# apple/ml-neuman

Measured on AMD Instinct MI355X. Metric: rays_per_sec (800x800 frame, 128 samples/ray coarse + 128 importance, NeuMan background NeRF), higher is better.
Workload: dtype coarse (sampling) pass: split-fp16 hi+lo MFMA x3, f32 accumulate; fine (shading) pass: per-row-scaled int16 as two int8 limbs on the i8 MFMA x3, exact int32 accumulate, encodings on split bf16

## Files before the change

include/neuman_hip.h:

```cpp
#ifndef NEUMAN_HIP_H
#define NEUMAN_HIP_H

#include <stdint.h>

#ifdef __cplusplus
extern "C" {
#endif

#define NM_OK 0
#define NM_ERR_ARG (-1)
#define NM_ERR_HIP (-2)
#define NM_ERR_UNSUPPORTED (-3)

#define NM_ABI_VERSION 1

typedef void* nm_stream_t;

#define NM_PREC_FP32 0
#define NM_PREC_BF16X3 1
#define NM_PREC_BF16 2
#define NM_PREC_I8X3 3
#define NM_PREC_FP16X3 4

#define NM_PE_POSENC 0
#define NM_PE_ROTATE 1

int nm_version(void);
const char* nm_last_error(void);
int nm_device_count(void);

int nm_ray_to_samples(const float* origin, const float* direction, const float* near, const float* far,
                      int64_t R, int S, const float* t_vals, int lindisp, const float* t_rand,
                      float* pts, float* dirs, float* z_vals, nm_stream_t stream);

int nm_z_to_points(const float* origin, const float* direction, const float* z_vals, int64_t R, int S,
                   float* pts, float* dirs, nm_stream_t stream);

int nm_composite(const float* raw, const float* z_vals, const float* rays_d, int64_t R, int S, int white_bkg,
                 const float* noise, float* rgb, float* disp, float* acc, float* weights, float* depth,
                 nm_stream_t stream);

int nm_sample_pdf(const float* bins, const float* weights, int64_t R, int B, const float* u, int N,
                  float* samples, nm_stream_t stream);
int nm_importance_z(const float* z_vals, const float* weights, int64_t R, int S, const float* u, int N,
                    int including_old, float* z_out, nm_stream_t stream);

int nm_near_far(const float* origin, const float* direction, int64_t R, const float* verts, int V, double geo_threshold,
                float* near, float* far, nm_stream_t stream);
int64_t nm_compact_workspace_ints(int64_t R);
int nm_compact_hits(const float* near, const float* far, int64_t R, int32_t* hit_idx, int32_t* miss_idx,
                    int32_t* counts, int32_t* workspace, nm_stream_t stream);

typedef struct nm_mlp_s* nm_mlp_t;

typedef struct nm_mlp_desc {
    int32_t depth;
    int32_t width;
    int32_t skip;
    int32_t pe_kind;
    int32_t pos_n_freqs;
    int32_t dir_n_freqs;
    int32_t plain_head;
} nm_mlp_desc;

int64_t nm_mlp_pack_bytes(const nm_mlp_desc* desc);
int nm_mlp_pack(const nm_mlp_desc* desc, const float* const* host_params, void* host_out);
int nm_mlp_pack_f16(const nm_mlp_desc* desc, const float* const* host_params, void* host_out);
int64_t nm_mlp_pack_i8_bytes(const nm_mlp_desc* desc);
int nm_mlp_pack_i8(const nm_mlp_desc* desc, const float* const* host_params, void* host_out);
int64_t nm_mlp_pack_i8s_bytes(const nm_mlp_desc* desc);
int nm_mlp_pack_i8s(const nm_mlp_desc* desc, const float* const* host_params, void* host_out);
int nm_mlp_create(const nm_mlp_desc* desc, const float* const* host_params, const float* host_pos_tab,
                  const float* host_dir_tab, nm_mlp_t* out);
int nm_mlp_destroy(nm_mlp_t mlp);

int nm_mlp_forward(nm_mlp_t mlp, const float* pts, const float* dirs, int64_t n, int precision,
                   float sigma_scale, float* out, nm_stream_t stream);
int nm_mlp_refresh_f16(nm_mlp_t mlp, const float* const* dev_params, nm_stream_t stream);
int nm_mlp_forward_save(nm_mlp_t mlp, const float* pts, const float* dirs, int64_t n, float* save_h, float* save_hv,
                        float* out, nm_stream_t stream);
int nm_mlp_forward_save_bits(nm_mlp_t mlp, const float* pts, const float* dirs, int64_t n, float* save_h, float* save_hv,
                             uint32_t* save_bits, float* out, nm_stream_t stream);
int64_t nm_mlp_backward_chain_workspace_floats(int64_t n);
int nm_mlp_backward_chain(nm_mlp_t mlp, const float* const* dev_params, const float* dz_top, const float* d_feat, const float* d_raw,
                          const float* acts, const uint32_t* relu_bits, int64_t n, float* dz_out, float* bias_grads, float* workspace,
                          int64_t workspace_floats, nm_stream_t stream);
int nm_mlp_forward_save16(nm_mlp_t mlp, const float* pts, const float* dirs, int64_t n, uint16_t* save_h16, float* save_feat, uint16_t* save_feat16,
                          float* save_hv, uint32_t* save_bits, uint32_t* save_hvbits, uint16_t* save_x0h, uint16_t* save_d0h, float* out,
                          nm_stream_t stream);
int nm_mlp_backward_chain16(nm_mlp_t mlp, const float* const* dev_params, const float* d_feat, const float* d_raw, const uint32_t* relu_bits,
                            int64_t n, const float* amax, uint16_t* dz16, uint16_t* dfeat16, float* dz32_layer5, float* dz32_layer0,
                            float* bias_grads, float* workspace, int64_t workspace_floats, nm_stream_t stream);
int nm_mlp_backward_plain16(nm_mlp_t mlp, const float* const* dev_params, const float* d_out, const uint32_t* relu_bits, int64_t n, const float* amax,
                            uint16_t* dz16, float* dz32_layer5, float* dz32_layer0, float* bias_grads, float* workspace, int64_t workspace_floats,
                            nm_stream_t stream);
int nm_mlp_backward_net16(nm_mlp_t mlp, const float* const* dev_params, const float* d_raw, const float* d_feat_add, const uint32_t* relu_bits,
                          const uint32_t* hv_bits, int64_t n, const float* amax, uint16_t* dz16, uint16_t* dfeat16, uint16_t* dhv16, float* dz32_layer5, float* dz32_layer0,
                          float* dhv32, float* bias_grads, float* workspace, int64_t workspace_floats, nm_stream_t stream);
int nm_mlp_forward_rays(nm_mlp_t mlp, const float* origin, const float* direction, const float* z_vals,
                        int64_t R, int S, int precision, float sigma_scale, float* out, nm_stream_t stream);
int nm_mlp_sigma_rays(nm_mlp_t mlp, const float* origin, const float* direction, const float* z_vals,
                      int64_t R, int S, int precision, float sigma_scale, float* out, nm_stream_t stream);
int nm_mlp_forward_ray_chunk(nm_mlp_t mlp, const float* origin, const float* direction, const float* z_vals, int S_total,
                             const int32_t* ray_idx, const int32_t* n_rays_dev, int64_t n_rays, int s0, int S, int precision,
                             float sigma_scale, float* out, nm_stream_t stream);
int nm_mlp_sigma_ray_chunk(nm_mlp_t mlp, const float* origin, const float* direction, const float* z_vals, int S_total,
                           const int32_t* ray_idx, const int32_t* n_rays_dev, int64_t n_rays, int s0, int S, int precision,
                           float sigma_scale, float* out, nm_stream_t stream);
float nm_occ_probe_offset(int probes, int seed, int k, int axis);
int64_t nm_occ_build_workspace_floats(int res, int probes);
int nm_occ_build(nm_mlp_t mlp, const float* aabb, int res, int probes, int dilate, float sigma_threshold, int seed, int precision,
                 float* workspace, int64_t workspace_floats, uint32_t* bits, nm_stream_t stream);
int64_t nm_occ_compact_workspace_ints(int64_t n_samples);
int nm_occ_compact_samples(const uint32_t* bits, int res, const float* aabb, const float* origin, const float* direction, const float* z_vals,
                           int64_t R, int S, int32_t* sample_idx, int32_t* counts, int32_t* workspace, nm_stream_t stream);
int nm_mlp_forward_samples(nm_mlp_t mlp, const float* origin, const float* direction, const float* z_vals, int64_t R, int S,
                           const int32_t* sample_idx, const int32_t* n_dev, int64_t n_max, int precision, float sigma_scale, float* out,
                           nm_stream_t stream);
int nm_mlp_sigma_samples(nm_mlp_t mlp, const float* origin, const float* direction, const float* z_vals, int64_t R, int S,
                         const int32_t* sample_idx, const int32_t* n_dev, int64_t n_max, int precision, float sigma_scale, float* out,
                         nm_stream_t stream);
int nm_occ_compact_points(const uint32_t* bits, int res, const float* aabb, const float* pts, int64_t n, int32_t* point_idx, int32_t* counts,
                          int32_t* workspace, nm_stream_t stream);
int nm_mlp_forward_listed(nm_mlp_t mlp, const float* pts, const float* dirs, int64_t n_points, const int32_t* point_idx, const int32_t* n_dev,
                          int64_t n_max, int precision, float sigma_scale, float* out, nm_stream_t stream);
int nm_transmittance_chunk(const float* raw, const float* z_vals, const float* rays_d, const int32_t* ray_idx, const int32_t* n_rays_dev,
                           int64_t n_rays, int s0, int S, int S_total, float* T, nm_stream_t stream);
int nm_transmittance_chunk_dz(const float* raw, const float* dz, const float* rays_d, const int32_t* ray_idx, const int32_t* n_rays_dev,
                              int64_t n_rays, int s0, int S, int S_total, float* T, nm_stream_t stream);
int nm_mlp_sigma_f16t_debug(nm_mlp_t mlp, const float* pts, const float* dirs, int64_t n, int stage, float* state, float* out, nm_stream_t stream);
int nm_mlp_forward_debug(nm_mlp_t mlp, const float* pts, const float* dirs, int64_t n, int precision,
                         int stage, float* hidden, nm_stream_t stream);
int nm_mlp_forward_profile(nm_mlp_t mlp, const float* pts, const float* dirs, int64_t n, int precision, float* out,
                           uint64_t* cycles, nm_stream_t stream);

#define NM_SEARCH_TREE 0
#define NM_SEARCH_ALL 1
#define NM_SEARCH_TREE_WIDE 2
typedef struct nm_mesh_s* nm_mesh_t;
int nm_mesh_create(const float* verts, int V, const int32_t* faces, int F, int search, nm_mesh_t* out,
                   nm_stream_t stream);
int nm_mesh_update(nm_mesh_t mesh, const float* verts, nm_stream_t stream);
int nm_mesh_destroy(nm_mesh_t mesh);
int nm_mesh_info(nm_mesh_t mesh, int32_t* levels, int64_t* nodes, int64_t* bytes);
int nm_warp_to_canonical(nm_mesh_t mesh, const float* pts, int64_t R, int S, const double* T, float* can_pts,
                         float* can_dirs, float* closest, nm_stream_t stream);
int nm_signed_distance(nm_mesh_t mesh, const float* pts, int64_t N, float* sdist, int32_t* face, float* closest,
                       nm_stream_t stream);

int nm_warp_apply_forward(const float* T, const int32_t* tri, const float* bary, const float* pts, int64_t N, float* can, nm_stream_t stream);
int nm_warp_apply_backward(const float* T, const int32_t* tri, const float* bary, const float* pts, const float* g_can, int64_t N, int64_t V,
                           float* g_T, float* g_bary, nm_stream_t stream);
int nm_bary_forward(const float* verts, const int32_t* tri, const float* closest, int64_t N, float* bary, nm_stream_t stream);
int nm_bary_backward(const float* verts, const int32_t* tri, const float* closest, const float* g_bary, int64_t N, int64_t V, float* g_verts,
                     nm_stream_t stream);

typedef struct nm_smpl_s* nm_smpl_t;
int nm_smpl_create(const float* v_template, const float* shapedirs, const float* j_regressor, const int32_t* parents,
                   const float* lbs_weights, const float* da_pose, int V, int J, int NB, nm_smpl_t* out);
int nm_smpl_destroy(nm_smpl_t smpl);
int64_t nm_smpl_vertex_workspace_floats(nm_smpl_t smpl);
int nm_smpl_vertex_forward(nm_smpl_t smpl, const float* pose, const float* beta, const double* alignment, double scale, const float* da_pose,
                           float* workspace, float* world_out, float* T_out, nm_stream_t stream);
int nm_smpl_vertex_backward(nm_smpl_t smpl, const float* pose, const float* beta, const double* alignment, double scale, const float* da_pose,
                            const float* g_world, const float* g_T, float* workspace, float* g_pose, float* g_beta, float* g_align,
                            nm_stream_t stream);
int nm_smpl_frames(nm_smpl_t smpl, const float* poses, const float* betas, const double* alignments, int B, double scale,
                   int precise, double* T_out, float* world_out, float* static_out, nm_stream_t stream);

int64_t nm_render_rays_bkg_workspace_floats(int64_t R, int S, int N);
int nm_render_rays_bkg(nm_mlp_t coarse, nm_mlp_t fine, const float* origin, const float* direction, const float* near, const float* far,
                       int64_t R, int S, int N, const float* t_vals, const float* u, int white_bkg, int precision_coarse, int precision_fine,
                       float* workspace, float* raw_out, float* z_out, float* rgb, float* depth, float* acc, nm_stream_t stream);
int64_t nm_render_rays_human_workspace_floats(int64_t R, int S, int posed);
int nm_render_rays_human(nm_mlp_t human, nm_mesh_t mesh, const double* T, const float* origin, const float* direction, const float* near,
                         const float* far, int64_t R, int S, const float* t_vals, int white_bkg, float sigma_scale, int precision,
                         float* workspace, float* raw_out, float* z_out, float* rgb, float* depth, float* acc, nm_stream_t stream);
int64_t nm_render_rays_human_occ_workspace_floats(int64_t R, int S, int posed);
int nm_render_rays_human_occ(nm_mlp_t human, nm_mesh_t mesh, const double* T, const uint32_t* bits, int res, const float* aabb, const float* origin,
                             const float* direction, const float* near, const float* far, int64_t R, int S, const float* t_vals, int white_bkg,
                             float sigma_scale, int precision, float* workspace, float* raw_out, float* z_out, int32_t* counts, float* rgb, float* depth,
                             float* acc, nm_stream_t stream);
int64_t nm_render_rays_hybrid_workspace_floats(int64_t R, int S, int N, int S_human);
int nm_render_rays_hybrid(nm_mlp_t coarse, nm_mlp_t fine, nm_mlp_t human, nm_mesh_t mesh, const double* T, const float* verts, int V,
                          double geo_threshold, const float* origin, const float* direction, int64_t R, float bkg_near, float bkg_far, int S, int N,
                          int S_human, const float* t_vals, const float* u, const float* t_vals_human, int white_bkg, int precision_coarse,
                          int precision_fine, int precision_human, float* workspace, float* rgb, float* depth, float* acc, nm_stream_t stream);
int nm_merge_composite_lists(int k, const float* const* z, const float* const* raw, const int32_t* const* rows, const int* S, int64_t R,
                             const float* rays_d, int white_bkg, float* rgb, float* depth, float* acc, nm_stream_t stream);
int nm_importance_from_raw(const float* raw, const float* z_vals, const float* rays_d, int64_t R, int S, const float* u, int N, float* z_out,
                           float* weights_out, nm_stream_t stream);
int nm_merged_intervals(int k, const float* const* z, const int* S, int64_t R, float* const* dz, nm_stream_t stream);
int64_t nm_merge_composite_workspace_floats(int64_t R, int Sa, int Sb);
int nm_merge_composite(const float* za, const float* rawa, int Sa, const float* zb, const float* rawb, int Sb, int64_t R, const float* rays_d,
                       int white_bkg, float* workspace, float* rgb, float* depth, float* acc, nm_stream_t stream);

int nm_merge_sorted(const float* za, const float* rawa, int Sa, const float* zb, const float* rawb, int Sb,
                    int64_t R, float* z_out, float* raw_out, nm_stream_t stream);

int nm_gather_rows(const float* src, const int32_t* idx, const int32_t* n_dev, int64_t n_max, int width,
                   float* dst, nm_stream_t stream);
int nm_scatter_rows(const float* src, const int32_t* idx, const int32_t* n_dev, int64_t n_max, int width,
                    float* dst, nm_stream_t stream);

int nm_shot_rays(const int32_t* xy, int64_t n, int width, int mode, const double* inv_intrinsic,
                 const double* cam2world, float* origin, float* direction, nm_stream_t stream);

int nm_shot_rays_cams(const int32_t* xy, const int32_t* cam_id, int64_t n, int mode, const double* cams,
                      int n_cams, float* origin, float* direction, nm_stream_t stream);

int nm_frame_to_uint8(const float* src, int64_t n, uint8_t* dst, nm_stream_t stream);
int nm_ssd_u8(const uint8_t* a, const uint8_t* b, int64_t n, uint64_t* ssd, nm_stream_t stream);
#define NM_SSIM_WORKSPACE_DOUBLES 4096
int nm_ssim_u8(const uint8_t* a, const uint8_t* b, int H, int W, int C, double* ssim, double* workspace, nm_stream_t stream);

#define NM_GEMM_ACCUMULATE 1
#define NM_GEMM_BIAS 2
#define NM_GEMM_RELU 4
#define NM_GEMM_MASK 8
#define NM_GEMM_COLSUM 16
int64_t nm_gemm_workspace_floats(int M, int N, int K);
int nm_gemm_f32(int a_kmajor, int b_kmajor, int M, int N, int K, const float* A, int lda, const float* B, int ldb, float* C,
                int ldc, const float* bias, const float* mask, int ldmask, int flags, float* workspace,
                int64_t workspace_floats, nm_stream_t stream);
int nm_gemm_bf16x3(int a_kmajor, int b_kmajor, int M, int N, int K, const float* A, int lda, const float* B, int ldb, float* C,
                   int ldc, const float* bias, const float* mask, int ldmask, int flags, float* workspace,
                   int64_t workspace_floats, nm_stream_t stream);
int nm_gemm_fp16x3(int a_kmajor, int b_kmajor, int M, int N, int K, const float* A, int lda, const float* B, int ldb, float* C,
                   int ldc, const float* bias, const float* mask, int ldmask, int flags, float* workspace,
                   int64_t workspace_floats, nm_stream_t stream);
int nm_pe_encode(const float* x, int64_t n, int dims, int kind, int n_freqs, const float* table, float* out, int ld,
                 nm_stream_t stream);
int nm_pe_encode16(const float* x, int64_t n, int dims, int kind, int n_freqs, const float* table, uint16_t* out, int ld, int ones_col,
                   nm_stream_t stream);
int nm_absmax(const float* x, int64_t count, float* out_max, nm_stream_t stream);
int64_t nm_wgrad16_workspace_floats(int nprod, int64_t n, int p_cols, int q_cols);
int nm_wgrad16(int nprod, int p_cols, int q_cols, const uint16_t* const* dz16, const uint16_t* const* act16, float* const* dW, const int* ldw,
               int64_t n, const float* amax, float* workspace, int64_t workspace_floats, nm_stream_t stream);
int64_t nm_wgrad_heads16_workspace_floats(int64_t n);
int nm_wgrad_heads16(const float* d_raw, const uint16_t* h16_7, const float* hv, int64_t n, float* out644, float* amax, float* workspace,
                     int64_t workspace_floats, nm_stream_t stream);
int64_t nm_wgrad_out16_workspace_floats(int64_t n);
int nm_wgrad_out16(const float* d_out, const uint16_t* h16_7, int64_t n, float* out1028, float* amax, float* workspace, int64_t workspace_floats,
                   nm_stream_t stream);
int64_t nm_wgrad_alpha16_workspace_floats(int64_t n);
int nm_wgrad_alpha16(const float* d_raw, const uint16_t* h16, int64_t n, float* out, float* workspace, int64_t workspace_floats,
                     nm_stream_t stream);
int64_t nm_colsum_workspace_floats(int64_t n, int W);
int nm_colsum(const float* X, int64_t n, int W, int ld, float* out, float* workspace, int64_t workspace_floats, nm_stream_t stream);
int nm_pe_backward(const float* x, int64_t n, int dims, int kind, int n_freqs, const float* table, const float* g, int ld,
                   float* dx, nm_stream_t stream);
int nm_composite_backward(const float* raw, const float* z_vals, const float* rays_d, int64_t R, int S, int white_bkg,
                          const float* g_rgb, const float* g_acc, const float* g_depth, const float* g_weights,
// ... 15 lines not shown
```

ml-neuman_amd/csrc/mlp_host.hip:

```cpp
#include <math.h>
#include <stdarg.h>
#include <stdio.h>
#include <stdlib.h>
#include <string.h>

#include <algorithm>
#include <vector>

#include "common.h"
#include "mlp_layout.h"
#include "mlp_launch.h"

namespace nm {

static thread_local char g_err[512] = "";

void set_error(const char* fmt, ...) {
    va_list ap;
    va_start(ap, fmt);
    vsnprintf(g_err, sizeof(g_err), fmt, ap);
    va_end(ap);
}
int check_hip(hipError_t e, const char* what) {
    if (e == hipSuccess) return NM_OK;
// ... 289 lines not shown
    }
}

static void pack_image8(const nm_mlp_desc* d, const float* const* P, uint8_t* img) {
    memset(img, 0, (size_t)image8_bytes());
    float* units = reinterpret_cast<float*>(img + kWeightBytes8 + kWeightPadBytes);
    float* bias = units + kBiasFloats;
    float* kappa = bias + kBiasFloats;
    const int kpe = 3 + 6 * d->pos_n_freqs, kdpe = 3 + 6 * d->dir_n_freqs;
    std::vector<double> est_in(288, 0.0), est(288, 0.0);
    for (int st = 0; st < kStages; ++st) {
        const StageShape8 sh = stage_shape8(st);
        const int nh = sh.i8steps * 32;
        const int nrows = sh.nblk * 32;
        float* u = units + stage_b_off(st);
        float* b = bias + stage_b_off(st);
        if (st <= 7) memcpy(b, P[P_PTS_W + 2 * st + 1], 256 * 4);
        else if (d->plain_head) { if (st == 8) memcpy(b + 256, P[P_OUT_B], 4 * 4); }
        else if (st == 8) { memcpy(b, P[P_FEAT_B], 256 * 4); b[256] = P[P_ALPHA_B][0]; }
        else if (st == 9) memcpy(b, P[P_VIEWS_B], 128 * 4);
        else memcpy(b, P[P_RGB_B], 3 * 4);
        kappa[st] = 1.f;
        for (int n = 0; n < nrows; ++n) u[n] = 1.f;
        for (int n = 0; n < nrows; ++n) {
            double v = (double)b[n] * b[n];
            const float* pe = nullptr;
            int npe = 0;
            if (st == 0) { pe = P[P_PTS_W] + (int64_t)n * kpe; npe = kpe; }
            else if (st == 5) { pe = P[P_PTS_W + 10] + (int64_t)n * (kpe + 256); npe = kpe; }
            else if (st == 9 && !d->plain_head) { pe = P[P_VIEWS_W] + (int64_t)n * (256 + kdpe) + 256; npe = kdpe; }
            for (int f = 0; f < npe; ++f) v += (double)pe[f] * pe[f];
            int col0 = 0;
            const float* row = sh.i8steps ? hidden_row(d, P, st, n, &col0) : nullptr;
            if (row) for (int f = 0; f < nh; ++f) { const double w = (double)row[col0 + f] * est_in[f]; v += w * w; }
            est[n] = sqrt(v);
        }
        if (sh.i8steps) {
            const float* uin = units + stage_b_off(st - 1);
            std::vector<float> q(nrows, 0.f);
            float kap = 0.f;
            for (int n = 0; n < nrows; ++n) {
                int col0 = 0;
                const float* row = hidden_row(d, P, st, n, &col0);
                float mx = 0.f;
                if (row) for (int f = 0; f < nh; ++f) mx = fmaxf(mx, fabsf(row[col0 + f] * uin[f]));
                q[n] = mx / (float)kFixedMax;
            }
            std::vector<double> stored;
            for (int n = 0; n < nrows; ++n) if (q[n] > 0.f) stored.push_back(est[n] / q[n]);
            if (!stored.empty()) {
                std::nth_element(stored.begin(), stored.begin() + stored.size() / 2, stored.end());
                const double cap = (double)kUnitOutlier * stored[stored.size() / 2];
                for (int n = 0; n < nrows; ++n) {
                    int col0 = 0;
                    if (hidden_row(d, P, st, n, &col0) && cap > 0.0 && est[n] > cap * q[n]) q[n] = (float)(est[n] / cap);
                }
            }
            const int nxt = st == 10 ? -1 : st + 1, nfeed = st == 9 ? 128 : 256;
            if (nxt > 0 && !(d->plain_head && nxt > 8)) {
                std::vector<double> c(nfeed, 0.0), g;
                for (int m = 0; m < stage_shape8(nxt).nblk * 32; ++m) {
                    int col0 = 0;
                    const float* row = hidden_row(d, P, nxt, m, &col0);
                    if (row) for (int n = 0; n < nfeed; ++n) c[n] = fmax(c[n], fabs((double)row[col0 + n]));
                }
                for (int n = 0; n < nfeed; ++n) if (q[n] > 0.f && c[n] > 0.0) g.push_back(q[n] * c[n]);
                if (!g.empty()) {
                    std::nth_element(g.begin(), g.begin() + g.size() / 2, g.end());
                    const double med = g[g.size() / 2], top = *std::max_element(g.begin(), g.end());
                    if (top > (double)kBalanceFrom * med) {
                        std::vector<double> qs;
                        double qtop = 0.0;
                        for (int n = 0; n < nfeed; ++n) if (q[n] > 0.f && c[n] > 0.0) { qs.push_back(q[n]); if (q[n] * c[n] == top) qtop = q[n]; }
                        std::nth_element(qs.begin(), qs.begin() + qs.size() / 2, qs.end());
                        const bool row_outlier = qtop > (double)kBalanceFrom * qs[qs.size() / 2];
                        const double floor_g = row_outlier ? sqrt(top * med) : cbrt(top * med * med);
                        for (int n = 0; n < nfeed; ++n)
                            if (q[n] > 0.f && c[n] > 0.0 && q[n] * c[n] < floor_g) q[n] = (float)(floor_g / c[n]);
                    }
                }
            }
            for (int n = 0; n < nrows; ++n) kap = fmaxf(kap, q[n]);
            if (!(kap > 0.f)) kap = 1.f;
            kappa[st] = kap;
            for (int n = 0; n < nrows; ++n) {
                if (!(q[n] > 0.f)) q[n] = kap;
                u[n] = q[n] / kap;
            }
            for (int nb = 0; nb < sh.nblk; ++nb)
                for (int r = 0; r < 32; ++r) {
                    const int n = 32 * nb + r;
                    int col0 = 0;
                    const float* row = hidden_row(d, P, st, n, &col0);
                    for (int t = 0; t < sh.i8steps; ++t) {
                        int8_t* hi = reinterpret_cast<int8_t*>(img + frag_off8(st, nb, t));
                        int8_t* lo = hi + 1024;
                        for (int g = 0; g < 2; ++g)
                            for (int e = 0; e < 16; ++e) {
                                const int f = slot_feature8(2 * t + g, e);
                                const float w = row ? row[col0 + f] * uin[f] : 0.f;
                                int v = (int)lrintf(w / q[n]);
                                if (v > kFixedMax) v = kFixedMax;
                                if (v < -kFixedMax) v = -kFixedMax;
                                const int l = ((v + 128) & 255) - 128;
                                const int h = (v - l) >> 8;
                                hi[(g * 32 + r) * 16 + e] = (int8_t)h;
                                lo[(g * 32 + r) * 16 + e] = (int8_t)l;
                            }
                    }
                }
        }
        for (int n = 0; n < nrows; ++n) b[n] /= u[n];
        est_in.swap(est);
        for (int nb = 0; nb < sh.nblk; ++nb)
            for (int t = 0; t < sh.bfsteps; ++t) {
                uint16_t* hi = reinterpret_cast<uint16_t*>(img + frag_off8(st, nb, sh.i8steps + t));
                uint16_t* lo = hi + 64 * 8;
                const int cc0 = st == 9 ? 32 : 0;
                for (int lane = 0; lane < 64; ++lane)
                    for (int j = 0; j < 8; ++j) {
                        const int n = 32 * nb + (lane & 31);
                        const float wv = stage_weight(d, P, st, n, cc0 + 2 * t + (lane >> 5), j) / u[n];
                        const uint16_t h = f32_to_bf16(wv);
                        hi[lane * 8 + j] = h;
                        lo[lane * 8 + j] = f32_to_bf16(wv - bf16_to_f32(h));
                    }
            }
    }
}

static void pack_stream8s(const uint8_t* img8, uint8_t* out, bool plain = false) {
    memset(out, 0, (size_t)(kWeightBytes8 + kWeightPadBytes));
    uint8_t* dst = out;
    auto put = [&](int st, int nb, int t0, int n) {
        for (int t = 0; t < n; ++t, dst += kStepBytes) memcpy(dst, img8 + frag_off8(st, nb, t0 + t), (size_t)kStepBytes);
    };
    for (int nb = 0; nb < 8; ++nb) put(0, nb, 0, 4);
    for (int st = 1; st <= 7; ++st) {
        for (int nb = 0; nb < 8; ++nb) put(st, nb, 0, 8);
        if (st == 5)
            for (int nb = 0; nb < 8; ++nb) put(5, nb, 8, 4);
    }
    put(8, 8, 0, 8);
    if (plain) {
        for (int nb = 0; nb < 2; ++nb) { put(0, nb, 0, 4); dst += 4 * kStepBytes; }
        if (dst - out != kPlainStreamBytes8) abort();
        return;
    }
    for (int nb = 0; nb < 8; ++nb) put(8, nb, 0, 8);
    for (int nb = 0; nb < 4; ++nb) put(9, nb, 0, 10);
    put(10, 0, 0, 4);
    if (dst - out != kWeightBytes8) abort();
}

constexpr int kSigmaSteps = 8 * 4 + 6 * 8 * 16 + 8 * 20 + 16;
static void sigma_stream_table(std::vector<int>& tab, int ndir) {
    tab.clear();
    std::vector<int> direct;
    auto put = [&](int st, int b, int t0, int n) {
        for (int t = 0; t < n; ++t)
            for (int k = 0; k < 4; ++k) {
                const int off = (int)frag_off(st, b + (k >> 1), t0 + t) + 1024 * (k & 1);
                (k < 4 - ndir ? tab : direct).push_back(off);
            }
    };
    for (int st = 0; st <= 7; ++st) {
        const StageShape sh = stage_shape(st);
        for (int b = 0; b < 8; b += 2) {
            if (sh.pe_steps) put(st, b, 0, sh.pe_steps);
            for (int t0 = sh.pe_steps; t0 < sh.steps; t0 += 8) put(st, b, t0, 8);
        }
    }
    for (int t = 0; t < 16; ++t) { tab.push_back((int)frag_off(8, 8, t)); tab.push_back((int)frag_off(8, 8, t) + 1024); }
    tab.insert(tab.end(), direct.begin(), direct.end());
    if ((int)tab.size() != 2 * kSigmaSteps) abort();
}
__global__ void sigma_stream_kernel(const uint4* __restrict__ image, const int* __restrict__ tab, int npieces, uint4* __restrict__ out) {
    const int i = blockIdx.x * blockDim.x + threadIdx.x;
    if (i >= npieces * 64) return;
    out[i] = image[tab[i >> 6] / 16 + (i & 63)];
}

static void pack_stream8(const uint8_t* img8, uint8_t* out) {
    memset(out, 0, (size_t)kWeightBytes8w);
    for (int q = 0; q < 4; ++q) {
        uint8_t* dst = out + wstream_off(q);
        auto put = [&](int st, int nb, int t0, int n) {
            for (int t = 0; t < n; ++t, dst += kStepBytes) memcpy(dst, img8 + frag_off8(st, nb, t0 + t), (size_t)kStepBytes);
        };
        put(0, 2 * q, 0, 4); put(0, 2 * q + 1, 0, 4);
        for (int st = 1; st <= 8; ++st) {
            put(st, 2 * q, 0, 8); put(st, 2 * q + 1, 0, 8);
            if (st == 5) { put(5, 2 * q, 8, 4); put(5, 2 * q + 1, 8, 4); }
        }
        if (q < 2) put(8, 8, 0, 8);
        put(9, q, 0, 8); put(9, q, 8, 2);
        dst += 2 * kStepBytes;
        if (q < 2) put(10, 0, 0, 4);
        dst += kW8Pad * kStepBytes;
        if (dst != out + wstream_off(q) + (int64_t)wstream_steps(q) * kStepBytes) abort();
    }
}

}

struct nm_mlp_s {
    nm_mlp_desc desc;
    uint8_t* d_image;
    uint8_t* d_image16;
    float* d_consts8;
    uint8_t* d_stream8;
    uint8_t* d_image8;
    uint8_t* d_stream16t;
    int* d_sigma_tab;
    uint8_t* d_bwd_image;
    int sigma_ndir;
    float* d_petab;
    float* d_ref;
    float* d_wscale16;
    int ref_off[12], ref_boff[12];
    int pos_octaves, dir_octaves;
};

extern "C" {

int nm_version(void) { return NM_ABI_VERSION; }
const char* nm_last_error(void) { return nm::g_err; }
int nm_device_count(void) {
    int n = 0;
    if (hipGetDeviceCount(&n) != hipSuccess) { (void)hipGetLastError(); return 0; }
    return n;
}

int64_t nm_mlp_pack_bytes(const nm_mlp_desc* desc) {
    if (nm::validate_desc(desc) != NM_OK) return -1;
    return nm::image_bytes();
}

int nm_mlp_pack(const nm_mlp_desc* desc, const float* const* host_params, void* host_out) {
    if (int e = nm::validate_desc(desc)) return e;
    NM_REQUIRE(host_params && host_out, "nm_mlp_pack: null pointer");
    for (int i = 0; i < (desc->plain_head ? 18 : 24); ++i) NM_REQUIRE(host_params[i], "nm_mlp_pack: host_params[%d] is null", i);
    if (int e = nm::check_finite("nm_mlp_pack", desc, host_params)) return e;
    nm::pack_image(desc, host_params, static_cast<uint8_t*>(host_out));
    return NM_OK;
}

int nm_mlp_pack_f16(const nm_mlp_desc* desc, const float* const* host_params, void* host_out) {
    if (int e = nm::validate_desc(desc)) return e;
    NM_REQUIRE(host_params && host_out, "nm_mlp_pack_f16: null pointer");
    for (int i = 0; i < (desc->plain_head ? 18 : 24); ++i) NM_REQUIRE(host_params[i], "nm_mlp_pack_f16: host_params[%d] is null", i);
    if (int e = nm::check_finite("nm_mlp_pack_f16", desc, host_params)) return e;
    nm::pack_image(desc, host_params, static_cast<uint8_t*>(host_out), true);
    return NM_OK;
}

int64_t nm_mlp_pack_i8_bytes(const nm_mlp_desc* desc) {
    if (nm::validate_desc(desc) != NM_OK) return -1;
    return nm::image8_bytes();
}

int nm_mlp_pack_i8(const nm_mlp_desc* desc, const float* const* host_params, void* host_out) {
    if (int e = nm::validate_desc(desc)) return e;
    NM_REQUIRE(host_params && host_out, "nm_mlp_pack_i8: null pointer");
    for (int i = 0; i < (desc->plain_head ? 18 : 24); ++i) NM_REQUIRE(host_params[i], "nm_mlp_pack_i8: host_params[%d] is null", i);
    if (int e = nm::check_finite("nm_mlp_pack_i8", desc, host_params)) return e;
    nm::pack_image8(desc, host_params, static_cast<uint8_t*>(host_out));
    return NM_OK;
}

int64_t nm_mlp_pack_i8s_bytes(const nm_mlp_desc* desc) {
    if (nm::validate_desc(desc) != NM_OK) return -1;
    return nm::kWeightBytes8 + nm::kWeightPadBytes;
}

int nm_mlp_pack_i8s(const nm_mlp_desc* desc, const float* const* host_params, void* host_out) {
    if (int e = nm::validate_desc(desc)) return e;
    NM_REQUIRE(host_params && host_out, "nm_mlp_pack_i8s: null pointer");
    for (int i = 0; i < (desc->plain_head ? 18 : 24); ++i) NM_REQUIRE(host_params[i], "nm_mlp_pack_i8s: host_params[%d] is null", i);
    if (int e = nm::check_finite("nm_mlp_pack_i8s", desc, host_params)) return e;
    std::vector<uint8_t> img8((size_t)nm::image8_bytes());
    nm::pack_image8(desc, host_params, img8.data());
    nm::pack_stream8s(img8.data(), static_cast<uint8_t*>(host_out), desc->plain_head != 0);
    return NM_OK;
}

int nm_mlp_create(const nm_mlp_desc* desc, const float* const* host_params, const float* host_pos_tab,
                  const float* host_dir_tab, nm_mlp_t* out) {
    if (int e = nm::validate_desc(desc)) return e;
    NM_REQUIRE(host_params && host_pos_tab && host_dir_tab && out, "nm_mlp_create: null pointer");
    const int plain = desc->plain_head;
    for (int i = 0; i < (plain ? 18 : 24); ++i) NM_REQUIRE(host_params[i], "nm_mlp_create: host_params[%d] is null", i);
    if (int e = nm::check_finite("nm_mlp_create", desc, host_params)) return e;
    const int64_t bytes = nm_mlp_pack_bytes(desc);
    std::vector<uint8_t> img((size_t)bytes);
    nm::pack_image(desc, host_params, img.data());
    std::vector<uint8_t> img16((size_t)bytes);
    nm::pack_image(desc, host_params, img16.data(), true);
    std::vector<uint8_t> img8((size_t)nm::image8_bytes());
    std::vector<uint8_t> str8((size_t)nm::kWeightBytes8w);
    std::vector<uint8_t> str8s((size_t)(nm::kWeightBytes8 + nm::kWeightPadBytes));
    nm::pack_image8(desc, host_params, img8.data());
    nm::pack_stream8(img8.data(), str8.data());
    nm::pack_stream8s(img8.data(), str8s.data(), plain != 0);

    const int kpe = 3 + 6 * desc->pos_n_freqs, kdpe = 3 + 6 * desc->dir_n_freqs;
    const int K[12] = {kpe, 256, 256, 256, 256, kpe + 256, 256, 256, plain ? 0 : 256 + kdpe, plain ? 0 : 256, 256, plain ? 0 : 128};
    const int N[12] = {256, 256, 256, 256, 256, 256, 256, 256, plain ? 0 : 128, plain ? 0 : 256, plain ? 4 : 1, plain ? 0 : 3};
    const int src[12] = {0, 2, 4, 6, 8, 10, 12, 14, 16, 18, plain ? (int)nm::P_OUT_W : 20, 22};
    nm_mlp_s* m = new nm_mlp_s();
    m->desc = *desc;
    int woff = 0;
    for (int l = 0; l < 12; ++l) { m->ref_off[l] = woff; woff += K[l] * N[l]; }
    int boff = woff;
    for (int l = 0; l < 12; ++l) { m->ref_boff[l] = boff; boff += N[l]; }
    std::vector<float> ref((size_t)boff);
    for (int l = 0; l < 12; ++l) {
        if (!K[l]) continue;
        const float* W = host_params[src[l]];
        for (int k = 0; k < K[l]; ++k)
            for (int n = 0; n < N[l]; ++n) ref[m->ref_off[l] + (size_t)k * N[l] + n] = W[(size_t)n * K[l] + k];
        memcpy(&ref[m->ref_boff[l]], host_params[src[l] + 1], (size_t)N[l] * 4);
    }
    float tab[192];
    memset(tab, 0, sizeof(tab));
    const int npos = desc->pe_kind == NM_PE_POSENC ? desc->pos_n_freqs : 9 * desc->pos_n_freqs;
    const int ndir = desc->pe_kind == NM_PE_POSENC ? desc->dir_n_freqs : 9 * desc->dir_n_freqs;
    memcpy(tab, host_pos_tab, (size_t)npos * 4);
    memcpy(tab + 96, host_dir_tab, (size_t)ndir * 4);
    auto octaves = [&](const float* t, int nfreq) {
        const int per = desc->pe_kind == NM_PE_POSENC ? 1 : 9;
        for (int b = 0; b + 1 < nfreq; ++b)
            for (int k = 0; k < per; ++k)
                if (t[(b + 1) * per + k] != 2.f * t[b * per + k]) return 0;
        return 1;
    };
    m->pos_octaves = octaves(tab, desc->pos_n_freqs);
    m->dir_octaves = octaves(tab + 96, desc->dir_n_freqs);

    m->d_image = nullptr; m->d_image16 = nullptr; m->d_consts8 = nullptr; m->d_stream8 = nullptr; m->d_image8 = nullptr; m->d_stream16t = nullptr; m->d_sigma_tab = nullptr; m->d_bwd_image = nullptr; m->d_petab = nullptr; m->d_ref = nullptr; m->d_wscale16 = nullptr;
    int rc = nm::check_hip(hipMalloc(&m->d_image, (size_t)bytes), "nm_mlp_create: hipMalloc(image)");
    const size_t consts_off = (size_t)(nm::kWeightBytes8 + nm::kWeightPadBytes), consts_bytes = img8.size() - consts_off;
    if (!rc) rc = nm::check_hip(hipMalloc(&m->d_consts8, consts_bytes), "nm_mlp_create: hipMalloc(consts8)");
    if (!rc) rc = nm::check_hip(hipMemcpy(m->d_consts8, img8.data() + consts_off, consts_bytes, hipMemcpyHostToDevice), "nm_mlp_create: upload consts8");
    if (!rc) rc = nm::check_hip(hipMalloc(&m->d_stream8, str8.size()), "nm_mlp_create: hipMalloc(stream8)");
    if (!rc) rc = nm::check_hip(hipMemcpy(m->d_stream8, str8.data(), str8.size(), hipMemcpyHostToDevice), "nm_mlp_create: upload stream8");
    if (!rc) rc = nm::check_hip(hipMalloc(&m->d_image8, consts_off), "nm_mlp_create: hipMalloc(image8)");
    if (!rc) rc = nm::check_hip(hipMemcpy(m->d_image8, str8s.data(), consts_off, hipMemcpyHostToDevice), "nm_mlp_create: upload image8");
    if (!rc) rc = nm::check_hip(hipMalloc(&m->d_petab, sizeof(tab)), "nm_mlp_create: hipMalloc(petab)");
    if (!rc) rc = nm::check_hip(hipMalloc(&m->d_ref, ref.size() * 4), "nm_mlp_create: hipMalloc(ref)");
    if (!rc) rc = nm::check_hip(hipMemcpy(m->d_image, img.data(), (size_t)bytes, hipMemcpyHostToDevice), "nm_mlp_create: upload image");
    if (!rc) rc = nm::check_hip(hipMalloc(&m->d_image16, (size_t)bytes), "nm_mlp_create: hipMalloc(image16)");
    if (!rc) rc = nm::check_hip(hipMemcpy(m->d_image16, img16.data(), (size_t)bytes, hipMemcpyHostToDevice), "nm_mlp_create: upload image16");
    if (!rc) rc = nm::check_hip(hipMemcpy(m->d_petab, tab, sizeof(tab), hipMemcpyHostToDevice), "nm_mlp_create: upload petab");
    if (!rc) rc = nm::check_hip(hipMemcpy(m->d_ref, ref.data(), ref.size() * 4, hipMemcpyHostToDevice), "nm_mlp_create: upload ref");
    if (!rc && !plain) {
        std::vector<int> stab;
        m->sigma_ndir = nm::sigma_f16t_ndir();
        nm::sigma_stream_table(stab, m->sigma_ndir);
        rc = nm::check_hip(hipMalloc(&m->d_sigma_tab, stab.size() * sizeof(int)), "nm_mlp_create: hipMalloc(sigma table)");
        if (!rc) rc = nm::check_hip(hipMemcpy(m->d_sigma_tab, stab.data(), stab.size() * sizeof(int), hipMemcpyHostToDevice), "nm_mlp_create: upload sigma table");
        if (!rc) rc = nm::check_hip(hipMalloc(&m->d_stream16t, (size_t)nm::kSigmaSteps * nm::kStepBytes), "nm_mlp_create: hipMalloc(stream16t)");
        if (!rc) {
            const int n16 = nm::kSigmaSteps * (nm::kStepBytes / 16);
            hipLaunchKernelGGL(nm::sigma_stream_kernel, dim3((n16 + 255) / 256), dim3(256), 0, 0, reinterpret_cast<const uint4*>(m->d_image16), m->d_sigma_tab,
                               2 * nm::kSigmaSteps, reinterpret_cast<uint4*>(m->d_stream16t));
            rc = nm::check_launch("sigma_stream_kernel");
            if (!rc) rc = nm::check_hip(hipDeviceSynchronize(), "nm_mlp_create: sigma stream");
        }
    }
    if (rc) { nm_mlp_destroy(m); return rc; }
    *out = m;
    return NM_OK;
}

int nm_mlp_refresh_f16(nm_mlp_t m, const float* const* dev_params, nm_stream_t stream) {
    NM_REQUIRE(m && dev_params, "nm_mlp_refresh_f16: null pointer");
    nm::DevParams P;
    const int need = m->desc.plain_head ? 18 : 24;
    for (int i = 0; i < 24; ++i) {
        NM_REQUIRE(i >= need || dev_params[i], "nm_mlp_refresh_f16: dev_params[%d] is null", i);
        P.p[i] = i < need ? dev_params[i] : nullptr;
    }
    if (!m->d_wscale16)
        if (int rc = nm::check_hip(hipMalloc(&m->d_wscale16, 3 * nm::kStages * sizeof(float)), "nm_mlp_refresh_f16: hipMalloc")) return rc;
    hipStream_t st = nm::as_stream(stream);
    float* bias = reinterpret_cast<float*>(m->d_image16 + nm::kWeightBytes + nm::kWeightPadBytes);
    unsigned* scale_work = reinterpret_cast<unsigned*>(m->d_wscale16 + nm::kStages);
    if (int rc = nm::check_hip(hipMemsetAsync(scale_work, 0, 2 * nm::kStages * sizeof(unsigned), st), "nm_mlp_refresh_f16: clear")) return rc;
    hipLaunchKernelGGL(nm::f16_stage_scale_kernel, dim3(nm::kStages, nm::kScaleSlices), dim3(1024), 0, st, m->desc, P, scale_work, m->d_wscale16);
    const int threads = (int)(nm::kWeightBytes / nm::kStepBytes) * 64;
    hipLaunchKernelGGL(nm::f16_pack_kernel, dim3((threads + 255) / 256), dim3(256), 0, st, m->desc, P, m->d_wscale16, m->d_image16);
    hipLaunchKernelGGL(nm::f16_bias_kernel, dim3((nm::kBiasFloats + nm::kF16TabFloats + 255) / 256), dim3(256), 0, st, P, m->d_wscale16, bias, m->desc.plain_head);
    if (m->d_stream16t) {
        const int n16 = nm::kSigmaSteps * (nm::kStepBytes / 16);
        hipLaunchKernelGGL(nm::sigma_stream_kernel, dim3((n16 + 255) / 256), dim3(256), 0, st, reinterpret_cast<const uint4*>(m->d_image16), m->d_sigma_tab,
                           2 * nm::kSigmaSteps, reinterpret_cast<uint4*>(m->d_stream16t));
    }
    return nm::check_launch("nm_mlp_refresh_f16");
}

int nm_mlp_destroy(nm_mlp_t m) {
    if (!m) return NM_OK;
    if (m->d_image) (void)hipFree(m->d_image);
    if (m->d_image16) (void)hipFree(m->d_image16);
    if (m->d_consts8) (void)hipFree(m->d_consts8);
    if (m->d_stream8) (void)hipFree(m->d_stream8);
    if (m->d_image8) (void)hipFree(m->d_image8);
    if (m->d_stream16t) (void)hipFree(m->d_stream16t);
    if (m->d_sigma_tab) (void)hipFree(m->d_sigma_tab);
    if (m->d_bwd_image) (void)hipFree(m->d_bwd_image);
    if (m->d_petab) (void)hipFree(m->d_petab);
    if (m->d_ref) (void)hipFree(m->d_ref);
    if (m->d_wscale16) (void)hipFree(m->d_wscale16);
    delete m;
    return NM_OK;
}

static int mlp_dispatch(nm_mlp_t m, const float* pts, const float* dirs, const float* origin, const float* direction,
                        const float* z, int64_t n, int S, int in_mode, int precision, int stop_stage, float sigma_scale,
                        float* out, float* dbg, nm_stream_t stream, void* prof = nullptr, int sigma_only = 0,
                        const nm::MlpChunk* chunk = nullptr) {
    NM_REQUIRE(m, "nm_mlp_forward: null handle");
    NM_REQUIRE(n >= 0, "nm_mlp_forward: negative n");
    NM_REQUIRE(precision == NM_PREC_FP32 || precision == NM_PREC_BF16X3 || precision == NM_PREC_BF16 || precision == NM_PREC_I8X3 ||
                   precision == NM_PREC_FP16X3,
               "nm_mlp_forward: bad precision %d", precision);
    if (n == 0) return NM_OK;
    NM_REQUIRE(!(chunk && precision == NM_PREC_FP32), "nm_mlp_forward_ray_chunk: the exact-f32 validation kernel has no chunked form");
    NM_REQUIRE(!(m->desc.plain_head && precision == NM_PREC_I8X3 && (stop_stage != -2 || dbg || prof || sigma_only)),
               "nm_mlp_forward: the plain-head (use_viewdirs=False) net's i8x3 form is the whole-network launch only (no stage-by-stage / density-only form)");
    NM_REQUIRE(!(m->desc.plain_head && stop_stage > 7), "nm_mlp_forward_debug: the plain-head net has stages -1..7 only");
    if (precision == NM_PREC_FP32) {
        nm::RefLaunch L;
        L.plain_head = m->desc.plain_head;
        L.wt = m->d_ref; L.bias = m->d_ref; L.petab = m->d_petab;
        for (int i = 0; i < 12; ++i) { L.off[i] = m->ref_off[i]; L.boff[i] = m->ref_boff[i]; }
        L.pe_kind = m->desc.pe_kind; L.pos_nfreq = m->desc.pos_n_freqs; L.dir_nfreq = m->desc.dir_n_freqs;
        return nm::launch_mlp_ref(L, pts, dirs, origin, direction, z, n, S, in_mode, stop_stage, sigma_scale, out, dbg,
                                  nm::as_stream(stream));
    }
    nm::MlpLaunch L;
    L.wpack = m->d_image;
    L.bias = reinterpret_cast<const float*>(m->d_image + nm::kWeightBytes + nm::kWeightPadBytes);
    L.wpack16 = m->d_image16;
    L.bias16 = reinterpret_cast<const float*>(m->d_image16 + nm::kWeightBytes + nm::kWeightPadBytes);
    L.petab = m->d_petab;
    L.pe_kind = m->desc.pe_kind; L.pos_nfreq = m->desc.pos_n_freqs; L.dir_nfreq = m->desc.dir_n_freqs;
    L.pos_octaves = m->pos_octaves; L.dir_octaves = m->dir_octaves;
    L.plain_head = m->desc.plain_head;
    L.wstream8 = m->d_stream8;
    L.consts8 = m->d_consts8;
    static const bool i8_as = [] { const char* e = getenv("NEUMAN_I8_KERNEL"); return !e || !strcmp(e, "as"); }();
    const char* sk = getenv("NEUMAN_SIGMA_KERNEL");
    const bool sigma_t = !(sk && !strcmp(sk, "w")) && m->d_stream16t;
    if (sigma_t && precision == NM_PREC_FP16X3 && sigma_only == 1 && stop_stage == -2 && !dbg && !prof && !m->desc.plain_head)
        return nm::launch_sigma_f16t(L, m->d_stream16t, m->sigma_ndir, pts, dirs, origin, direction, z, n, S, in_mode, sigma_scale, out, nm::as_stream(stream), chunk, nullptr, -1);
    if ((i8_as || m->desc.plain_head) && precision == NM_PREC_I8X3 && stop_stage == -2 && !dbg && !prof && !sigma_only)
        return nm::launch_mlp_i8s(L, m->d_image8, pts, dirs, origin, direction, z, n, S, in_mode, sigma_scale, out, nm::as_stream(stream), chunk);
    return nm::launch_mlp_mfma(L, pts, dirs, origin, direction, z, n, S, in_mode, precision, stop_stage, sigma_scale, out, dbg,
                               prof, nm::as_stream(stream), sigma_only, chunk);
}

int nm_mlp_forward(nm_mlp_t mlp, const float* pts, const float* dirs, int64_t n, int precision, float sigma_scale,
                   float* out, nm_stream_t stream) {
    NM_REQUIRE(n == 0 || (pts && dirs && out), "nm_mlp_forward: null pointer");
    NM_REQUIRE((reinterpret_cast<uintptr_t>(out) & 15) == 0, "nm_mlp_forward: out must be 16-byte aligned");
    return mlp_dispatch(mlp, pts, dirs, nullptr, nullptr, nullptr, n, 1, 0, precision, -2, sigma_scale, out, nullptr, stream);
}

int nm_mlp_forward_save(nm_mlp_t m, const float* pts, const float* dirs, int64_t n, float* save_h, float* save_hv, float* out,
                        nm_stream_t stream) {
    return nm_mlp_forward_save_bits(m, pts, dirs, n, save_h, save_hv, nullptr, out, stream);
}

static int forward_save_impl(nm_mlp_t m, const float* pts, const float* dirs, int64_t n, float* save_h, float* save_hv, uint32_t* save_bits,
                             void* save_h16, float* out, nm_stream_t stream, void* save_feat16 = nullptr, uint32_t* save_hvbits = nullptr,
                             void* save_x0h = nullptr, void* save_d0h = nullptr) {
    NM_REQUIRE(m, "nm_mlp_forward_save: null handle");
    NM_REQUIRE(n >= 0, "nm_mlp_forward_save: negative n");
    if (n == 0) return NM_OK;
    const bool plain = m->desc.plain_head != 0;
    NM_REQUIRE(!plain || (save_h16 && !save_h && !save_feat16 && !save_hvbits && !save_d0h), "nm_mlp_forward_save: the plain-head net keeps save_h16 / save_bits / save_x0h only");
    NM_REQUIRE(pts && (dirs || plain) && (plain || ((save_h || (save_h16 && save_feat16)) && save_hv)) && out, "nm_mlp_forward_save: null pointer");
    NM_REQUIRE(((reinterpret_cast<uintptr_t>(out) | reinterpret_cast<uintptr_t>(save_h) | reinterpret_cast<uintptr_t>(save_hv) | reinterpret_cast<uintptr_t>(save_h16) |
                 reinterpret_cast<uintptr_t>(save_feat16)) & 15) == 0, "nm_mlp_forward_save: outputs must be 16-byte aligned");
    nm::MlpLaunch L;
    L.wpack = m->d_image;
    L.bias = reinterpret_cast<const float*>(m->d_image + nm::kWeightBytes + nm::kWeightPadBytes);
    L.wpack16 = m->d_image16;
    L.bias16 = reinterpret_cast<const float*>(m->d_image16 + nm::kWeightBytes + nm::kWeightPadBytes);
    L.petab = m->d_petab;
    L.pe_kind = m->desc.pe_kind; L.pos_nfreq = m->desc.pos_n_freqs; L.dir_nfreq = m->desc.dir_n_freqs;
    L.pos_octaves = m->pos_octaves; L.dir_octaves = m->dir_octaves;
    L.plain_head = plain ? 1 : 0;
    L.wstream8 = m->d_stream8;
    L.consts8 = m->d_consts8;
    L.save_h = save_h; L.save_hv = save_hv; L.save_bits = save_bits; L.save_h16 = save_h16; L.save_feat16 = save_feat16; L.save_hvbits = save_hvbits; L.save_x0h = save_x0h; L.save_d0h = save_d0h;
    return nm::launch_mlp_mfma(L, pts, dirs ? dirs : pts, nullptr, nullptr, nullptr, n, 1, 0, NM_PREC_FP16X3, -2, 1.f, out, nullptr, nullptr,
                               nm::as_stream(stream), 0, nullptr);
}

int nm_mlp_forward_save_bits(nm_mlp_t m, const float* pts, const float* dirs, int64_t n, float* save_h, float* save_hv, uint32_t* save_bits,
                             float* out, nm_stream_t stream) {
    return forward_save_impl(m, pts, dirs, n, save_h, save_hv, save_bits, nullptr, out, stream);
}

int nm_mlp_forward_save16(nm_mlp_t m, const float* pts, const float* dirs, int64_t n, uint16_t* save_h16, float* save_feat, uint16_t* save_feat16,
                          float* save_hv, uint32_t* save_bits, uint32_t* save_hvbits, uint16_t* save_x0h, uint16_t* save_d0h, float* out, nm_stream_t stream) {
    NM_REQUIRE(n == 0 || (save_h16 && save_bits && (save_feat || save_feat16 || (m && m->desc.plain_head))), "nm_mlp_forward_save16: null pointer");
    NM_REQUIRE(((reinterpret_cast<uintptr_t>(save_x0h) | reinterpret_cast<uintptr_t>(save_d0h)) & 15) == 0, "nm_mlp_forward_save16: outputs must be 16-byte aligned");
    return forward_save_impl(m, pts, dirs, n, save_feat, save_hv, save_bits, save_h16, out, stream, save_feat16, save_hvbits, save_x0h, save_d0h);
}

int64_t nm_mlp_backward_chain_workspace_floats(int64_t n) { return ((n + nm::kTileM - 1) / nm::kTileM) * 9 * 256; }

int nm_mlp_backward_chain(nm_mlp_t m, const float* const* dev_params, const float* dz_top, const float* d_feat, const float* d_raw, const float* acts,
                          const uint32_t* relu_bits, int64_t n, float* dz_out, float* bias_grads, float* workspace, int64_t workspace_floats,
                          nm_stream_t stream) {
    NM_REQUIRE(m && dev_params, "nm_mlp_backward_chain: null pointer");
    NM_REQUIRE(n >= 0, "nm_mlp_backward_chain: negative n");
    if (n == 0) return NM_OK;
    NM_REQUIRE((dz_top || (d_feat && d_raw)) && (acts || relu_bits) && dz_out && bias_grads && workspace, "nm_mlp_backward_chain: null pointer");
    NM_REQUIRE(!d_feat || !m->desc.plain_head, "nm_mlp_backward_chain: the plain-head net has no feature layer (pass dz_top)");
    NM_REQUIRE(workspace_floats >= nm_mlp_backward_chain_workspace_floats(n), "nm_mlp_backward_chain: workspace of %lld floats, %lld needed",
               (long long)workspace_floats, (long long)nm_mlp_backward_chain_workspace_floats(n));
    NM_REQUIRE(((reinterpret_cast<uintptr_t>(dz_top) | reinterpret_cast<uintptr_t>(d_feat) | reinterpret_cast<uintptr_t>(d_raw) | reinterpret_cast<uintptr_t>(acts) |
                 reinterpret_cast<uintptr_t>(dz_out) | reinterpret_cast<uintptr_t>(workspace)) & 15) == 0, "nm_mlp_backward_chain: buffers must be 16-byte aligned");
    nm::DevParams P;
    const int need = d_feat ? 24 : 16;
    for (int i = 0; i < 24; ++i) {
        NM_REQUIRE(i >= need || dev_params[i], "nm_mlp_backward_chain: dev_params[%d] is null", i);
        P.p[i] = i < need ? dev_params[i] : nullptr;
    }
    if (!m->d_bwd_image)
        if (int rc = nm::check_hip(hipMalloc(&m->d_bwd_image, (size_t)nm::mlp_bwd_image_bytes()), "nm_mlp_backward_chain: hipMalloc")) return rc;
    return nm::launch_mlp_bwd(P, 3 + 6 * m->desc.pos_n_freqs, m->d_bwd_image, dz_top, d_feat, d_raw, acts, relu_bits, n, dz_out, workspace, bias_grads,
                              nm::as_stream(stream));
}

int nm_mlp_backward_chain16(nm_mlp_t m, const float* const* dev_params, const float* d_feat, const float* d_raw, const uint32_t* relu_bits, int64_t n,
                            const float* amax, uint16_t* dz16, uint16_t* dfeat16, float* dz32_layer5, float* dz32_layer0, float* bias_grads,
                            float* workspace, int64_t workspace_floats, nm_stream_t stream) {
    NM_REQUIRE(m && dev_params, "nm_mlp_backward_chain16: null pointer");
    NM_REQUIRE(n >= 0, "nm_mlp_backward_chain16: negative n");
    if (n == 0) return NM_OK;
    NM_REQUIRE(d_feat && d_raw && relu_bits && amax && dz16 && bias_grads && workspace, "nm_mlp_backward_chain16: null pointer");
    NM_REQUIRE(!m->desc.plain_head, "nm_mlp_backward_chain16: the plain-head net has no feature layer");
    NM_REQUIRE(workspace_floats >= nm_mlp_backward_chain_workspace_floats(n), "nm_mlp_backward_chain16: workspace of %lld floats, %lld needed",
               (long long)workspace_floats, (long long)nm_mlp_backward_chain_workspace_floats(n));
    NM_REQUIRE(((reinterpret_cast<uintptr_t>(d_feat) | reinterpret_cast<uintptr_t>(d_raw) | reinterpret_cast<uintptr_t>(dz16) | reinterpret_cast<uintptr_t>(dfeat16) |
                 reinterpret_cast<uintptr_t>(dz32_layer5) | reinterpret_cast<uintptr_t>(dz32_layer0) | reinterpret_cast<uintptr_t>(workspace)) & 15) == 0,
               "nm_mlp_backward_chain16: buffers must be 16-byte aligned");
    nm::DevParams P;
    for (int i = 0; i < 24; ++i) {
        NM_REQUIRE(dev_params[i], "nm_mlp_backward_chain16: dev_params[%d] is null", i);
        P.p[i] = dev_params[i];
    }
    if (!m->d_bwd_image)
        if (int rc = nm::check_hip(hipMalloc(&m->d_bwd_image, (size_t)nm::mlp_bwd_image_bytes()), "nm_mlp_backward_chain16: hipMalloc")) return rc;
    nm::Bwd16 h;
    h.dz16 = dz16; h.dfeat16 = dfeat16; h.amax = amax;
    for (int i = 0; i < 8; ++i) h.dz32[i] = nullptr;
    h.dz32[5] = dz32_layer5; h.dz32[0] = dz32_layer0;
    return nm::launch_mlp_bwd(P, 3 + 6 * m->desc.pos_n_freqs, m->d_bwd_image, nullptr, d_feat, d_raw, nullptr, relu_bits, n, nullptr, workspace, bias_grads,
                              nm::as_stream(stream), &h);
}

int nm_mlp_backward_net16(nm_mlp_t m, const float* const* dev_params, const float* d_raw, const float* d_feat_add, const uint32_t* relu_bits,
                          const uint32_t* hv_bits, int64_t n, const float* amax, uint16_t* dz16, uint16_t* dfeat16, uint16_t* dhv16, float* dz32_layer5, float* dz32_layer0, float* dhv32,
                          float* bias_grads, float* workspace, int64_t workspace_floats, nm_stream_t stream) {
    NM_REQUIRE(m && dev_params, "nm_mlp_backward_net16: null pointer");
    NM_REQUIRE(n >= 0, "nm_mlp_backward_net16: negative n");
    if (n == 0) return NM_OK;
    NM_REQUIRE(d_raw && relu_bits && hv_bits && amax && dz16 && dfeat16 && dhv16 && bias_grads && workspace, "nm_mlp_backward_net16: null pointer");
    NM_REQUIRE(!m->desc.plain_head, "nm_mlp_backward_net16: the plain-head net has no views layer");
    NM_REQUIRE(workspace_floats >= nm_mlp_backward_chain_workspace_floats(n), "nm_mlp_backward_net16: workspace of %lld floats, %lld needed",
               (long long)workspace_floats, (long long)nm_mlp_backward_chain_workspace_floats(n));
    NM_REQUIRE(((reinterpret_cast<uintptr_t>(d_raw) | reinterpret_cast<uintptr_t>(d_feat_add) | reinterpret_cast<uintptr_t>(dz16) | reinterpret_cast<uintptr_t>(dfeat16) |
                 reinterpret_cast<uintptr_t>(dhv16) | reinterpret_cast<uintptr_t>(dz32_layer5) | reinterpret_cast<uintptr_t>(dz32_layer0) | reinterpret_cast<uintptr_t>(dhv32) |
                 reinterpret_cast<uintptr_t>(workspace)) & 15) == 0, "nm_mlp_backward_net16: buffers must be 16-byte aligned");
    nm::DevParams P;
    for (int i = 0; i < 24; ++i) {
        NM_REQUIRE(dev_params[i], "nm_mlp_backward_net16: dev_params[%d] is null", i);
        P.p[i] = dev_params[i];
    }
    NM_REQUIRE((reinterpret_cast<uintptr_t>(P.p[nm::P_RGB_W]) & 15) == 0, "nm_mlp_backward_net16: rgb_linear.weight must be 16-byte aligned");
    if (!m->d_bwd_image)
        if (int rc = nm::check_hip(hipMalloc(&m->d_bwd_image, (size_t)nm::mlp_bwd_image_bytes()), "nm_mlp_backward_net16: hipMalloc")) return rc;
    nm::Bwd16 h;
    h.dz16 = dz16; h.dfeat16 = dfeat16; h.amax = amax;
    for (int i = 0; i < 8; ++i) h.dz32[i] = nullptr;
    h.dz32[5] = dz32_layer5; h.dz32[0] = dz32_layer0;
    h.hvbits = hv_bits; h.dhv16 = dhv16; h.dhv32 = dhv32; h.kdir = 3 + 6 * m->desc.dir_n_freqs;
    return nm::launch_mlp_bwd(P, 3 + 6 * m->desc.pos_n_freqs, m->d_bwd_image, nullptr, d_feat_add, d_raw, nullptr, relu_bits, n, nullptr, workspace, bias_grads,
                              nm::as_stream(stream), &h);
}

int nm_mlp_backward_plain16(nm_mlp_t m, const float* const* dev_params, const float* d_out, const uint32_t* relu_bits, int64_t n, const float* amax,
                            uint16_t* dz16, float* dz32_layer5, float* dz32_layer0, float* bias_grads, float* workspace, int64_t workspace_floats,
                            nm_stream_t stream) {
    NM_REQUIRE(m && dev_params, "nm_mlp_backward_plain16: null pointer");
    NM_REQUIRE(n >= 0, "nm_mlp_backward_plain16: negative n");
    if (n == 0) return NM_OK;
    NM_REQUIRE(d_out && relu_bits && amax && dz16 && bias_grads && workspace, "nm_mlp_backward_plain16: null pointer");
    NM_REQUIRE(m->desc.plain_head, "nm_mlp_backward_plain16: the net has the view-dependent head (nm_mlp_backward_net16)");
    NM_REQUIRE(workspace_floats >= nm_mlp_backward_chain_workspace_floats(n), "nm_mlp_backward_plain16: workspace of %lld floats, %lld needed",
               (long long)workspace_floats, (long long)nm_mlp_backward_chain_workspace_floats(n));
    NM_REQUIRE(((reinterpret_cast<uintptr_t>(d_out) | reinterpret_cast<uintptr_t>(dz16) | reinterpret_cast<uintptr_t>(dz32_layer5) | reinterpret_cast<uintptr_t>(dz32_layer0) |
                 reinterpret_cast<uintptr_t>(workspace)) & 15) == 0, "nm_mlp_backward_plain16: buffers must be 16-byte aligned");
    nm::DevParams P;
    for (int i = 0; i < 24; ++i) {
        NM_REQUIRE(i >= 18 || dev_params[i], "nm_mlp_backward_plain16: dev_params[%d] is null", i);
        P.p[i] = i < 18 ? dev_params[i] : nullptr;
    }
    if (!m->d_bwd_image)
        if (int rc = nm::check_hip(hipMalloc(&m->d_bwd_image, (size_t)nm::mlp_bwd_image_bytes()), "nm_mlp_backward_plain16: hipMalloc")) return rc;
    nm::Bwd16 h;
    h.dz16 = dz16; h.dfeat16 = nullptr; h.amax = amax;
    for (int i = 0; i < 8; ++i) h.dz32[i] = nullptr;
    h.dz32[5] = dz32_layer5; h.dz32[0] = dz32_layer0;
    h.plain = 1;
    return nm::launch_mlp_bwd(P, 3 + 6 * m->desc.pos_n_freqs, m->d_bwd_image, nullptr, nullptr, d_out, nullptr, relu_bits, n, nullptr, workspace, bias_grads,
                              nm::as_stream(stream), &h);
}

int nm_mlp_forward_rays(nm_mlp_t mlp, const float* origin, const float* direction, const float* z_vals, int64_t R, int S,
                        int precision, float sigma_scale, float* out, nm_stream_t stream) {
    NM_REQUIRE(R == 0 || (origin && direction && z_vals && out), "nm_mlp_forward_rays: null pointer");
    NM_REQUIRE(R >= 0 && S >= 1, "nm_mlp_forward_rays: bad sizes");
    NM_REQUIRE((reinterpret_cast<uintptr_t>(out) & 15) == 0, "nm_mlp_forward_rays: out must be 16-byte aligned");
    return mlp_dispatch(mlp, nullptr, nullptr, origin, direction, z_vals, R * (int64_t)S, S, 1, precision, -2, sigma_scale, out,
                        nullptr, stream);
}

int nm_mlp_sigma_rays(nm_mlp_t mlp, const float* origin, const float* direction, const float* z_vals, int64_t R, int S,
                      int precision, float sigma_scale, float* out, nm_stream_t stream) {
    NM_REQUIRE(R == 0 || (origin && direction && z_vals && out), "nm_mlp_sigma_rays: null pointer");
    NM_REQUIRE(R >= 0 && S >= 1, "nm_mlp_sigma_rays: bad sizes");
    NM_REQUIRE((reinterpret_cast<uintptr_t>(out) & 15) == 0, "nm_mlp_sigma_rays: out must be 16-byte aligned");
    return mlp_dispatch(mlp, nullptr, nullptr, origin, direction, z_vals, R * (int64_t)S, S, 1, precision, -2, sigma_scale, out,
                        nullptr, stream, nullptr, 1);
}

int nm_mlp_forward_ray_chunk(nm_mlp_t mlp, const float* origin, const float* direction, const float* z_vals, int S_total,
                             const int32_t* ray_idx, const int32_t* n_rays_dev, int64_t n_rays, int s0, int S, int precision,
                             float sigma_scale, float* out, nm_stream_t stream) {
    NM_REQUIRE(n_rays == 0 || (origin && direction && z_vals && ray_idx && out), "nm_mlp_forward_ray_chunk: null pointer");
    NM_REQUIRE(n_rays >= 0 && S >= 1 && s0 >= 0 && s0 + S <= S_total, "nm_mlp_forward_ray_chunk: bad sizes (s0=%d S=%d S_total=%d)", s0, S, S_total);
    NM_REQUIRE((reinterpret_cast<uintptr_t>(out) & 15) == 0, "nm_mlp_forward_ray_chunk: out must be 16-byte aligned");
    nm::MlpChunk c{ray_idx, n_rays_dev, s0, S_total};
    return mlp_dispatch(mlp, nullptr, nullptr, origin, direction, z_vals, n_rays * (int64_t)S, S, 2, precision, -2, sigma_scale, out,
                        nullptr, stream, nullptr, 0, &c);
}

int nm_mlp_sigma_ray_chunk(nm_mlp_t mlp, const float* origin, const float* direction, const float* z_vals, int S_total,
                           const int32_t* ray_idx, const int32_t* n_rays_dev, int64_t n_rays, int s0, int S, int precision,
                           float sigma_scale, float* out, nm_stream_t stream) {
    NM_REQUIRE(n_rays == 0 || (origin && direction && z_vals && ray_idx && out), "nm_mlp_sigma_ray_chunk: null pointer");
    NM_REQUIRE(n_rays >= 0 && S >= 1 && s0 >= 0 && s0 + S <= S_total, "nm_mlp_sigma_ray_chunk: bad sizes (s0=%d S=%d S_total=%d)", s0, S, S_total);
    NM_REQUIRE((reinterpret_cast<uintptr_t>(out) & 15) == 0, "nm_mlp_sigma_ray_chunk: out must be 16-byte aligned");
    nm::MlpChunk c{ray_idx, n_rays_dev, s0, S_total};
    return mlp_dispatch(mlp, nullptr, nullptr, origin, direction, z_vals, n_rays * (int64_t)S, S, 2, precision, -2, sigma_scale, out,
                        nullptr, stream, nullptr, 1, &c);
}

static int forward_samples(const char* what, int sigma_only, nm_mlp_t mlp, const float* origin, const float* direction, const float* z_vals, int64_t R,
                           int S, const int32_t* sample_idx, const int32_t* n_dev, int64_t n_max, int precision, float sigma_scale, float* out,
                           nm_stream_t stream) {
    NM_REQUIRE(n_max == 0 || (origin && direction && z_vals && sample_idx && out), "%s: null pointer", what);
    NM_REQUIRE(R >= 0 && S >= 1 && n_max >= 0 && n_max <= R * (int64_t)S && R * (int64_t)S < (1ll << 31), "%s: bad sizes (R=%lld S=%d n_max=%lld)", what,
               (long long)R, S, (long long)n_max);
    NM_REQUIRE(precision != NM_PREC_FP32, "%s: the exact-f32 validation kernel has no sample-list form", what);
    NM_REQUIRE((reinterpret_cast<uintptr_t>(out) & 15) == 0, "%s: out must be 16-byte aligned", what);
    nm::MlpChunk c{sample_idx, n_dev, 0, S};
    return mlp_dispatch(mlp, nullptr, nullptr, origin, direction, z_vals, n_max, S, 3, precision, -2, sigma_scale, out, nullptr, stream, nullptr,
                        sigma_only, &c);
}

int nm_mlp_forward_samples(nm_mlp_t mlp, const float* origin, const float* direction, const float* z_vals, int64_t R, int S,
                           const int32_t* sample_idx, const int32_t* n_dev, int64_t n_max, int precision, float sigma_scale, float* out,
                           nm_stream_t stream) {
    return forward_samples("nm_mlp_forward_samples", 0, mlp, origin, direction, z_vals, R, S, sample_idx, n_dev, n_max, precision, sigma_scale, out, stream);
}

int nm_mlp_sigma_samples(nm_mlp_t mlp, const float* origin, const float* direction, const float* z_vals, int64_t R, int S,
                         const int32_t* sample_idx, const int32_t* n_dev, int64_t n_max, int precision, float sigma_scale, float* out,
                         nm_stream_t stream) {
    return forward_samples("nm_mlp_sigma_samples", 1, mlp, origin, direction, z_vals, R, S, sample_idx, n_dev, n_max, precision, sigma_scale, out, stream);
}

}

bool nm::mlp_plain_head(nm_mlp_t m) { return m && m->desc.plain_head; }

extern "C" {

int nm_mlp_forward_listed(nm_mlp_t mlp, const float* pts, const float* dirs, int64_t n_points, const int32_t* point_idx, const int32_t* n_dev,
                          int64_t n_max, int precision, float sigma_scale, float* out, nm_stream_t stream) {
    NM_REQUIRE(n_max == 0 || (pts && dirs && point_idx && out), "nm_mlp_forward_listed: null pointer");
    NM_REQUIRE(n_points >= 0 && n_max >= 0 && n_max <= n_points && n_points < (1ll << 31), "nm_mlp_forward_listed: bad sizes (n_points=%lld n_max=%lld)",
               (long long)n_points, (long long)n_max);
    NM_REQUIRE(precision != NM_PREC_FP32, "nm_mlp_forward_listed: the exact-f32 validation kernel has no point-list form");
    NM_REQUIRE((reinterpret_cast<uintptr_t>(out) & 15) == 0, "nm_mlp_forward_listed: out must be 16-byte aligned");
    nm::MlpChunk c{point_idx, n_dev, 0, 1};
    return mlp_dispatch(mlp, pts, dirs, nullptr, nullptr, nullptr, n_max, 1, 4, precision, -2, sigma_scale, out, nullptr, stream, nullptr, 0, &c);
}

int nm_mlp_forward_profile(nm_mlp_t mlp, const float* pts, const float* dirs, int64_t n, int precision, float* out,
                           uint64_t* cycles, nm_stream_t stream) {
    NM_REQUIRE(n == 0 || (pts && dirs && out && cycles), "nm_mlp_forward_profile: null pointer");
    NM_REQUIRE(precision == NM_PREC_BF16X3 || precision == NM_PREC_I8X3 || precision == NM_PREC_FP16X3,
               "nm_mlp_forward_profile: precision %d has no profiling build",
               precision);
    return mlp_dispatch(mlp, pts, dirs, nullptr, nullptr, nullptr, n, 1, 0, precision, -2, 1.f, out, nullptr, stream, cycles);
}

int nm_mlp_sigma_f16t_debug(nm_mlp_t mlp, const float* pts, const float* dirs, int64_t n, int stage, float* state, float* out, nm_stream_t stream) {
    NM_REQUIRE(mlp && pts && dirs && state && out && n > 0, "nm_mlp_sigma_f16t_debug: null pointer");
    NM_REQUIRE(stage >= 0 && stage % 100 <= 7 && !mlp->desc.plain_head, "nm_mlp_sigma_f16t_debug: stage %d outside 0..7 (+ 100 x tile round)", stage);
    nm::MlpLaunch L;
    L.petab = mlp->d_petab;
    L.pe_kind = mlp->desc.pe_kind; L.pos_nfreq = mlp->desc.pos_n_freqs; L.dir_nfreq = mlp->desc.dir_n_freqs;
    L.pos_octaves = mlp->pos_octaves; L.dir_octaves = mlp->dir_octaves;
    L.plain_head = 0;
    L.bias16 = reinterpret_cast<const float*>(mlp->d_image16 + nm::kWeightBytes + nm::kWeightPadBytes);
    return nm::launch_sigma_f16t(L, mlp->d_stream16t, mlp->sigma_ndir, pts, dirs, nullptr, nullptr, nullptr, n, 1, 0, 1.f, out, nm::as_stream(stream), nullptr, state, stage);
}

int nm_mlp_forward_debug(nm_mlp_t mlp, const float* pts, const float* dirs, int64_t n, int precision, int stage,
                         float* hidden, nm_stream_t stream) {
    NM_REQUIRE(n == 0 || (pts && dirs && hidden), "nm_mlp_forward_debug: null pointer");
    NM_REQUIRE(stage >= -1 && stage <= 9, "nm_mlp_forward_debug: stage %d outside -1..9", stage);
    return mlp_dispatch(mlp, pts, dirs, nullptr, nullptr, nullptr, n, 1, 0, precision, stage, 1.f, nullptr, hidden, stream);
}

}
```

ml-neuman_amd/csrc/mlp_i8as.h:

```cpp
#pragma once
#include "mlp_device.h"

namespace {

typedef __attribute__((ext_vector_type(4))) int i32x4;
typedef __attribute__((ext_vector_type(16))) int i32x16;
typedef __attribute__((ext_vector_type(2))) short i16x2;
typedef __attribute__((address_space(3))) const float lds_cfloat;
typedef __attribute__((ext_vector_type(4))) float vf4;
typedef __attribute__((address_space(3))) const vf4 lds_cvf4;

constexpr int kRows = 32;
struct Args8s {
    MlpArgs a;
    const float* consts8;
    const uint4* image8;
};

__device__ __forceinline__ i32x4 as_i32x4(uint4 v) { return __builtin_bit_cast(i32x4, v); }

template <bool F16 = false>
__device__ __forceinline__ void fill_pe_wave(uint4* pw, bool is_dir, const MlpArgs& a, int64_t base_row, int lane) {
    const PeSpec spec = is_dir ? a.dir : a.pos;
    const float* tab = a.petab + (is_dir ? 96 : 0);
    unsigned short* hi = reinterpret_cast<unsigned short*>(pw);
    auto put = [&](int row, int p, float v, bool clamp = false) {
        const int off = ((p >> 3) * (2 * kRows) + row) * 8 + (p & 7);
        if (F16) {
            float sv = v * kF16ActScale;
            if (clamp) sv = __builtin_amdgcn_fmed3f(sv, -65504.f, 65504.f);
            const _Float16 hb = (_Float16)sv;
            const _Float16 lb = (_Float16)(sv - (float)hb);
            hi[off] = __builtin_bit_cast(unsigned short, hb);
            hi[off + kRows * 8] = __builtin_bit_cast(unsigned short, lb);
            return;
        }
        const bf16x2 hb = __builtin_convertvector((f32x2){v, 0.f}, bf16x2);
        const f32x2 hf = __builtin_convertvector(hb, f32x2);
        const bf16x2 lb = __builtin_convertvector((f32x2){v - hf.x, 0.f}, bf16x2);
        hi[off] = (unsigned short)(__builtin_bit_cast(unsigned, hb) & 0xffffu);
        hi[off + kRows * 8] = (unsigned short)(__builtin_bit_cast(unsigned, lb) & 0xffffu);
    };
    if (spec.octaves) {
#pragma unroll 1
        for (int round = 0; round < 2; ++round) {
            const int j = 2 * round + (lane >> 5), row = lane & 31;
            if (j > 2) break;
            int64_t i = base_row + row;
            if (i >= a.n) i = a.n - 1;
            float x0, x1, x2;
            sample_input(a, i, is_dir, x0, x1, x2);
            const float xj = j == 0 ? x0 : (j == 1 ? x1 : x2);
            const float a0 = spec.kind == NM_PE_POSENC ? xj * tab[0] : fmaf(x2, tab[3 * j + 2], fmaf(x1, tab[3 * j + 1], x0 * tab[3 * j]));
            put(row, j, xj);
            double sn, cs;
            sincos_f64((double)a0, sn, cs);
            const int n3 = 3 * spec.nfreq;
            for (int b = 0; b < spec.nfreq; ++b) {
                if (spec.kind == NM_PE_POSENC) { put(row, 3 + 6 * b + j, (float)sn); put(row, 3 + 6 * b + 3 + j, (float)cs); }
                else { put(row, 3 + 3 * b + j, (float)sn); put(row, 3 + n3 + 3 * b + j, (float)cs); }
                const double s2 = 2.0 * sn * cs, c2 = 1.0 - 2.0 * sn * sn;
                sn = s2; cs = c2;
            }
        }
    } else {
        const int nchunks = is_dir ? 4 : nm::kPeChunks;
        for (int item = lane; item < nchunks * kRows; item += 64) {
            const int c = item >> 5, row = item & 31;
            int64_t i = base_row + row;
            if (i >= a.n) i = a.n - 1;
            float x0, x1, x2;
            sample_input(a, i, is_dir, x0, x1, x2);
#pragma unroll
            for (int e = 0; e < 8; ++e) put(row, 8 * c + e, pe_feature(8 * c + e, x0, x1, x2, spec, tab), true);
        }
    }
}

struct X8 {
    uint4 h[8], l[8];
};

__device__ __forceinline__ void glds16(const void* gsrc, unsigned lds_dst) {
    unsigned keep;
    asm volatile("s_mov_b32 %0, m0\n\ts_mov_b32 m0, %2\n\ts_nop 0\n\tglobal_load_lds_dwordx4 %1, off\n\ts_mov_b32 m0, %0"
                 : "=&s"(keep) : "v"(gsrc), "s"(lds_dst) : "memory");
}
__device__ __forceinline__ void bias16(f32x16& f, lds_cfloat* bias_blk) {
#pragma unroll
    for (int q = 0; q < 4; ++q) {
        const vf4 bs = *(lds_cvf4*)(bias_blk + 8 * q);
        f[4 * q] = bs.x; f[4 * q + 1] = bs.y; f[4 * q + 2] = bs.z; f[4 * q + 3] = bs.w;
    }
}
__device__ __forceinline__ void dequant16(f32x16& f, const i32x16& t, float sx256, lds_cfloat* bias_blk) {
#pragma unroll
    for (int q = 0; q < 4; ++q) {
        const vf4 bs = *(lds_cvf4*)(bias_blk + 8 * q);
        const float bsv[4] = {bs.x, bs.y, bs.z, bs.w};
#pragma unroll
        for (int j = 0; j < 4; ++j) f[4 * q + j] = fmaf((float)t[4 * q + j], sx256, bsv[j]);
    }
}
template <bool RELU>
__device__ __forceinline__ float max16(float m, const f32x16& f) {
#pragma unroll
    for (int r = 0; r < 16; ++r) m = fmaxf(m, RELU ? f[r] : fabsf(f[r]));
    return m;
}
__device__ __forceinline__ float row_max(float m) {
    typedef __attribute__((ext_vector_type(2))) unsigned u32x2;
    const u32x2 sw = __builtin_amdgcn_permlane32_swap(__float_as_uint(m), __float_as_uint(m), false, false);
    return fmaxf(__uint_as_float(sw.x), __uint_as_float(sw.y));
}
template <bool RELU>
__device__ __forceinline__ void quant16(const f32x16& f, float inv, uint4& xh, uint4& xl) {
    i16x2 P[8], Y[8];
#pragma unroll
    for (int i = 0; i < 8; ++i) {
        float y0 = f[2 * i] * inv, y1 = f[2 * i + 1] * inv;
        if (RELU) {
            y0 = __builtin_amdgcn_fmed3f(y0, 0.f, 1.f);
            y1 = __builtin_amdgcn_fmed3f(y1, 0.f, 1.f);
        }
        const i16x2 p = __builtin_amdgcn_cvt_pknorm_i16(y0, y1);
        P[i] = p;
        Y[i] = p + (i16x2){128, 128};
    }
    unsigned lo[4], hi[4];
#pragma unroll
    for (int k = 0; k < 4; ++k) {
        lo[k] = __builtin_amdgcn_perm(__builtin_bit_cast(unsigned, P[2 * k + 1]), __builtin_bit_cast(unsigned, P[2 * k]), 0x06040200u);
        hi[k] = __builtin_amdgcn_perm(__builtin_bit_cast(unsigned, Y[2 * k + 1]), __builtin_bit_cast(unsigned, Y[2 * k]), 0x07050301u);
    }
    xh = make_uint4(hi[0], hi[1], hi[2], hi[3]);
    xl = make_uint4(lo[0], lo[1], lo[2], lo[3]);
}
__device__ __forceinline__ float inv_of(float M) { return M > 0.f ? ((float)nm::kFixedMax / 32767.f) * __builtin_amdgcn_rcpf(M) : 0.f; }
__device__ __forceinline__ float scale_of(float M) { return M > 0.f ? M * (1.f / (float)nm::kFixedMax) : 1.f; }


}
```

ml-neuman_amd/csrc/mlp_i8s.hip:

```cpp
#include "mlp_i8as.h"

namespace {

constexpr int kWaves = 8;
constexpr int kTile = kWaves * kRows;
constexpr int kPWaveU4 = nm::kPeChunks * 2 * kRows;
constexpr int kPeU4 = kWaves * kPWaveU4;
constexpr int kStepU4 = nm::kStepBytes / 16;
constexpr int kSlotU4 = 12 * kStepU4;
constexpr int kSlots = 3;
constexpr int kBiasU4 = (nm::kBiasFloats + 16 + 3) / 4;
constexpr int kTileBlocks = 82;
__host__ __device__ constexpr int block_steps(int i) {
    i = i >= kTileBlocks ? i - kTileBlocks : i;
    return i < 8 ? 4 : i < 77 ? 8 : i < 81 ? 10 : 4;
}
__host__ __device__ constexpr int block_pieces(int nsteps) { return (2 * nsteps + kWaves - 1) / kWaves; }

struct Ring {
    const char* src;
    const uint4* rd;
    unsigned lds0;
    int off;
    int slot;
    int refill, np, nsteps2;
};
__device__ __forceinline__ void ring_piece(const Ring& R, int off, int slot, int j) {
    glds16(R.src + off + j * (kWaves * 1024), __builtin_amdgcn_readfirstlane(R.lds0 + slot * (kSlotU4 * 16) + j * (kWaves * 1024)));
}
__device__ __forceinline__ void ring_advance(Ring& R, int nsteps) {
    R.off += nsteps * nm::kStepBytes;
    if (R.off == (int)nm::kWeightBytes8) R.off = 0;
}
__device__ __forceinline__ const uint4* ring_enter(Ring& R, int i) {
    const int np1 = block_pieces(block_steps(i + 1));
    if (np1 == 1) asm volatile("s_waitcnt vmcnt(1)" ::: "memory");
    else if (np1 == 2) asm volatile("s_waitcnt vmcnt(2)" ::: "memory");
    else asm volatile("s_waitcnt vmcnt(3)" ::: "memory");
    __builtin_amdgcn_s_barrier();
    const uint4* cur = R.rd + R.slot * kSlotU4;
    R.refill = R.slot == 0 ? kSlots - 1 : R.slot - 1;
    R.slot = R.slot == kSlots - 1 ? 0 : R.slot + 1;
    R.np = block_pieces(block_steps(i + 2));
    R.nsteps2 = block_steps(i + 2);
    return cur;
}
__device__ __forceinline__ void ring_copy(Ring& R, int j) {
    if (j < R.np) ring_piece(R, R.off, R.refill, j);
    if (j == R.np - 1) ring_advance(R, R.nsteps2);
}
struct W8 {
    uint4 h, l;
};

template <int NSTEPS, bool PEND, bool RELU = true>
__device__ __forceinline__ void k_i8_impl(i32x16& t, const X8& X, const uint4* ws, Ring& R, f32x16& fp, const i32x16& tp, lds_cfloat* bias_blk,
                                          float sx256, float& m) {
    i32x16 ah, ac;
#pragma unroll
    for (int r = 0; r < 16; ++r) { ah[r] = 0; ac[r] = 0; }
    W8 w[2];
    w[0].h = ws[0]; w[0].l = ws[64];
    w[1].h = ws[kStepU4]; w[1].l = ws[kStepU4 + 64];
#pragma unroll
    for (int s = 0; s < NSTEPS; ++s) {
        const uint4 wh = w[s & 1].h, wl = w[s & 1].l;
        ac = __builtin_amdgcn_mfma_i32_32x32x32_i8(as_i32x4(wh), as_i32x4(X.l[s]), ac, 0, 0, 0);
        ah = __builtin_amdgcn_mfma_i32_32x32x32_i8(as_i32x4(wh), as_i32x4(X.h[s]), ah, 0, 0, 0);
        ac = __builtin_amdgcn_mfma_i32_32x32x32_i8(as_i32x4(wl), as_i32x4(X.h[s]), ac, 0, 0, 0);
        if (s + 2 < NSTEPS) { w[s & 1].h = ws[(s + 2) * kStepU4]; w[s & 1].l = ws[(s + 2) * kStepU4 + 64]; }
        if (s == 0 || s == 2 || s == 4) ring_copy(R, s >> 1);
        if (PEND) {
            const int r = 2 * s;
            const float b0 = bias_blk[8 * (r >> 2) + (r & 3)], b1 = bias_blk[8 * (r >> 2) + (r & 3) + 1];
            const float f0 = fmaf((float)tp[r], sx256, b0), f1 = fmaf((float)tp[r + 1], sx256, b1);
            fp[r] = f0;
            fp[r + 1] = f1;
            m = RELU ? fmaxf(m, fmaxf(f0, f1)) : fmaxf(m, fmaxf(fabsf(f0), fabsf(f1)));
            __builtin_amdgcn_sched_barrier(0);
        }
    }
#pragma unroll
    for (int r = 0; r < 16; ++r) t[r] = (ah[r] << 8) + ac[r];
}
template <int NSTEPS>
__device__ __forceinline__ void k_i8(i32x16& t, const X8& X, const uint4* ws, Ring& R) {
    f32x16 nf;
    float nm_ = 0.f;
    k_i8_impl<NSTEPS, false>(t, X, ws, R, nf, t, nullptr, 0.f, nm_);
}
template <int NSTEPS, bool COPY = false>
__device__ __forceinline__ void k_bf(f32x16& f, const uint4* pw, int g, int s, const uint4* ws, Ring* R = nullptr, int j0 = 0) {
#pragma unroll
    for (int t = 0; t < NSTEPS; ++t) {
        if (COPY && (t == 1 || t == 3)) ring_copy(*R, j0 + (t >> 1));
        const uint4 wh = ws[t * kStepU4], wl = ws[t * kStepU4 + 64];
        const uint4 xh = pw[(2 * t + g) * (2 * kRows) + s], xl = pw[(2 * t + g) * (2 * kRows) + kRows + s];
        f = __builtin_amdgcn_mfma_f32_32x32x16_bf16(as_bf16x8(wh), as_bf16x8(xl), f, 0, 0, 0);
        f = __builtin_amdgcn_mfma_f32_32x32x16_bf16(as_bf16x8(wl), as_bf16x8(xh), f, 0, 0, 0);
        f = __builtin_amdgcn_mfma_f32_32x32x16_bf16(as_bf16x8(wh), as_bf16x8(xh), f, 0, 0, 0);
    }
}
template <bool PLAIN>
__global__ __launch_bounds__(kWaves * 64, 2) void nerf_mlp_i8s_kernel(const Args8s A) {
    __shared__ uint4 lds[kPeU4 + kSlots * kSlotU4 + kBiasU4];
    const MlpArgs a = resolve_args(A.a);
    const int tid = threadIdx.x, lane = tid & 63;
    const int w = __builtin_amdgcn_readfirstlane(tid >> 6);
    const int g = lane >> 5, s = lane & 31;
    uint4* pw = lds + w * kPWaveU4;
    Ring R;
    R.src = reinterpret_cast<const char*>(A.image8) + lane * 16 + w * 1024;
    R.rd = lds + kPeU4 + lane;
    R.lds0 = (unsigned)(uintptr_t)(lds + kPeU4) + w * 1024;
    R.off = 0;
    R.slot = 0;
    {
        float* lb = reinterpret_cast<float*>(lds + kPeU4 + kSlots * kSlotU4);
        for (int i = tid; i < nm::kBiasFloats + 16; i += kWaves * 64) lb[i] = A.consts8[nm::kBiasFloats + i];
    }
    __syncthreads();
    ring_piece(R, 0, 0, 0);
    ring_piece(R, block_steps(0) * nm::kStepBytes, 1, 0);
    R.off = (block_steps(0) + block_steps(1)) * nm::kStepBytes;
    const float u_sigma = A.consts8[nm::stage_b_off(8) + 256];
    const float u_r = A.consts8[nm::stage_b_off(10)], u_g = A.consts8[nm::stage_b_off(10) + 1], u_b = A.consts8[nm::stage_b_off(10) + 2];
    const float* kappa = reinterpret_cast<const float*>(lds + kPeU4 + kSlots * kSlotU4) + nm::kBiasFloats;
    unsigned bias_lds = (unsigned)(uintptr_t)(lds + kPeU4 + kSlots * kSlotU4) + 16 * g;
    asm volatile("" : "+v"(bias_lds));
    lds_cfloat* bias = (lds_cfloat*)(uintptr_t)bias_lds;
    const int64_t ntiles = (a.n + kTile - 1) / kTile;
    for (int i = lane; i < kPWaveU4; i += 64) pw[i] = make_uint4(0, 0, 0, 0);

#pragma unroll 1
    for (int64_t tile = blockIdx.x; tile < ntiles; tile += gridDim.x) {
        const int64_t row0 = tile * kTile + w * kRows;
        fill_pe_wave(pw, false, a, row0, lane);
        X8 X;
        float sx;
        {
            f32x16 f[8];
            float m = 0.f;
#pragma unroll
            for (int b = 0; b < 8; ++b) {
                const uint4* ws = ring_enter(R, b);
                bias16(f[b], bias + nm::stage_b_off(0) + 32 * b);
                k_bf<4, true>(f[b], pw, g, s, ws, &R);
                m = max16<true>(m, f[b]);
            }
            const float M = row_max(m), inv = inv_of(M);
#pragma unroll
            for (int b = 0; b < 8; ++b) quant16<true>(f[b], inv, X.h[b], X.l[b]);
            sx = scale_of(M);
        }
#pragma unroll 1
        for (int st = 1; st <= 7; ++st) {
            const float sxin = sx * (256.f * kappa[st]);
            const int i0 = 8 * st + (st > 5 ? 4 : 0);
            f32x16 f[8];
            float m = 0.f;
            i32x16 tp;
#pragma unroll
            for (int b = 0; b < 8; ++b) {
                const uint4* ws = ring_enter(R, i0 + b);
                if (b == 0) {
                    k_i8<8>(tp, X, ws, R);
                } else {
                    i32x16 t;
                    k_i8_impl<8, true>(t, X, ws, R, f[b - 1], tp, bias + 256 * st + 32 * (b - 1), sxin, m);
                    tp = t;
                }
            }
            dequant16(f[7], tp, sxin, bias + 256 * st + 32 * 7);
            if (st == 5) {
#pragma unroll
                for (int u = 0; u < 4; ++u) {
                    const uint4* ws = ring_enter(R, 48 + u);
                    k_bf<4, true>(f[2 * u], pw, g, s, ws, &R, 0);
                    k_bf<4, true>(f[2 * u + 1], pw, g, s, ws + 4 * kStepU4, &R, 2);
                }
                m = 0.f;
#pragma unroll
                for (int b = 0; b < 7; ++b) m = max16<true>(m, f[b]);
            }
            m = max16<true>(m, f[7]);
            const float M = row_max(m), inv = inv_of(M);
#pragma unroll
            for (int b = 0; b < 8; ++b) quant16<true>(f[b], inv, X.h[b], X.l[b]);
            sx = scale_of(M);
            if (st == 5 && !(PLAIN && a.sigma_only == 2)) {
                fill_pe_wave(pw, true, a, row0, lane);
            }
        }
        if (PLAIN && a.sigma_only == 2) {
            i32x16 t;
            f32x16 fo;
            k_i8<8>(t, X, ring_enter(R, 68), R);
            dequant16(fo, t, sx * (256.f * kappa[8]), bias + nm::stage_b_off(8) + 256);
            const float* up = A.consts8 + nm::stage_b_off(8) + 256;
            const int64_t i = row0 + s;
            if (g == 0 && i < a.n)
                reinterpret_cast<float4*>(a.out)[sample_record(a, i)] = make_float4(fo[0] * up[0], fo[1] * up[1], fo[2] * up[2], fo[3] * up[3] * a.sigma_scale);
            R.off = (block_steps(0) + block_steps(1)) * nm::kStepBytes;
            continue;
        }
        float sigma;
        {
            const float sxin = sx * (256.f * kappa[8]);
            {
                i32x16 t;
                f32x16 fa;
                k_i8<8>(t, X, ring_enter(R, 68), R);
                dequant16(fa, t, sxin, bias + nm::stage_b_off(8) + 256);
                sigma = fa[0] * u_sigma;
            }
            f32x16 f[8];
            float m = 0.f;
#pragma unroll
            for (int b = 0; b < 8; ++b) {
                i32x16 t;
                k_i8<8>(t, X, ring_enter(R, 69 + b), R);
                dequant16(f[b], t, sxin, bias + nm::stage_b_off(8) + 32 * b);
                m = max16<false>(m, f[b]);
            }
            const float M = row_max(m), inv = inv_of(M);
#pragma unroll
            for (int b = 0; b < 8; ++b) quant16<false>(f[b], inv, X.h[b], X.l[b]);
            sx = scale_of(M);
        }
        {
            const float sxin = sx * (256.f * kappa[9]);
            f32x16 f[4];
            float m = 0.f;
#pragma unroll
            for (int b = 0; b < 4; ++b) {
                i32x16 t;
                const uint4* ws = ring_enter(R, 77 + b);
                k_i8<8>(t, X, ws, R);
                dequant16(f[b], t, sxin, bias + nm::stage_b_off(9) + 32 * b);
                k_bf<2>(f[b], pw, g, s, ws + 8 * kStepU4);
                m = max16<true>(m, f[b]);
            }
            const float M = row_max(m), inv = inv_of(M);
#pragma unroll
            for (int b = 0; b < 4; ++b) quant16<true>(f[b], inv, X.h[b], X.l[b]);
            sx = scale_of(M);
        }
        {
            i32x16 t;
            f32x16 fr;
            k_i8<4>(t, X, ring_enter(R, 81), R);
            dequant16(fr, t, sx * (256.f * kappa[10]), bias + nm::stage_b_off(10));
            const int64_t i = row0 + s;
            if (g == 0 && i < a.n)
                reinterpret_cast<float4*>(a.out)[sample_record(a, i)] =
                    make_float4(fr[0] * u_r, fr[1] * u_g, fr[2] * u_b,
                                sigma * a.sigma_scale);
        }
    }
    asm volatile("s_waitcnt vmcnt(0)" ::: "memory");
}

}

namespace nm {

int launch_mlp_i8s(const MlpLaunch& L, const void* image8, const float* pts, const float* dirs, const float* origin, const float* direction,
                   const float* z, int64_t n, int S, int in_mode, float sigma_scale, float* out, hipStream_t stream, const MlpChunk* chunk) {
    Args8s A;
    MlpArgs& a = A.a;
    a.ray_idx = chunk ? chunk->ray_idx : nullptr;
    a.n_rays_dev = chunk ? chunk->n_rays_dev : nullptr;
    a.s0 = chunk ? chunk->s0 : 0;
    a.S_total = chunk ? chunk->S_total : S;
    a.wpack = nullptr; a.bias = nullptr;
    a.petab = L.petab;
    a.pts = pts; a.dirs = dirs; a.origin = origin; a.direction = direction; a.z = z;
    a.out = out; a.dbg = nullptr; a.prof = nullptr; a.n = n; a.S = S; a.in_mode = in_mode; a.stop_stage = -2; a.sigma_scale = sigma_scale;
    a.sigma_only = L.plain_head ? 2 : 0;
    a.save_h = nullptr; a.save_hv = nullptr; a.save_bits = nullptr; a.save_h16 = nullptr; a.save_feat16 = nullptr; a.save_hvbits = nullptr; a.save_x0h = nullptr; a.save_d0h = nullptr;
    a.pos = PeSpec{L.pe_kind, L.pos_nfreq, L.pos_octaves};
    a.dir = PeSpec{L.pe_kind, L.dir_nfreq, L.dir_octaves};
    A.consts8 = L.consts8;
    A.image8 = reinterpret_cast<const uint4*>(image8);
    const int64_t ntiles = (n + kTile - 1) / kTile;
    int dev = 0, cus = 256;
    if (hipGetDevice(&dev) == hipSuccess) {
        int v = 0;
        if (hipDeviceGetAttribute(&v, hipDeviceAttributeMultiprocessorCount, dev) == hipSuccess && v > 0) cus = v;
    }
    const int grid = (int)(ntiles < cus ? ntiles : cus);
    if (L.plain_head) hipLaunchKernelGGL(nerf_mlp_i8s_kernel<true>, dim3(grid), dim3(kWaves * 64), 0, stream, A);
    else hipLaunchKernelGGL(nerf_mlp_i8s_kernel<false>, dim3(grid), dim3(kWaves * 64), 0, stream, A);
    return check_launch("nerf_mlp_i8s_kernel");
}

}
```

ml-neuman_amd/csrc/mlp_launch.h:

```cpp
#pragma once
#include "common.h"

namespace nm {

enum { P_OUT_W = 16, P_OUT_B = 17 };
enum { P_PTS_W = 0, P_VIEWS_W = 16, P_VIEWS_B = 17, P_FEAT_W = 18, P_FEAT_B = 19, P_ALPHA_W = 20, P_ALPHA_B = 21, P_RGB_W = 22, P_RGB_B = 23 };
struct DevParams {
    const float* p[24];
};

struct MlpLaunch {
    const void* wpack; const float* bias; const float* petab;
    int pe_kind, pos_nfreq, dir_nfreq;
    int pos_octaves, dir_octaves;
    int plain_head;
    const void* wpack16; const float* bias16;
    const void* wstream8; const float* consts8;
    float* save_h = nullptr;
    float* save_hv = nullptr;
    unsigned* save_bits = nullptr;
    void* save_h16 = nullptr;
    void* save_feat16 = nullptr;
    unsigned* save_hvbits = nullptr;
    void* save_x0h = nullptr; void* save_d0h = nullptr;
};
struct RefLaunch {
    const float* wt; const float* bias; int off[12]; int boff[12]; const float* petab;
    int pe_kind, pos_nfreq, dir_nfreq;
    int plain_head;
};

struct MlpChunk {
    const int* ray_idx; const int* n_rays_dev; int s0, S_total;
};

int launch_mlp_mfma(const MlpLaunch& L, const float* pts, const float* dirs, const float* origin, const float* direction,
                    const float* z, int64_t n, int S, int in_mode, int precision, int stop_stage, float sigma_scale, float* out,
                    float* dbg, void* prof, hipStream_t stream, int sigma_only = 0, const MlpChunk* chunk = nullptr);
int launch_mlp_i8s(const MlpLaunch& L, const void* image8, const float* pts, const float* dirs, const float* origin, const float* direction,
                   const float* z, int64_t n, int S, int in_mode, float sigma_scale, float* out, hipStream_t stream, const MlpChunk* chunk);
int sigma_f16t_ndir();
int launch_sigma_f16t(const MlpLaunch& L, const void* stream16t, int stream_ndir, const float* pts, const float* dirs, const float* origin, const float* direction,
                      const float* z, int64_t n, int S, int in_mode, float sigma_scale, float* out, hipStream_t stream, const MlpChunk* chunk,
                      float* dbg, int dbg_stage);
int64_t mlp_bwd_image_bytes();
struct Bwd16 {
    void* dz16; void* dfeat16; const float* amax; float* dz32[8];
    const unsigned* hvbits = nullptr; void* dhv16 = nullptr; float* dhv32 = nullptr; int kdir = 0;
    int plain = 0;
};
int launch_mlp_bwd(const DevParams& P, int kpe, uint8_t* image, const float* dz_top, const float* d_feat, const float* d_raw, const float* acts,
                   const unsigned* relu_bits, int64_t n, float* dz_out, float* colsum, float* gb, hipStream_t stream, const Bwd16* h = nullptr);
int launch_mlp_ref(const RefLaunch& L, const float* pts, const float* dirs, const float* origin, const float* direction,
                   const float* z, int64_t n, int S, int in_mode, int stop_stage, float sigma_scale, float* out, float* dbg,
                   hipStream_t stream);

}
```

ml-neuman_amd/neuman_hip/_lib.py:

```python
import ctypes
import os

import torch

_HERE = os.path.dirname(os.path.abspath(__file__))
LIB_PATH = os.environ.get("NEUMAN_HIP_LIB") or os.path.join(_HERE, "..", "lib", "libneuman_hip.so")

c_f32p = ctypes.c_void_p
c_i32p = ctypes.c_void_p
c_stream = ctypes.c_void_p
i64 = ctypes.c_int64
i32 = ctypes.c_int

NM_PREC_FP32, NM_PREC_BF16X3, NM_PREC_BF16, NM_PREC_I8X3, NM_PREC_FP16X3 = 0, 1, 2, 3, 4
NM_PE_POSENC, NM_PE_ROTATE = 0, 1
PRECISIONS = {"fp32": NM_PREC_FP32, "bf16x3": NM_PREC_BF16X3, "bf16": NM_PREC_BF16, "i8x3": NM_PREC_I8X3, "fp16x3": NM_PREC_FP16X3}


class MlpDesc(ctypes.Structure):
    _fields_ = [("depth", ctypes.c_int32), ("width", ctypes.c_int32), ("skip", ctypes.c_int32),
                ("pe_kind", ctypes.c_int32), ("pos_n_freqs", ctypes.c_int32), ("dir_n_freqs", ctypes.c_int32),
                ("plain_head", ctypes.c_int32)]


SIGNATURES = {
    "nm_version": (i32, []),
    "nm_last_error": (ctypes.c_char_p, []),
    "nm_device_count": (i32, []),
    "nm_ray_to_samples": (i32, [c_f32p, c_f32p, c_f32p, c_f32p, i64, i32, c_f32p, i32, c_f32p, c_f32p, c_f32p, c_f32p, c_stream]),
    "nm_z_to_points": (i32, [c_f32p, c_f32p, c_f32p, i64, i32, c_f32p, c_f32p, c_stream]),
    "nm_composite": (i32, [c_f32p, c_f32p, c_f32p, i64, i32, i32, c_f32p, c_f32p, c_f32p, c_f32p, c_f32p, c_f32p, c_stream]),
    "nm_sample_pdf": (i32, [c_f32p, c_f32p, i64, i32, c_f32p, i32, c_f32p, c_stream]),
    "nm_importance_z": (i32, [c_f32p, c_f32p, i64, i32, c_f32p, i32, i32, c_f32p, c_stream]),
    "nm_near_far": (i32, [c_f32p, c_f32p, i64, c_f32p, i32, ctypes.c_double, c_f32p, c_f32p, c_stream]),
    "nm_compact_workspace_ints": (i64, [i64]),
    "nm_occ_probe_offset": (ctypes.c_float, [i32, i32, i32, i32]),
    "nm_occ_build_workspace_floats": (i64, [i32, i32]),
    "nm_occ_build": (i32, [ctypes.c_void_p, ctypes.c_void_p, i32, i32, i32, ctypes.c_float, i32, i32, c_f32p, i64, c_i32p, c_stream]),
    "nm_occ_compact_workspace_ints": (i64, [i64]),
    "nm_occ_compact_samples": (i32, [c_i32p, i32, ctypes.c_void_p, c_f32p, c_f32p, c_f32p, i64, i32, c_i32p, c_i32p, c_i32p, c_stream]),
    "nm_mlp_forward_samples": (i32, [ctypes.c_void_p, c_f32p, c_f32p, c_f32p, i64, i32, c_i32p, c_i32p, i64, i32, ctypes.c_float, c_f32p, c_stream]),
    "nm_mlp_sigma_samples": (i32, [ctypes.c_void_p, c_f32p, c_f32p, c_f32p, i64, i32, c_i32p, c_i32p, i64, i32, ctypes.c_float, c_f32p, c_stream]),
    "nm_occ_compact_points": (i32, [c_i32p, i32, ctypes.c_void_p, c_f32p, i64, c_i32p, c_i32p, c_i32p, c_stream]),
    "nm_mlp_forward_listed": (i32, [ctypes.c_void_p, c_f32p, c_f32p, i64, c_i32p, c_i32p, i64, i32, ctypes.c_float, c_f32p, c_stream]),
    "nm_render_rays_human_occ_workspace_floats": (i64, [i64, i32, i32]),
    "nm_render_rays_human_occ": (i32, [ctypes.c_void_p, ctypes.c_void_p, ctypes.c_void_p, c_i32p, i32, ctypes.c_void_p, c_f32p, c_f32p, c_f32p, c_f32p, i64, i32,
                                       c_f32p, i32, ctypes.c_float, i32, c_f32p, c_f32p, c_f32p, c_i32p, c_f32p, c_f32p, c_f32p, c_stream]),
    "nm_compact_hits": (i32, [c_f32p, c_f32p, i64, c_i32p, c_i32p, c_i32p, c_i32p, c_stream]),
    "nm_mlp_pack_bytes": (i64, [ctypes.POINTER(MlpDesc)]),
    "nm_mlp_pack_i8s_bytes": (i64, [ctypes.POINTER(MlpDesc)]),
    "nm_mlp_pack_i8s": (i32, [ctypes.POINTER(MlpDesc), ctypes.POINTER(ctypes.c_void_p), ctypes.c_void_p]),
    "nm_mlp_pack": (i32, [ctypes.POINTER(MlpDesc), ctypes.POINTER(ctypes.c_void_p), ctypes.c_void_p]),
    "nm_mlp_pack_f16": (i32, [ctypes.POINTER(MlpDesc), ctypes.POINTER(ctypes.c_void_p), ctypes.c_void_p]),
    "nm_mlp_pack_i8_bytes": (i64, [ctypes.POINTER(MlpDesc)]),
    "nm_mlp_pack_i8": (i32, [ctypes.POINTER(MlpDesc), ctypes.POINTER(ctypes.c_void_p), ctypes.c_void_p]),
    "nm_mlp_create": (i32, [ctypes.POINTER(MlpDesc), ctypes.POINTER(ctypes.c_void_p), ctypes.c_void_p, ctypes.c_void_p,
                            ctypes.POINTER(ctypes.c_void_p)]),
    "nm_mlp_destroy": (i32, [ctypes.c_void_p]),
    "nm_mlp_forward": (i32, [ctypes.c_void_p, c_f32p, c_f32p, i64, i32, ctypes.c_float, c_f32p, c_stream]),
    "nm_mlp_refresh_f16": (i32, [ctypes.c_void_p, ctypes.c_void_p, c_stream]),
    "nm_mlp_forward_save": (i32, [ctypes.c_void_p, c_f32p, c_f32p, i64, c_f32p, c_f32p, c_f32p, c_stream]),
    "nm_mlp_backward_chain_workspace_floats": (i64, [i64]),
    "nm_mlp_forward_save_bits": (i32, [ctypes.c_void_p, c_f32p, c_f32p, i64, c_f32p, c_f32p, ctypes.c_void_p, c_f32p, c_stream]),
    "nm_mlp_backward_chain": (i32, [ctypes.c_void_p, ctypes.c_void_p, c_f32p, c_f32p, c_f32p, c_f32p, ctypes.c_void_p, i64, c_f32p, c_f32p, c_f32p, i64, c_stream]),
    "nm_mlp_forward_save16": (i32, [ctypes.c_void_p, c_f32p, c_f32p, i64, ctypes.c_void_p, c_f32p, ctypes.c_void_p, c_f32p, ctypes.c_void_p, ctypes.c_void_p,
                                    ctypes.c_void_p, ctypes.c_void_p, c_f32p, c_stream]),
    "nm_mlp_backward_plain16": (i32, [ctypes.c_void_p, ctypes.c_void_p, c_f32p, ctypes.c_void_p, i64, c_f32p, ctypes.c_void_p, c_f32p, c_f32p, c_f32p, c_f32p, i64, c_stream]),
    "nm_mlp_backward_net16": (i32, [ctypes.c_void_p, ctypes.c_void_p, c_f32p, c_f32p, ctypes.c_void_p, ctypes.c_void_p, i64, c_f32p, ctypes.c_void_p, ctypes.c_void_p,
                                    ctypes.c_void_p, c_f32p, c_f32p, c_f32p, c_f32p, c_f32p, i64, c_stream]),
    "nm_mlp_backward_chain16": (i32, [ctypes.c_void_p, ctypes.c_void_p, c_f32p, c_f32p, ctypes.c_void_p, i64, c_f32p, ctypes.c_void_p, ctypes.c_void_p, c_f32p, c_f32p,
                                      c_f32p, c_f32p, i64, c_stream]),
    "nm_mlp_forward_rays": (i32, [ctypes.c_void_p, c_f32p, c_f32p, c_f32p, i64, i32, i32, ctypes.c_float, c_f32p, c_stream]),
    "nm_mlp_sigma_rays": (i32, [ctypes.c_void_p, c_f32p, c_f32p, c_f32p, i64, i32, i32, ctypes.c_float, c_f32p, c_stream]),
    "nm_mlp_forward_ray_chunk": (i32, [ctypes.c_void_p, c_f32p, c_f32p, c_f32p, i32, c_i32p, c_i32p, i64, i32, i32, i32, ctypes.c_float, c_f32p,
                                       c_stream]),
    "nm_mlp_sigma_ray_chunk": (i32, [ctypes.c_void_p, c_f32p, c_f32p, c_f32p, i32, c_i32p, c_i32p, i64, i32, i32, i32, ctypes.c_float, c_f32p,
                                     c_stream]),
    "nm_transmittance_chunk": (i32, [c_f32p, c_f32p, c_f32p, c_i32p, c_i32p, i64, i32, i32, i32, c_f32p, c_stream]),
    "nm_transmittance_chunk_dz": (i32, [c_f32p, c_f32p, c_f32p, c_i32p, c_i32p, i64, i32, i32, i32, c_f32p, c_stream]),
    "nm_mlp_sigma_f16t_debug": (i32, [ctypes.c_void_p, c_f32p, c_f32p, i64, i32, c_f32p, c_f32p, c_stream]),
    "nm_mlp_forward_debug": (i32, [ctypes.c_void_p, c_f32p, c_f32p, i64, i32, i32, c_f32p, c_stream]),
    "nm_mlp_forward_profile": (i32, [ctypes.c_void_p, c_f32p, c_f32p, i64, i32, c_f32p, ctypes.c_void_p, c_stream]),
    "nm_mesh_create": (i32, [c_f32p, i32, c_i32p, i32, i32, ctypes.POINTER(ctypes.c_void_p), c_stream]),
    "nm_mesh_update": (i32, [ctypes.c_void_p, c_f32p, c_stream]),
    "nm_mesh_destroy": (i32, [ctypes.c_void_p]),
    "nm_mesh_info": (i32, [ctypes.c_void_p, ctypes.c_void_p, ctypes.c_void_p, ctypes.c_void_p]),
    "nm_warp_to_canonical": (i32, [ctypes.c_void_p, c_f32p, i64, i32, ctypes.c_void_p, c_f32p, c_f32p, c_f32p, c_stream]),
    "nm_warp_apply_forward": (i32, [c_f32p, c_i32p, c_f32p, c_f32p, i64, c_f32p, c_stream]),
    "nm_warp_apply_backward": (i32, [c_f32p, c_i32p, c_f32p, c_f32p, c_f32p, i64, i64, c_f32p, c_f32p, c_stream]),
    "nm_bary_forward": (i32, [c_f32p, c_i32p, c_f32p, i64, c_f32p, c_stream]),
    "nm_bary_backward": (i32, [c_f32p, c_i32p, c_f32p, c_f32p, i64, i64, c_f32p, c_stream]),
    "nm_smpl_create": (i32, [c_f32p, c_f32p, c_f32p, c_i32p, c_f32p, c_f32p, i32, i32, i32, ctypes.POINTER(ctypes.c_void_p)]),
    "nm_smpl_destroy": (i32, [ctypes.c_void_p]),
    "nm_smpl_vertex_workspace_floats": (i64, [ctypes.c_void_p]),
    "nm_smpl_vertex_forward": (i32, [ctypes.c_void_p, c_f32p, c_f32p, ctypes.c_void_p, ctypes.c_double, c_f32p, c_f32p, c_f32p, c_f32p, c_stream]),
    "nm_smpl_vertex_backward": (i32, [ctypes.c_void_p, c_f32p, c_f32p, ctypes.c_void_p, ctypes.c_double, c_f32p, c_f32p, c_f32p, c_f32p, c_f32p,
                                      c_f32p, c_f32p, c_stream]),
    "nm_smpl_frames": (i32, [ctypes.c_void_p, c_f32p, c_f32p, ctypes.c_void_p, i32, ctypes.c_double, i32, ctypes.c_void_p, c_f32p, c_f32p,
                             c_stream]),
    "nm_gemm_workspace_floats": (i64, [i32, i32, i32]),
    "nm_gemm_f32": (i32, [i32, i32, i32, i32, i32, c_f32p, i32, c_f32p, i32, c_f32p, i32, c_f32p, c_f32p, i32, i32, c_f32p, i64, c_stream]),
    "nm_gemm_bf16x3": (i32, [i32, i32, i32, i32, i32, c_f32p, i32, c_f32p, i32, c_f32p, i32, c_f32p, c_f32p, i32, i32, c_f32p, i64, c_stream]),
    "nm_gemm_fp16x3": (i32, [i32, i32, i32, i32, i32, c_f32p, i32, c_f32p, i32, c_f32p, i32, c_f32p, c_f32p, i32, i32, c_f32p, i64, c_stream]),
    "nm_pe_encode": (i32, [c_f32p, i64, i32, i32, i32, c_f32p, c_f32p, i32, c_stream]),
    "nm_pe_encode16": (i32, [c_f32p, i64, i32, i32, i32, c_f32p, ctypes.c_void_p, i32, i32, c_stream]),
    "nm_absmax": (i32, [c_f32p, i64, c_f32p, c_stream]),
    "nm_wgrad16_workspace_floats": (i64, [i32, i64, i32, i32]),
    "nm_wgrad16": (i32, [i32, i32, i32, ctypes.POINTER(ctypes.c_void_p), ctypes.POINTER(ctypes.c_void_p), ctypes.POINTER(ctypes.c_void_p), ctypes.POINTER(ctypes.c_int), i64,
                         c_f32p, c_f32p, i64, c_stream]),
    "nm_wgrad_heads16_workspace_floats": (i64, [i64]),
    "nm_wgrad_heads16": (i32, [c_f32p, ctypes.c_void_p, c_f32p, i64, c_f32p, c_f32p, c_f32p, i64, c_stream]),
    "nm_wgrad_out16_workspace_floats": (i64, [i64]),
    "nm_wgrad_out16": (i32, [c_f32p, ctypes.c_void_p, i64, c_f32p, c_f32p, c_f32p, i64, c_stream]),
    "nm_wgrad_alpha16_workspace_floats": (i64, [i64]),
    "nm_wgrad_alpha16": (i32, [c_f32p, ctypes.c_void_p, i64, c_f32p, c_f32p, i64, c_stream]),
    "nm_colsum_workspace_floats": (i64, [i64, i32]),
    "nm_colsum": (i32, [c_f32p, i64, i32, i32, c_f32p, c_f32p, i64, c_stream]),
    "nm_pe_backward": (i32, [c_f32p, i64, i32, i32, i32, c_f32p, c_f32p, i32, c_f32p, c_stream]),
    "nm_composite_backward": (i32, [c_f32p, c_f32p, c_f32p, i64, i32, i32, c_f32p, c_f32p, c_f32p, c_f32p, c_f32p, c_stream]),
    "nm_signed_distance": (i32, [ctypes.c_void_p, c_f32p, i64, c_f32p, c_i32p, c_f32p, c_stream]),
    "nm_ssim_u8": (i32, [ctypes.c_void_p, ctypes.c_void_p, i32, i32, i32, ctypes.c_void_p, ctypes.c_void_p, c_stream]),
    "nm_merge_sorted": (i32, [c_f32p, c_f32p, i32, c_f32p, c_f32p, i32, i64, c_f32p, c_f32p, c_stream]),
    "nm_gather_rows": (i32, [c_f32p, c_i32p, c_i32p, i64, i32, c_f32p, c_stream]),
    "nm_scatter_rows": (i32, [c_f32p, c_i32p, c_i32p, i64, i32, c_f32p, c_stream]),
    "nm_shot_rays": (i32, [c_i32p, i64, i32, i32, ctypes.POINTER(ctypes.c_double), ctypes.POINTER(ctypes.c_double), c_f32p, c_f32p,
                           c_stream]),
    "nm_shot_rays_cams": (i32, [c_i32p, c_i32p, i64, i32, ctypes.c_void_p, i32, c_f32p, c_f32p, c_stream]),
    "nm_render_rays_bkg_workspace_floats": (i64, [i64, i32, i32]),
    "nm_render_rays_bkg": (i32, [ctypes.c_void_p, ctypes.c_void_p, c_f32p, c_f32p, c_f32p, c_f32p, i64, i32, i32, c_f32p, c_f32p, i32, i32, i32, c_f32p, c_f32p,
                                 c_f32p, c_f32p, c_f32p, c_f32p, c_stream]),
    "nm_render_rays_human_workspace_floats": (i64, [i64, i32, i32]),
    "nm_render_rays_human": (i32, [ctypes.c_void_p, ctypes.c_void_p, ctypes.c_void_p, c_f32p, c_f32p, c_f32p, c_f32p, i64, i32, c_f32p, i32, ctypes.c_float, i32,
                                   c_f32p, c_f32p, c_f32p, c_f32p, c_f32p, c_f32p, c_stream]),
    "nm_render_rays_hybrid_workspace_floats": (i64, [i64, i32, i32, i32]),
    "nm_render_rays_hybrid": (i32, [ctypes.c_void_p, ctypes.c_void_p, ctypes.c_void_p, ctypes.c_void_p, ctypes.c_void_p, c_f32p, i32, ctypes.c_double, c_f32p, c_f32p,
                                    i64, ctypes.c_float, ctypes.c_float, i32, i32, i32, c_f32p, c_f32p, c_f32p, i32, i32, i32, i32, c_f32p, c_f32p, c_f32p, c_f32p,
                                    c_stream]),
    "nm_merge_composite_lists": (i32, [i32, ctypes.POINTER(ctypes.c_void_p), ctypes.POINTER(ctypes.c_void_p), ctypes.POINTER(ctypes.c_void_p),
                                       ctypes.POINTER(ctypes.c_int), i64, c_f32p, i32, c_f32p, c_f32p, c_f32p, c_stream]),
    "nm_merged_intervals": (i32, [i32, ctypes.POINTER(ctypes.c_void_p), ctypes.POINTER(ctypes.c_int), i64, ctypes.POINTER(ctypes.c_void_p), c_stream]),
    "nm_importance_from_raw": (i32, [c_f32p, c_f32p, c_f32p, i64, i32, c_f32p, i32, c_f32p, c_f32p, c_stream]),
    "nm_merge_composite_workspace_floats": (i64, [i64, i32, i32]),
    "nm_merge_composite": (i32, [c_f32p, c_f32p, i32, c_f32p, c_f32p, i32, i64, c_f32p, i32, c_f32p, c_f32p, c_f32p, c_f32p, c_stream]),
    "nm_loss_workspace_doubles": (i64, []),
    "nm_loss_bimodal": (i32, [c_f32p, i64, i32, ctypes.c_float, c_f32p, c_f32p, ctypes.c_void_p, c_stream]),
    "nm_loss_pair_mse": (i32, [i32, c_f32p, c_f32p, i64, ctypes.c_float, c_f32p, c_f32p, c_f32p, ctypes.c_void_p, c_stream]),
    "nm_loss_shape": (i32, [c_f32p, c_f32p, i64, c_f32p, c_f32p, i64, ctypes.c_float, ctypes.c_float, ctypes.c_float, ctypes.c_float, c_f32p, c_f32p, c_f32p,
                            ctypes.c_void_p, c_f32p, c_stream]),
    "nm_frame_to_uint8": (i32, [c_f32p, i64, ctypes.c_void_p, c_stream]),
    "nm_ssd_u8": (i32, [ctypes.c_void_p, ctypes.c_void_p, i64, ctypes.c_void_p, c_stream]),
}

_lib = None


class NeumanHipError(RuntimeError):
    pass


def lib():
    global _lib
    if _lib is None:
        path = os.path.abspath(LIB_PATH)
        if not os.path.exists(path):
            raise NeumanHipError(f"{path} is missing: run `python ml-neuman_amd/build.py` (there is no CPU fallback)")
        handle = ctypes.CDLL(path)
        for name, (res, args) in SIGNATURES.items():
            fn = getattr(handle, name)
            fn.restype = res
            fn.argtypes = args
        _lib = handle
    return _lib


def check(rc, what):
    if rc != 0:
        raise NeumanHipError(f"{what} failed (code {rc}): {lib().nm_last_error().decode(errors='replace')}")


def stream_ptr():
    return ctypes.c_void_p(torch.cuda.current_stream().cuda_stream)


def dev_ptr(t, dtype=torch.float32, name="tensor"):
    if t is None:
        return None
    if not isinstance(t, torch.Tensor) or not t.is_cuda:
        raise NeumanHipError(f"{name} must be a CUDA (HIP) tensor: libneuman_hip has no CPU path")
    if t.dtype != dtype:
        raise NeumanHipError(f"{name} must be {dtype}, got {t.dtype}")
    if not t.is_contiguous():
        raise NeumanHipError(f"{name} must be contiguous")
    return ctypes.c_void_p(t.data_ptr())


def require_gpu():
    if not torch.cuda.is_available() or lib().nm_device_count() < 1:
        raise NeumanHipError("no HIP device visible: the NeuMan HIP path cannot run (there is no CPU fallback)")
```

ml-neuman_amd/neuman_hip/render_utils.py:

```python
import ctypes
import os

import numpy as np
import torch

from . import _lib, occupancy, parallel, ray_utils
from .ray_utils import DEFAULT_GEO_THRESH

MAX_RAYS_PER_LAUNCH = int(os.environ.get("NEUMAN_MAX_RAYS_PER_LAUNCH", 1 << 20))
TERMINATION_EPS = float(os.environ.get("NEUMAN_TERMINATION_EPS", "0"))
TERMINATION_CHUNK = int(os.environ.get("NEUMAN_TERMINATION_CHUNK", "32"))
TERMINATION_COARSE = float(os.environ.get("NEUMAN_TERMINATION_COARSE", "4e-13"))
TERMINATION_MIN_CHUNK = 16
FUSED_HYBRID_RAYS = int(os.environ.get("NEUMAN_FUSED_HYBRID_RAYS", 1 << 17))


def raw2outputs(raw, z_vals, rays_d, raw_noise_std=0, white_bkg=True, want_weights=True):
    _lib.require_gpu()
    R, S = z_vals.shape
    dev = raw.device
    noise = None
    if raw_noise_std > 0.:
        noise = (torch.randn((R, S), device=dev) * raw_noise_std).contiguous()
    if torch.is_grad_enabled() and raw.requires_grad:
# ... 87 lines not shown
        _transmittance_chunk(raw, z, dz, d, live, counts, R, s0 - c, c, S, T)
        T_eff = T if occluder is None else T * torch.where(z[:, s0] >= occluder[0], occluder[1], torch.ones_like(T))
        nxt = torch.empty(R, device=dev, dtype=torch.int32)
        counts = torch.zeros(2, device=dev, dtype=torch.int32)
        _lib.check(_lib.lib().nm_compact_hits(_lib.dev_ptr(thr), _lib.dev_ptr(T_eff.contiguous()), R, _lib.dev_ptr(nxt, torch.int32), None,
                                              _lib.dev_ptr(counts, torch.int32), _lib.dev_ptr(ws, torch.int32), _lib.stream_ptr()), "nm_compact_hits")
        live = nxt
        if adaptive:
            n_new = int(counts[0].item())
            if n_new == 0:
                break
            cut = 1.0 - n_new / max(1, n_live)
            chunk = max(TERMINATION_MIN_CHUNK, chunk // 2) if cut > 0.02 else min(max(chunk, TERMINATION_CHUNK), chunk * 2)
            n_live = n_new
    if stats is not None:
        n = int(evaluated.item())
        stats['evaluated'] = stats.get('evaluated', 0) + n
        stats['total'] = stats.get('total', 0) + R * S
        stats['launches'] = stats.get('launches', 0) + launches
    return raw


def transmittance_of(raw, z, d, dz=None):
    R, S = z.shape
    T = torch.ones(R, device=z.device, dtype=torch.float32)
    _transmittance_chunk(raw.contiguous(), z.contiguous(), None if dz is None else dz.contiguous(), d.contiguous(), None, None, R, 0, S, S, T)
    return T


def human_march_rays(human_net, o, d, near, far, samples_per_ray, mesh, eps, sigma_scale=1.0, precision=None, chunk=None, trace=None,
                     stats=None, dz=None):
    _lib.require_gpu()
    R, S = o.shape[0], int(samples_per_ray)
    dev = o.device
    chunk = chunk or TERMINATION_MIN_CHUNK
    pts, _, z = ray_utils.sample_z(o.contiguous(), d.contiguous(), near.reshape(-1).contiguous(), far.reshape(-1).contiguous(), S, want_points=True)
    raw = torch.zeros((R, S, 4), device=dev, dtype=torch.float32)
    T = torch.ones(R, device=dev, dtype=torch.float32)
    d = d.contiguous()
    live = torch.arange(R, device=dev)
    s0, evaluated, launches = 0, 0, 0
    grid = occupancy.grid_of(human_net)
    occ_stats = {} if grid is not None else None
    while s0 < S and live.numel() > 0:
        c = min(chunk, S - s0)
        a = s0 - 1 if (s0 + c == S and c == 1) else s0
        b = min(S, s0 + c + 1)
        can_pts, can_dirs, _ = ray_utils.warp_to_canonical_dev(pts[live, a:b].contiguous(), mesh)
        k = s0 - a
        if grid is None:
            out = human_net(can_pts[:, k:k + c].contiguous(), can_dirs[:, k:k + c].contiguous(), precision=precision, sigma_scale=sigma_scale,
                            role='shading')
            evaluated += live.numel() * c
        else:
            out = occupancy.forward_points(human_net, can_pts[:, k:k + c].contiguous(), can_dirs[:, k:k + c].contiguous(), precision=precision,
                                           sigma_scale=sigma_scale, role='shading', stats=occ_stats)
        raw[live, s0:s0 + c] = out
        launches += 1
        s0 += c
        if s0 >= S or eps <= 0:
            continue
        idx = live.to(torch.int32)
        cnt = torch.tensor([idx.numel(), 0], device=dev, dtype=torch.int32)
        _transmittance_chunk(raw, z, dz, d, idx, cnt, R, s0 - c, c, S, T)
        n_live = live.numel()
        live = live[T[live] >= eps]
        chunk = max(TERMINATION_MIN_CHUNK, chunk // 2) if live.numel() < 0.98 * n_live else chunk * 2
    if occ_stats is not None:
        evaluated = occ_stats.get('evaluated', 0)
        _note(trace, occupancy_human={'evaluated': evaluated, 'total': R * S})
    if stats is not None:
        stats['human_evaluated'] = stats.get('human_evaluated', 0) + evaluated
        stats['human_total'] = stats.get('human_total', 0) + R * S
        stats['human_launches'] = stats.get('human_launches', 0) + launches
    _note(trace, human_z=z)
    return raw, z


def _given_near_far(given, actor, i, j, o, d, verts, geo_threshold):
    if given is not None and 'near_far' in given:
        n, f = given['near_far'][actor]
        return n[i:j].to(torch.float32).contiguous(), f[i:j].to(torch.float32).contiguous()
    return ray_utils.geometry_guided_near_far(o, d, verts, geo_threshold)


def _ws(n_floats, device):
    return torch.empty(max(int(n_floats), 4), device=device, dtype=torch.float32)


def bkg_pass_rays_fused(coarse_net, fine_net, o, d, near, far, samples_per_ray, importance_samples_per_ray, white_bkg, precision=None):
    _lib.require_gpu()
    if _occupancy_on(coarse_net, fine_net):
        raw, z = bkg_pass_rays(coarse_net, fine_net, o.contiguous(), d.contiguous(), near.reshape(-1).contiguous(), far.reshape(-1).contiguous(),
                               samples_per_ray, importance_samples_per_ray, white_bkg, precision)
        return raw, z
    R, S = o.shape[0], int(samples_per_ray)
    N = int(importance_samples_per_ray) if fine_net is not None else 0
    dev = o.device
    for n_ in (coarse_net, fine_net):
        if n_ is not None:
            n_._guard(o, d, near)
    raw = torch.empty((R, S + N, 4), device=dev, dtype=torch.float32)
    z = torch.empty((R, S + N), device=dev, dtype=torch.float32)
    ws = _ws(_lib.lib().nm_render_rays_bkg_workspace_floats(R, S, N), dev)
    t_vals = torch.linspace(0., 1., steps=S, device=dev)
    u = torch.linspace(0., 1., steps=N, device=dev) if N else None
    _lib.check(_lib.lib().nm_render_rays_bkg(
        coarse_net.handle(), fine_net.handle() if fine_net is not None else None, _lib.dev_ptr(o.contiguous()), _lib.dev_ptr(d.contiguous()),
        _lib.dev_ptr(near.reshape(-1).contiguous()), _lib.dev_ptr(far.reshape(-1).contiguous()), R, S, N, _lib.dev_ptr(t_vals), _lib.dev_ptr(u),
        int(bool(white_bkg)), coarse_net._prec(precision, None if fine_net is not None else 'shading'),
        fine_net._prec(precision, 'shading') if fine_net is not None else 0, _lib.dev_ptr(ws), _lib.dev_ptr(raw), _lib.dev_ptr(z), None, None, None,
        _lib.stream_ptr()), "nm_render_rays_bkg")
    return raw, z


def _occupancy_on(*nets):
    on = any(occupancy.grid_of(n_) is not None for n_ in nets)
    if on and TERMINATION_EPS > 0:
        raise NotImplementedError("an occupancy grid together with early ray termination (TERMINATION_EPS > 0) is not served: "
                                  "detach the grid or set TERMINATION_EPS = 0")
    return on


def _occupancy_pass(net, o, d, z, precision, role, sigma_only, trace, key):
    stats = {} if trace is not None else None
    raw = occupancy.forward_rays(net, o, d, z, precision=precision, role=role, sigma_only=sigma_only, stats=stats)
    _note(trace, **{key: stats})
    return raw


def bkg_place_z(coarse_net, fine_net, o, d, near, far, samples_per_ray, importance_samples_per_ray, white_bkg, precision=None, trace=None):
    occ = _occupancy_on(coarse_net)
    _, _, z = ray_utils.sample_z(o, d, near, far, samples_per_ray)
    if occ:
        if fine_net is None:
            return z, _occupancy_pass(coarse_net, o, d, z, precision, 'shading', False, trace, 'occupancy_coarse')
        raw = _occupancy_pass(coarse_net, o, d, z, precision, None, True, trace, 'occupancy_coarse')
        z_fine, w = ray_utils.importance_z_from_raw(raw, z, d, importance_samples_per_ray, want_weights=trace is not None)
        _note(trace, coarse_z=z, coarse_w=w)
        return z_fine, None
    if fine_net is None:
        return z, (None if TERMINATION_EPS > 0 else coarse_net.forward_rays(o, d, z, precision=precision, role='shading'))
    if TERMINATION_EPS > 0:
        stats = {} if trace is not None else None
        raw = march_pass_rays(coarse_net, o, d, z, TERMINATION_COARSE, precision=precision, role=None, stats=stats, sigma_only=True)
        _note(trace, march_coarse=stats)
    else:
        raw = coarse_net.forward_rays(o, d, z, precision=precision, role=None, sigma_only=True)
    z_fine, w = ray_utils.importance_z_from_raw(raw, z, d, importance_samples_per_ray, want_weights=trace is not None)
    _note(trace, coarse_z=z, coarse_w=w)
    return z_fine, None


def bkg_shade(net, o, d, z, precision=None, trace=None, occluder=None, dz=None):
    if _occupancy_on(net):
        return _occupancy_pass(net, o, d, z, precision, 'shading', False, trace, 'occupancy')
    if TERMINATION_EPS > 0:
        stats = {} if trace is not None else None
        raw = march_pass_rays(net, o, d, z, TERMINATION_EPS, precision=precision, stats=stats, occluder=occluder, dz=dz)
        _note(trace, march=stats)
        return raw
    return net.forward_rays(o, d, z, precision=precision, role='shading')


def bkg_pass_rays(coarse_net, fine_net, o, d, near, far, samples_per_ray, importance_samples_per_ray, white_bkg,
                  precision=None, trace=None, given_z=None, occluder=None, dz=None):
    net = fine_net if fine_net is not None else coarse_net
    if given_z is not None:
        z = given_z.to(torch.float32).contiguous()
        _note(trace, bkg_z=z)
        return net.forward_rays(o, d, z, precision=precision, role='shading'), z
    z, raw = bkg_place_z(coarse_net, fine_net, o, d, near, far, samples_per_ray, importance_samples_per_ray, white_bkg, precision, trace)
    if raw is None:
        raw = bkg_shade(net, o, d, z, precision, trace, occluder, dz)
    _note(trace, bkg_z=z)
    return raw, z


def render_vanilla_rays(coarse_net, fine_net, o, d, near, far, samples_per_ray, importance_samples_per_ray, white_bkg=True,
                        precision=None, trace=None, given=None):
    R = o.shape[0]
    rgb = torch.empty((R, 3), device=o.device, dtype=torch.float32)
    depth = torch.empty(R, device=o.device, dtype=torch.float32)
    for i, j in _chunks(R):
        oc, dc = o[i:j], d[i:j]
        n = torch.full((j - i,), float(near), device=o.device, dtype=torch.float32)
        f = torch.full((j - i,), float(far), device=o.device, dtype=torch.float32)
        raw, z = bkg_pass_rays(coarse_net, fine_net, oc, dc, n, f, samples_per_ray, importance_samples_per_ray, white_bkg,
                               precision, trace, given['bkg_z'][i:j] if given is not None and 'bkg_z' in given else None)
        rgb[i:j], _, _, _, depth[i:j] = raw2outputs(raw, z, dc, white_bkg=white_bkg, want_weights=False)
    return rgb, depth


def human_pass_rays(human_net, o, d, near, far, samples_per_ray, mesh=None, render_can=False, sigma_scale=1.0, precision=None,
                    trace=None):
    _lib.require_gpu()
    R, S = o.shape[0], int(samples_per_ray)
    dev = o.device
    human_net._guard(o, d, near)
    posed = not render_can
    grid = occupancy.grid_of(human_net)
    raw = torch.empty((R, S, 4), device=dev, dtype=torch.float32)
    z = torch.empty((R, S), device=dev, dtype=torch.float32)
    t_vals = torch.linspace(0., 1., steps=S, device=dev)
    if grid is None:
        ws = _ws(_lib.lib().nm_render_rays_human_workspace_floats(R, S, int(posed)), dev)
        _lib.check(_lib.lib().nm_render_rays_human(
            human_net.handle(), mesh.handle if posed else None, _lib.dev_ptr(mesh.T, torch.float64, 'T') if posed else None, _lib.dev_ptr(o.contiguous()),
            _lib.dev_ptr(d.contiguous()), _lib.dev_ptr(near.reshape(-1).contiguous()), _lib.dev_ptr(far.reshape(-1).contiguous()), R, S, _lib.dev_ptr(t_vals), 1,
            float(sigma_scale), human_net._prec(precision, 'shading'), _lib.dev_ptr(ws), _lib.dev_ptr(raw), _lib.dev_ptr(z), None, None, None, _lib.stream_ptr()),
            "nm_render_rays_human")
    else:
        grid.check_device(dev)
        counts = torch.zeros(2, device=dev, dtype=torch.int32)
        ws = _ws(_lib.lib().nm_render_rays_human_occ_workspace_floats(R, S, int(posed)), dev)
        _lib.check(_lib.lib().nm_render_rays_human_occ(
            human_net.handle(), mesh.handle if posed else None, _lib.dev_ptr(mesh.T, torch.float64, 'T') if posed else None,
            _lib.dev_ptr(grid.bits, torch.int32), grid.res, grid.box_c(), _lib.dev_ptr(o.contiguous()), _lib.dev_ptr(d.contiguous()),
            _lib.dev_ptr(near.reshape(-1).contiguous()), _lib.dev_ptr(far.reshape(-1).contiguous()), R, S, _lib.dev_ptr(t_vals), 1, float(sigma_scale),
            human_net._prec(precision, 'shading'), _lib.dev_ptr(ws), _lib.dev_ptr(raw), _lib.dev_ptr(z), _lib.dev_ptr(counts, torch.int32), None, None, None,
            _lib.stream_ptr()), "nm_render_rays_human_occ")
        if trace is not None:
            _note(trace, occupancy_human={'evaluated': int(counts[0].item()), 'total': R * S})
    if trace is not None:
        if posed:
            n3 = (R * S * 3 + 3) & ~3
            _note(trace, human_z=z, can_pts=ws[n3:n3 + R * S * 3].reshape(R, S, 3).clone(), can_dirs=ws[2 * n3:2 * n3 + R * S * 3].reshape(R, S, 3).clone())
        else:
            _note(trace, human_z=z)
    return raw, z


def merge_composite(za, rawa, zb, rawb, rays_d, white_bkg=True):
    _lib.require_gpu()
    R, Sa = za.shape
    Sb = zb.shape[1]
    dev = za.device
    rgb = torch.empty((R, 3), device=dev, dtype=torch.float32)
    depth = torch.empty(R, device=dev, dtype=torch.float32)
    acc = torch.empty(R, device=dev, dtype=torch.float32)
    ws = _ws(_lib.lib().nm_merge_composite_workspace_floats(R, Sa, Sb), dev)
    _lib.check(_lib.lib().nm_merge_composite(_lib.dev_ptr(za.contiguous()), _lib.dev_ptr(rawa.contiguous()), Sa, _lib.dev_ptr(zb.contiguous()),
                                             _lib.dev_ptr(rawb.contiguous()), Sb, R, _lib.dev_ptr(rays_d.contiguous()), int(bool(white_bkg)), _lib.dev_ptr(ws),
                                             _lib.dev_ptr(rgb), _lib.dev_ptr(depth), _lib.dev_ptr(acc), _lib.stream_ptr()), "nm_merge_composite")
    return rgb, depth, acc


def merge_composite_lists(z_lists, raw_lists, rays_d, white_bkg=True, rows=None):
    _lib.require_gpu()
    k = len(z_lists)
    R = rays_d.shape[0]
    dev = rays_d.device
    zs = [z.to(torch.float32).contiguous() for z in z_lists]
    raws = [r_.to(torch.float32).contiguous() for r_ in raw_lists]
    rows = [None] * k if rows is None else [None if x is None else x.to(torch.int32).contiguous() for x in rows]
    for l_ in range(k):
        if rows[l_] is None and zs[l_].shape[0] != R:
            raise _lib.NeumanHipError(f"merge_composite_lists: list {l_} has {zs[l_].shape[0]} rows for {R} rays")
    arr = ctypes.c_void_p * k
    rgb = torch.empty((R, 3), device=dev, dtype=torch.float32)
    depth = torch.empty(R, device=dev, dtype=torch.float32)
    acc = torch.empty(R, device=dev, dtype=torch.float32)
    _lib.check(_lib.lib().nm_merge_composite_lists(
        k, arr(*[z.data_ptr() for z in zs]), arr(*[r_.data_ptr() for r_ in raws]), arr(*[None if x is None else x.data_ptr() for x in rows]),
        (ctypes.c_int * k)(*[int(z.shape[1]) for z in zs]), R, _lib.dev_ptr(rays_d.contiguous()), int(bool(white_bkg)), _lib.dev_ptr(rgb), _lib.dev_ptr(depth),
        _lib.dev_ptr(acc), _lib.stream_ptr()), "nm_merge_composite_lists")
    return rgb, depth, acc


def render_smpl_nerf_rays(human_net, o, d, posed_verts, mesh, samples_per_ray, white_bkg=True, render_can=False,
                          geo_threshold=DEFAULT_GEO_THRESH, interval_comp=1.0, precision=None, trace=None, given=None):
    R = o.shape[0]
    rgb = torch.full((R, 3), 1.0 if white_bkg else 0.0, device=o.device, dtype=torch.float32)
    depth = torch.zeros(R, device=o.device, dtype=torch.float32)
    acc = torch.zeros(R, device=o.device, dtype=torch.float32)
    for i, j in _chunks(R):
        oc, dc = o[i:j].contiguous(), d[i:j].contiguous()
        near, far = _given_near_far(given, 0, i, j, oc, dc, posed_verts, geo_threshold)
        _note(trace, near=near, far=far)
        hit, _ = ray_utils.compact_hits(near, far)
        if hit.numel() == 0:
            continue
        ho, hd = ray_utils.gather_rows(oc, hit), ray_utils.gather_rows(dc, hit)
        hn, hf = ray_utils.gather_rows(near, hit), ray_utils.gather_rows(far, hit)
        _note(trace, hit=hit + i)
        if TERMINATION_EPS > 0 and not render_can:
            mstats = {} if trace is not None else None
            raw, z = human_march_rays(human_net, ho, hd, hn, hf, samples_per_ray, mesh, TERMINATION_EPS, interval_comp, precision, None, trace, mstats)
            _note(trace, march_human=mstats)
        else:
            raw, z = human_pass_rays(human_net, ho, hd, hn, hf, samples_per_ray, mesh, render_can, interval_comp, precision, trace)
        _rgb, _, _acc, _, _depth = raw2outputs(raw, z, hd, white_bkg=white_bkg, want_weights=False)
        ray_utils.scatter_rows(rgb[i:j], hit, _rgb)
        ray_utils.scatter_rows(depth[i:j], hit, _depth)
        ray_utils.scatter_rows(acc[i:j], hit, _acc)
    return rgb, depth, acc


def render_hybrid_rays(coarse_bkg, fine_bkg, human_net, o, d, bkg_near, bkg_far, posed_verts, mesh, samples_per_ray,
                       importance_samples_per_ray, white_bkg=True, geo_threshold=DEFAULT_GEO_THRESH, precision=None, trace=None,
                       given=None):
    if TERMINATION_EPS <= 0 and trace is None and given is None and not _occupancy_on(coarse_bkg, fine_bkg) and occupancy.grid_of(human_net) is None:
        return render_hybrid_rays_fused(coarse_bkg, fine_bkg, human_net, o, d, bkg_near, bkg_far, posed_verts, mesh, samples_per_ray,
                                        importance_samples_per_ray, white_bkg, geo_threshold, precision)
    R = o.shape[0]
    rgb = torch.empty((R, 3), device=o.device, dtype=torch.float32)
    depth = torch.empty(R, device=o.device, dtype=torch.float32)
    acc = torch.zeros(R, device=o.device, dtype=torch.float32)
    for i, j in _chunks(R):
        oc, dc = o[i:j].contiguous(), d[i:j].contiguous()
        n = torch.full((j - i,), float(bkg_near), device=o.device, dtype=torch.float32)
        f = torch.full((j - i,), float(bkg_far), device=o.device, dtype=torch.float32)
        given_z = given['bkg_z'][i:j] if given is not None and 'bkg_z' in given else None

        def human_lists(merge_z=None):
            near, far = _given_near_far(given, 0, i, j, oc, dc, posed_verts, geo_threshold)
            _note(trace, near=near, far=far)
            hit, _ = ray_utils.compact_hits(near, far)
            if hit.numel() == 0:
                return hit, None, None, None, None
            ho, hd = ray_utils.gather_rows(oc, hit), ray_utils.gather_rows(dc, hit)
            hn, hf = ray_utils.gather_rows(near, hit), ray_utils.gather_rows(far, hit)
            _note(trace, hit=hit + i)
            if TERMINATION_EPS > 0:
                mstats = {} if trace is not None else None
                dz_h = None
                if merge_z is not None:
                    _, _, h_z0 = ray_utils.sample_z(ho, hd, hn, hf, samples_per_ray)
                    dz_h = merged_intervals([ray_utils.gather_rows(merge_z, hit), h_z0])[1]
                h_raw, h_z = human_march_rays(human_net, ho, hd, hn, hf, samples_per_ray, mesh, TERMINATION_EPS, 1.0, precision, None, trace, mstats,
                                              dz=dz_h)
                _note(trace, march_human=mstats)
            else:
                h_raw, h_z = human_pass_rays(human_net, ho, hd, hn, hf, samples_per_ray, mesh, False, 1.0, precision, trace)
            return hit, hd, hf, h_raw, h_z

        if TERMINATION_EPS > 0 and given_z is None:
            bkg_z, _ = bkg_place_z(coarse_bkg, fine_bkg, oc, dc, n, f, samples_per_ray, importance_samples_per_ray, white_bkg, precision, trace)
            _note(trace, bkg_z=bkg_z)
            dz_b = torch.cat([bkg_z[:, 1:] - bkg_z[:, :-1], torch.full_like(bkg_z[:, :1], 1e10)], 1)
            hit, hd, hf, h_raw, h_z = human_lists(bkg_z)
            occluder = None
# ... 334 lines not shown
```

ml-neuman_amd/neuman_hip/vanilla.py:

```python
import ctypes
import os

import numpy as np
import torch
import torch.nn as nn

from . import _lib

DEFAULT_PRECISION = os.environ.get("NEUMAN_PRECISION", "mixed")


def weight_reset(m):
    if isinstance(m, nn.Linear):
        m.reset_parameters()


class Embedder(nn.Module):

    def __init__(self, input_dims, max_freq, N_freqs, log_sampling=True, include_input=True, min_freq=0, mapping='posenc'):
        super().__init__()
        if mapping not in ('posenc', 'rotate'):
            raise ValueError(mapping)
        assert log_sampling or mapping == 'rotate', "log_sampling=False is not a configuration of the reference (models/vanilla.py:70)"
        self.input_dims, self.max_freq, self.min_freq, self.N_freqs = input_dims, max_freq, min_freq, N_freqs
        self.log_sampling, self.include_input, self.mapping = log_sampling, bool(include_input), mapping
        raw = input_dims if mapping == 'posenc' else 3
        self.out_dim = (raw if self.include_input else 0) + (2 * input_dims * N_freqs if mapping == 'posenc' else 6 * N_freqs)

    def table(self):
        if self.mapping == 'posenc':
            return (2. ** torch.linspace(self.min_freq, self.max_freq, steps=self.N_freqs)).numpy().astype(np.float32)
        bands = 2. ** np.linspace(self.min_freq, self.max_freq, num=self.N_freqs)
        b = (np.eye(3)[None] * bands[:, None, None]).reshape(3 * self.N_freqs, 3)
        c = 2 ** .5 / 2
        b = b @ np.array([[c, -c, 0], [c, c, 0], [0, 0, 1]]).T
        b = b @ np.array([[1, 0, 0], [0, c, -c], [0, c, c]]).T
        return np.ascontiguousarray(b.astype(np.float32))

    @property
    def bvals(self):
        return torch.from_numpy(self.table()) if self.mapping == 'rotate' else None

    def forward(self, inputs, cur_iter=None):
        raise _lib.NeumanHipError("Embedder.forward is fused into the HIP MLP kernel: call the Joiner")


class NeRF(nn.Module):

    def __init__(self, depth=8, width=256, input_ch=3, input_ch_views=3, output_ch=4, skips=[4], use_viewdirs=False,
                 scale=1.0, scale_type='no'):
        super().__init__()
        self.depth, self.width, self.input_ch, self.input_ch_views = depth, width, input_ch, input_ch_views
        self.skips, self.use_viewdirs, self.scale, self.scale_type = skips, use_viewdirs, scale, scale_type
        layers = [nn.Linear(input_ch, width)]
        for i in range(depth - 1):
            layers.append(nn.Linear(width + input_ch if i in skips else width, width))
        self.pts_linears = nn.ModuleList(layers)
        if use_viewdirs:
            self.views_linears = nn.ModuleList([nn.Linear(input_ch_views + width, width // 2)])
            self.feature_linear = nn.Linear(width, width)
            self.alpha_linear = nn.Linear(width, 1)
            self.rgb_linear = nn.Linear(width // 2, 3)
        else:
            self.output_linear = nn.Linear(width, output_ch)

    def ordered_params(self):
        heads = [self.views_linears[0], self.feature_linear, self.alpha_linear, self.rgb_linear] if self.use_viewdirs else [self.output_linear]
        if not self.use_viewdirs and self.output_linear.out_features != 4:
            raise NotImplementedError("the rendering kernels take the 4-output (r, g, b, sigma) plain head; other widths (the offset "
                                      "net's 3) run on the differentiable float32 path (neuman_hip/train.py)")
        out = []
        for lin in list(self.pts_linears) + heads:
            out += [lin.weight, lin.bias]
        return out

    def forward(self, input_pts, input_views=None):
        raise _lib.NeumanHipError("NeRF.forward on pre-encoded inputs is not exposed: the HIP kernel fuses PE + MLP (use Joiner)")


def absent_input_columns(pos_pe, dir_pe, nerf):
    pads = {}
    if not pos_pe.include_input:
        raw = pos_pe.input_dims if pos_pe.mapping == 'posenc' else 3
        pads[0] = (0, raw)
        for s in nerf.skips:
            if s + 1 < nerf.depth:
                pads[2 * (s + 1)] = (0, raw)
    if nerf.use_viewdirs and not dir_pe.include_input:
        pads[2 * nerf.depth] = (nerf.width, dir_pe.input_dims if dir_pe.mapping == 'posenc' else 3)
    return pads


def with_absent_columns(tensors, pads):
    out = list(tensors)
    for i, (at, cnt) in pads.items():
        w = out[i]
        out[i] = torch.cat([w[:, :at], torch.zeros((w.shape[0], cnt), device=w.device, dtype=w.dtype), w[:, at:]], 1)
    return out


class Joiner(nn.Module):

    def __init__(self, pos_pe, dir_pe, nerf):
        super().__init__()
        self.pos_pe, self.dir_pe, self.nerf = pos_pe, dir_pe, nerf
        self.precision = DEFAULT_PRECISION
        self._handle = None
        self._handle_key = None
        self._train_handle = None

    def _key(self):
        return tuple((p.data_ptr(), p._version) for p in self.nerf.ordered_params())

    def _release(self, train_too=True):
        if self._handle is not None:
            _lib.lib().nm_mlp_destroy(self._handle)
            self._handle = None
        if train_too and getattr(self, '_train_handle', None) is not None:
            _lib.lib().nm_mlp_destroy(self._train_handle)
            self._train_handle = None

    def __del__(self):
        try:
            self._release()
        except Exception:
            pass

    def __getstate__(self):
        state = self.__dict__.copy()
        state['_handle'] = None
        state['_handle_key'] = None
        state['_train_handle'] = None
        return state

    def __deepcopy__(self, memo):
        import copy
        new = self.__class__.__new__(self.__class__)
        memo[id(self)] = new
        for k, v in self.__dict__.items():
            new.__dict__[k] = None if k in ('_handle', '_handle_key', '_train_handle') else copy.deepcopy(v, memo)
        return new

    def handle(self):
        key = self._key()
        if self._handle is None or key != self._handle_key:
            self._release(train_too=False)
            n = self.nerf
            if n.scale_type != 'no':
                raise NotImplementedError("scale_type != 'no' (offset nets) is outside the HIP path")
            if self.pos_pe.mapping != self.dir_pe.mapping:
                raise NotImplementedError("mixed PE kinds")
            desc = _lib.MlpDesc(n.depth, n.width, n.skips[0] if len(n.skips) == 1 else -1,
                                _lib.NM_PE_ROTATE if self.pos_pe.mapping == 'rotate' else _lib.NM_PE_POSENC,
                                self.pos_pe.N_freqs, self.dir_pe.N_freqs, 0 if n.use_viewdirs else 1)
            host = [p.to('cpu', torch.float32).contiguous()
                    for p in with_absent_columns([q.detach() for q in n.ordered_params()], absent_input_columns(self.pos_pe, self.dir_pe, n))]
            arr = (ctypes.c_void_p * 24)(*([t.data_ptr() for t in host] + [None] * (24 - len(host))))
            pos_tab, dir_tab = self.pos_pe.table(), self.dir_pe.table()
            out = ctypes.c_void_p()
            _lib.check(_lib.lib().nm_mlp_create(ctypes.byref(desc), arr, pos_tab.ctypes.data, dir_tab.ctypes.data,
                                                ctypes.byref(out)), "nm_mlp_create")
            self._handle, self._handle_key = out, key
        return self._handle

    def train_handle(self):
        if self._train_handle is None:
            keep, keep_key = self._handle, self._handle_key
            self._handle = None
            try:
                self._train_handle = self.handle()
            finally:
                self._handle, self._handle_key = keep, keep_key
        return self._train_handle

    def _prec(self, precision, role=None):
        p = precision or self.precision
        if p == 'mixed':
            p = 'i8x3' if role == 'shading' else 'fp16x3'
        return _lib.PRECISIONS[p]

    @staticmethod
    def _guard(*tensors):
        _lib.require_gpu()
        if torch.is_grad_enabled() and any(t.requires_grad for t in tensors):
            raise _lib.NeumanHipError("the rendering kernels are forward-only: wrap in torch.no_grad(), or put the Joiner in train() mode "
                                       "for the differentiable float32 forward (neuman_hip/train.py)")

    def forward(self, input_pts, input_views=None, precision=None, sigma_scale=1.0, role=None):
        if input_views is None:
            if self.nerf.use_viewdirs:
                raise _lib.NeumanHipError("input_views is required by the use_viewdirs=True net (vanilla.py:133-134)")
            input_views = torch.zeros_like(input_pts)
        if self.pos_pe.input_dims != 3:
            from . import train
            if sigma_scale != 1.0:
                raise _lib.NeumanHipError("sigma_scale is a canonical-render option (render_utils.py:229)")
            if input_pts.shape[-1] != self.pos_pe.input_dims:
                raise _lib.NeumanHipError(f"input_pts has {input_pts.shape[-1]} components, the position encoding takes {self.pos_pe.input_dims}")
            return train.mlp_forward_train(self, input_pts, input_views)
        if self.training and torch.is_grad_enabled() and any(p.requires_grad for p in self.parameters()):
            from . import train
            if sigma_scale != 1.0:
                raise _lib.NeumanHipError("sigma_scale is a render-time option (render_utils.py:229)")
            return train.mlp_forward_train(self, input_pts, input_views)
        self._guard(input_pts, input_views)
        shp = input_pts.shape[:-1]
        p = input_pts.detach().reshape(-1, 3).contiguous()
        d = input_views.detach().reshape(-1, 3).contiguous()
        out = torch.empty((p.shape[0], 4), device=p.device, dtype=torch.float32)
        _lib.check(_lib.lib().nm_mlp_forward(self.handle(), _lib.dev_ptr(p, name='input_pts'), _lib.dev_ptr(d, name='input_views'),
                                             p.shape[0], self._prec(precision, role), float(sigma_scale), _lib.dev_ptr(out),
                                             _lib.stream_ptr()), "nm_mlp_forward")
        return out.reshape(*shp, 4)

    def forward_two_views(self, input_pts, input_views, other_views):
        from . import train
        n = input_pts.reshape(-1, input_pts.shape[-1]).shape[0]
        if not (self.training and torch.is_grad_enabled() and self.nerf.use_viewdirs and self.pos_pe.input_dims == 3 and train.two_views_ok(self, n)):
            return None
        return train.two_views(self, input_pts, input_views, other_views)

    def forward_rays(self, origin, direction, z_vals, precision=None, sigma_scale=1.0, role=None, sigma_only=False):
        self._guard(origin, direction, z_vals)
        R, S = z_vals.shape
        out = torch.empty((R, S, 4), device=z_vals.device, dtype=torch.float32)
        entry = _lib.lib().nm_mlp_sigma_rays if sigma_only else _lib.lib().nm_mlp_forward_rays
        _lib.check(entry(self.handle(), _lib.dev_ptr(origin, name='origin'), _lib.dev_ptr(direction, name='direction'),
                         _lib.dev_ptr(z_vals, name='z_vals'), R, S, self._prec(precision, role), float(sigma_scale),
                         _lib.dev_ptr(out), _lib.stream_ptr()), "nm_mlp_sigma_rays" if sigma_only else "nm_mlp_forward_rays")
        return out

    def forward_ray_chunk(self, origin, direction, z_vals, ray_idx, n_rays_dev, s0, chunk, out, precision=None, sigma_scale=1.0, role=None,
                          sigma_only=False):
        self._guard(origin, direction, z_vals)
        R, S = z_vals.shape
        entry = _lib.lib().nm_mlp_sigma_ray_chunk if sigma_only else _lib.lib().nm_mlp_forward_ray_chunk
        _lib.check(entry(
            self.handle(), _lib.dev_ptr(origin, name='origin'), _lib.dev_ptr(direction, name='direction'), _lib.dev_ptr(z_vals, name='z_vals'), S,
            _lib.dev_ptr(ray_idx, torch.int32, 'ray_idx'), _lib.dev_ptr(n_rays_dev, torch.int32, 'n_rays_dev'), ray_idx.shape[0], int(s0), int(chunk),
            self._prec(precision, role), float(sigma_scale), _lib.dev_ptr(out), _lib.stream_ptr()), "nm_mlp_forward_ray_chunk")
        return out

    def forward_debug(self, input_pts, input_views, stage, precision=None):
        self._guard(input_pts, input_views)
        p = input_pts.detach().reshape(-1, 3).contiguous()
        d = input_views.detach().reshape(-1, 3).contiguous()
        width = 64 if stage == -1 else (128 if stage == 9 else 256)
        out = torch.zeros((p.shape[0], width), device=p.device, dtype=torch.float32)
        _lib.check(_lib.lib().nm_mlp_forward_debug(self.handle(), _lib.dev_ptr(p), _lib.dev_ptr(d), p.shape[0],
                                                   self._prec(precision), int(stage), _lib.dev_ptr(out), _lib.stream_ptr()),
                   "nm_mlp_forward_debug")
        return out


def time_columns(pe):
    if pe.mapping != 'posenc' or pe.input_dims != 4:
        raise _lib.NeumanHipError("time_columns: a 4-D posenc encoding is expected (raw_pos_dim = 4)")
    N = pe.N_freqs
    raw = 4 if pe.include_input else 0
    spatial = [0, 1, 2][:raw] + [raw + 8 * b + k for b in range(N) for k in (0, 1, 2, 4, 5, 6)]
    timecol = [3][:raw] + [raw + 8 * b + k for b in range(N) for k in (3, 7)]
    return spatial, timecol


def time_encoding(pe, t):
    bands = pe.table().astype(np.float32)
    tt = np.float32(t)
    out = [float(tt)] if pe.include_input else []
    for b in range(pe.N_freqs):
        a = np.float64(np.float32(tt * bands[b]))
        out += [float(np.sin(a)), float(np.cos(a))]
    return np.asarray(out, np.float64)


def frozen_time_joiner(joiner, t):
    pe = joiner.pos_pe
    key = (joiner._key(), float(t))
    cache = joiner.__dict__.setdefault('_frozen_time', {})
    if key in cache:
        return cache[key]
    spatial, timecol = time_columns(pe)
    n = joiner.nerf
    with torch.no_grad():
        pe3 = Embedder(3, pe.max_freq, pe.N_freqs, pe.log_sampling, pe.include_input, min_freq=pe.min_freq, mapping='posenc')
        nerf = NeRF(depth=n.depth, width=n.width, input_ch=pe3.out_dim, input_ch_views=n.input_ch_views, use_viewdirs=n.use_viewdirs, skips=list(n.skips),
                    output_ch=(n.output_linear.out_features if not n.use_viewdirs else 4))
        dev = n.pts_linears[0].weight.device
        pt = torch.as_tensor(time_encoding(pe, t), dtype=torch.float64, device=dev)
        sp, tc = torch.as_tensor(spatial, device=dev), torch.as_tensor(timecol, device=dev)
        for i, lin in enumerate(n.pts_linears):
            takes_pe = i == 0 or (i - 1) in n.skips
            if not takes_pe:
                nerf.pts_linears[i] = lin
                continue
            w = lin.weight.detach()
            new = nn.Linear(pe3.out_dim + (0 if i == 0 else n.width), n.width)
            new.weight.copy_(torch.cat([w[:, sp], w[:, pe.out_dim:]], 1) if i else w[:, sp])
            new.bias.copy_((lin.bias.detach().double() + w[:, tc].double() @ pt).to(torch.float32))
            nerf.pts_linears[i] = new.to(dev)
        for name in (('views_linears', 'feature_linear', 'alpha_linear', 'rgb_linear') if n.use_viewdirs else ('output_linear',)):
            setattr(nerf, name, getattr(n, name))
        out = Joiner(pe3, joiner.dir_pe, nerf).to(dev).eval()
        out.precision = joiner.precision
    while len(cache) >= 4:
        cache.pop(next(iter(cache)))
    cache[key] = out
    return out


class OffsetNet(nn.Module):

    def __init__(self, pos_pe, nerf):
        super().__init__()
        self.pos_pe, self.nerf = pos_pe, nerf

    def forward(self, input_pts, cur_iter=None, const_time=None):
        assert cur_iter is None
        from . import train
        out = train.offset_forward_train(self, input_pts, const_time=const_time)
        if self.nerf.scale_type == 'no':
            return out
        if self.nerf.scale_type == 'linear':
            return out * self.nerf.scale
        if self.nerf.scale_type == 'tanh':
            return torch.tanh(out) * self.nerf.scale
        raise ValueError(self.nerf.scale_type)


def build_offset_net(opt):
    st_pe = Embedder(opt.raw_pos_dim + 1, opt.pos_max_freq, opt.pos_N_freqs, opt.log_sampling, opt.include_input, min_freq=opt.pos_min_freq)
    nerf = NeRF(depth=opt.nerf_depth, width=opt.nerf_width, input_ch=st_pe.out_dim, input_ch_views=0, output_ch=3, use_viewdirs=False,
                scale=opt.offset_scale, scale_type=opt.offset_scale_type)
    net = OffsetNet(st_pe, nerf)
    return net.cuda() if opt.use_cuda else net


def build_nerf(opt):
    mapping = opt.posenc if hasattr(opt, 'posenc') else 'posenc'
    pos_pe = Embedder(opt.raw_pos_dim, opt.pos_max_freq, opt.pos_N_freqs, opt.log_sampling, opt.include_input,
                      min_freq=opt.pos_min_freq, mapping=mapping)
    dir_pe = Embedder(opt.raw_dir_dim, opt.dir_max_freq, opt.dir_N_freqs, opt.log_sampling, opt.include_input, mapping=mapping)
    nets = []
    for _ in range(2):
        nerf = NeRF(depth=opt.nerf_depth, width=opt.nerf_width, input_ch=pos_pe.out_dim, input_ch_views=dir_pe.out_dim,
                    use_viewdirs=opt.use_viewdirs)
        nets.append(nerf)
    coarse, fine = Joiner(pos_pe, dir_pe, nets[0]), Joiner(pos_pe, dir_pe, nets[1])
    if opt.use_cuda:
        coarse, fine = coarse.cuda(), fine.cuda()
    return coarse, fine
```

Measured before the change: 1.447 million.

## Split i8 shading pass into trunk kernel plus colour head over live samples

```diff
diff --git a/include/neuman_hip.h b/include/neuman_hip.h
--- a/include/neuman_hip.h
+++ b/include/neuman_hip.h
@@ -70,6 +70,9 @@
 int nm_mlp_pack_i8(const nm_mlp_desc* desc, const float* const* host_params, void* host_out);
 int64_t nm_mlp_pack_i8s_bytes(const nm_mlp_desc* desc);
 int nm_mlp_pack_i8s(const nm_mlp_desc* desc, const float* const* host_params, void* host_out);
+int64_t nm_mlp_pack_i8s_trunk_bytes(const nm_mlp_desc* desc);
+int64_t nm_mlp_pack_i8s_head_bytes(const nm_mlp_desc* desc);
+int nm_mlp_pack_i8s_live(const nm_mlp_desc* desc, const float* const* host_params, void* host_trunk_out, void* host_head_out);
 int nm_mlp_create(const nm_mlp_desc* desc, const float* const* host_params, const float* host_pos_tab,
                   const float* host_dir_tab, nm_mlp_t* out);
 int nm_mlp_destroy(nm_mlp_t mlp);
@@ -99,6 +102,10 @@
                           float* dhv32, float* bias_grads, float* workspace, int64_t workspace_floats, nm_stream_t stream);
 int nm_mlp_forward_rays(nm_mlp_t mlp, const float* origin, const float* direction, const float* z_vals,
                         int64_t R, int S, int precision, float sigma_scale, float* out, nm_stream_t stream);
+#define NM_LIVE_CHUNK_SAMPLES (1 << 21)
+int64_t nm_mlp_forward_rays_live_workspace_bytes(int64_t R, int S, int64_t chunk_samples);
+int nm_mlp_forward_rays_live(nm_mlp_t mlp, const float* origin, const float* direction, const float* z_vals, int64_t R, int S, int precision,
+                             float sigma_scale, float* out, void* workspace, int64_t workspace_bytes, int64_t chunk_samples, nm_stream_t stream);
 int nm_mlp_sigma_rays(nm_mlp_t mlp, const float* origin, const float* direction, const float* z_vals,
                       int64_t R, int S, int precision, float sigma_scale, float* out, nm_stream_t stream);
 int nm_mlp_forward_ray_chunk(nm_mlp_t mlp, const float* origin, const float* direction, const float* z_vals, int S_total,
diff --git a/ml-neuman_amd/csrc/mlp_host.hip b/ml-neuman_amd/csrc/mlp_host.hip
--- a/ml-neuman_amd/csrc/mlp_host.hip
+++ b/ml-neuman_amd/csrc/mlp_host.hip
@@ -465,6 +465,17 @@
     put(10, 0, 0, 4);
     if (dst - out != kWeightBytes8) abort();
 }
+constexpr int64_t kTrunkSteps8 = 8 * 4 + 7 * 8 * 8 + 8 * 4 + 8, kHeadSteps8 = 8 * 8 + 4 * 10 + 4;
+static_assert((kTrunkSteps8 + kHeadSteps8) * kStepBytes == kWeightBytes8 && (kTrunkSteps8 + 16) * kStepBytes == kPlainStreamBytes8, "stream cuts");
+constexpr int64_t kTrunkStreamBytes8 = kPlainStreamBytes8 + kWeightPadBytes, kHeadStreamBytes8 = kHeadSteps8 * kStepBytes + kWeightPadBytes;
+static void pack_stream8s_live(const uint8_t* img8, uint8_t* trunk, uint8_t* head) {
+    std::vector<uint8_t> whole((size_t)(kWeightBytes8 + kWeightPadBytes)), cut(whole.size());
+    pack_stream8s(img8, whole.data());
+    pack_stream8s(img8, cut.data(), true);
+    memcpy(trunk, cut.data(), (size_t)kTrunkStreamBytes8);
+    memset(head, 0, (size_t)kHeadStreamBytes8);
+    memcpy(head, whole.data() + kTrunkSteps8 * kStepBytes, (size_t)(kHeadSteps8 * kStepBytes));
+}
 
 constexpr int kSigmaSteps = 8 * 4 + 6 * 8 * 16 + 8 * 20 + 16;
 static void sigma_stream_table(std::vector<int>& tab, int ndir) {
@@ -524,6 +535,7 @@
     float* d_consts8;
     uint8_t* d_stream8;
     uint8_t* d_image8;
+    uint8_t* d_trunk8;
     uint8_t* d_stream16t;
     int* d_sigma_tab;
     uint8_t* d_bwd_image;
@@ -595,6 +607,28 @@
     std::vector<uint8_t> img8((size_t)nm::image8_bytes());
     nm::pack_image8(desc, host_params, img8.data());
     nm::pack_stream8s(img8.data(), static_cast<uint8_t*>(host_out), desc->plain_head != 0);
+    return NM_OK;
+}
+
+int64_t nm_mlp_pack_i8s_trunk_bytes(const nm_mlp_desc* desc) {
+    if (nm::validate_desc(desc) != NM_OK || desc->plain_head) return -1;
+    return nm::kTrunkStreamBytes8;
+}
+
+int64_t nm_mlp_pack_i8s_head_bytes(const nm_mlp_desc* desc) {
+    if (nm::validate_desc(desc) != NM_OK || desc->plain_head) return -1;
+    return nm::kHeadStreamBytes8;
+}
+
+int nm_mlp_pack_i8s_live(const nm_mlp_desc* desc, const float* const* host_params, void* host_trunk_out, void* host_head_out) {
+    if (int e = nm::validate_desc(desc)) return e;
+    NM_REQUIRE(!desc->plain_head, "nm_mlp_pack_i8s_live: the plain-head net has no colour head to split off");
+    NM_REQUIRE(host_params && host_trunk_out && host_head_out, "nm_mlp_pack_i8s_live: null pointer");
+    for (int i = 0; i < 24; ++i) NM_REQUIRE(host_params[i], "nm_mlp_pack_i8s_live: host_params[%d] is null", i);
+    if (int e = nm::check_finite("nm_mlp_pack_i8s_live", desc, host_params)) return e;
+    std::vector<uint8_t> img8((size_t)nm::image8_bytes());
+    nm::pack_image8(desc, host_params, img8.data());
+    nm::pack_stream8s_live(img8.data(), static_cast<uint8_t*>(host_trunk_out), static_cast<uint8_t*>(host_head_out));
     return NM_OK;
 }
 
@@ -616,6 +650,8 @@
     nm::pack_image8(desc, host_params, img8.data());
     nm::pack_stream8(img8.data(), str8.data());
     nm::pack_stream8s(img8.data(), str8s.data(), plain != 0);
+    std::vector<uint8_t> live8(plain ? 0 : (size_t)(nm::kTrunkStreamBytes8 + nm::kHeadStreamBytes8));
+    if (!plain) nm::pack_stream8s_live(img8.data(), live8.data(), live8.data() + nm::kTrunkStreamBytes8);
 
     const int kpe = 3 + 6 * desc->pos_n_freqs, kdpe = 3 + 6 * desc->dir_n_freqs;
     const int K[12] = {kpe, 256, 256, 256, 256, kpe + 256, 256, 256, plain ? 0 : 256 + kdpe, plain ? 0 : 256, 256, plain ? 0 : 128};
@@ -651,7 +687,7 @@
     m->pos_octaves = octaves(tab, desc->pos_n_freqs);
     m->dir_octaves = octaves(tab + 96, desc->dir_n_freqs);
 
-    m->d_image = nullptr; m->d_image16 = nullptr; m->d_consts8 = nullptr; m->d_stream8 = nullptr; m->d_image8 = nullptr; m->d_stream16t = nullptr; m->d_sigma_tab = nullptr; m->d_bwd_image = nullptr; m->d_petab = nullptr; m->d_ref = nullptr; m->d_wscale16 = nullptr;
+    m->d_image = nullptr; m->d_image16 = nullptr; m->d_consts8 = nullptr; m->d_stream8 = nullptr; m->d_image8 = nullptr; m->d_trunk8 = nullptr; m->d_stream16t = nullptr; m->d_sigma_tab = nullptr; m->d_bwd_image = nullptr; m->d_petab = nullptr; m->d_ref = nullptr; m->d_wscale16 = nullptr;
     int rc = nm::check_hip(hipMalloc(&m->d_image, (size_t)bytes), "nm_mlp_create: hipMalloc(image)");
     const size_t consts_off = (size_t)(nm::kWeightBytes8 + nm::kWeightPadBytes), consts_bytes = img8.size() - consts_off;
     if (!rc) rc = nm::check_hip(hipMalloc(&m->d_consts8, consts_bytes), "nm_mlp_create: hipMalloc(consts8)");
@@ -660,6 +696,8 @@
     if (!rc) rc = nm::check_hip(hipMemcpy(m->d_stream8, str8.data(), str8.size(), hipMemcpyHostToDevice), "nm_mlp_create: upload stream8");
     if (!rc) rc = nm::check_hip(hipMalloc(&m->d_image8, consts_off), "nm_mlp_create: hipMalloc(image8)");
     if (!rc) rc = nm::check_hip(hipMemcpy(m->d_image8, str8s.data(), consts_off, hipMemcpyHostToDevice), "nm_mlp_create: upload image8");
+    if (!rc && !plain) rc = nm::check_hip(hipMalloc(&m->d_trunk8, live8.size()), "nm_mlp_create: hipMalloc(trunk8)");
+    if (!rc && !plain) rc = nm::check_hip(hipMemcpy(m->d_trunk8, live8.data(), live8.size(), hipMemcpyHostToDevice), "nm_mlp_create: upload trunk8");
     if (!rc) rc = nm::check_hip(hipMalloc(&m->d_petab, sizeof(tab)), "nm_mlp_create: hipMalloc(petab)");
     if (!rc) rc = nm::check_hip(hipMalloc(&m->d_ref, ref.size() * 4), "nm_mlp_create: hipMalloc(ref)");
     if (!rc) rc = nm::check_hip(hipMemcpy(m->d_image, img.data(), (size_t)bytes, hipMemcpyHostToDevice), "nm_mlp_create: upload image");
@@ -720,6 +758,7 @@
     if (m->d_consts8) (void)hipFree(m->d_consts8);
     if (m->d_stream8) (void)hipFree(m->d_stream8);
     if (m->d_image8) (void)hipFree(m->d_image8);
+    if (m->d_trunk8) (void)hipFree(m->d_trunk8);
     if (m->d_stream16t) (void)hipFree(m->d_stream16t);
     if (m->d_sigma_tab) (void)hipFree(m->d_sigma_tab);
     if (m->d_bwd_image) (void)hipFree(m->d_bwd_image);
@@ -728,6 +767,11 @@
     if (m->d_wscale16) (void)hipFree(m->d_wscale16);
     delete m;
     return NM_OK;
+}
+
+static bool i8_as_kernel() {
+    static const bool on = [] { const char* e = getenv("NEUMAN_I8_KERNEL"); return !e || !strcmp(e, "as"); }();
+    return on;
 }
 
 static int mlp_dispatch(nm_mlp_t m, const float* pts, const float* dirs, const float* origin, const float* direction,
@@ -764,7 +808,7 @@
     L.plain_head = m->desc.plain_head;
     L.wstream8 = m->d_stream8;
     L.consts8 = m->d_consts8;
-    static const bool i8_as = [] { const char* e = getenv("NEUMAN_I8_KERNEL"); return !e || !strcmp(e, "as"); }();
+    const bool i8_as = i8_as_kernel();
     const char* sk = getenv("NEUMAN_SIGMA_KERNEL");
     const bool sigma_t = !(sk && !strcmp(sk, "w")) && m->d_stream16t;
     if (sigma_t && precision == NM_PREC_FP16X3 && sigma_only == 1 && stop_stage == -2 && !dbg && !prof && !m->desc.plain_head)
@@ -947,6 +991,60 @@
                         nullptr, stream);
 }
 
+static int64_t live_chunk_rays(int64_t R, int S, int64_t chunk_samples) {
+    if (chunk_samples <= 0) chunk_samples = NM_LIVE_CHUNK_SAMPLES;
+    const int64_t rays = chunk_samples / S;
+    return rays < 1 ? 1 : rays > R ? R : rays;
+}
+static int64_t live_cap(int64_t R, int S, int64_t chunk_samples) {
+    return (live_chunk_rays(R, S, chunk_samples) * S + 255) / 256 * 256;
+}
+
+int64_t nm_mlp_forward_rays_live_workspace_bytes(int64_t R, int S, int64_t chunk_samples) {
+    if (R < 0 || S < 1) return -1;
+    return live_cap(R, S, chunk_samples) * (512 + 4 + 4) + 256;
+}
+
+int nm_mlp_forward_rays_live(nm_mlp_t m, const float* origin, const float* direction, const float* z_vals, int64_t R, int S, int precision,
+                             float sigma_scale, float* out, void* workspace, int64_t workspace_bytes, int64_t chunk_samples, nm_stream_t stream) {
+    NM_REQUIRE(m, "nm_mlp_forward_rays_live: null handle");
+    if (m->desc.plain_head || precision != NM_PREC_I8X3 || !i8_as_kernel())
+        return nm_mlp_forward_rays(m, origin, direction, z_vals, R, S, precision, sigma_scale, out, stream);
+    NM_REQUIRE(R == 0 || (origin && direction && z_vals && out && workspace), "nm_mlp_forward_rays_live: null pointer");
+    NM_REQUIRE(R >= 0 && S >= 1, "nm_mlp_forward_rays_live: bad sizes");
+    NM_REQUIRE(((reinterpret_cast<uintptr_t>(out) | reinterpret_cast<uintptr_t>(workspace)) & 15) == 0, "nm_mlp_forward_rays_live: out and workspace must be 16-byte aligned");
+    NM_REQUIRE(workspace_bytes >= nm_mlp_forward_rays_live_workspace_bytes(R, S, chunk_samples), "nm_mlp_forward_rays_live: workspace of %lld bytes, %lld needed",
+               (long long)workspace_bytes, (long long)nm_mlp_forward_rays_live_workspace_bytes(R, S, chunk_samples));
+    if (R == 0) return NM_OK;
+    const int64_t cap = live_cap(R, S, chunk_samples), rays = live_chunk_rays(R, S, chunk_samples);
+    NM_REQUIRE(rays * S < (1ll << 31), "nm_mlp_forward_rays_live: a chunk of %lld samples", (long long)(rays * S));
+    nm::MlpLaunch L;
+    L.wpack = nullptr; L.bias = nullptr; L.wpack16 = nullptr; L.bias16 = nullptr; L.wstream8 = nullptr;
+    L.petab = m->d_petab;
+    L.pe_kind = m->desc.pe_kind; L.pos_nfreq = m->desc.pos_n_freqs; L.dir_nfreq = m->desc.dir_n_freqs;
+    L.pos_octaves = m->pos_octaves; L.dir_octaves = m->dir_octaves;
+    L.plain_head = 0;
+    L.consts8 = m->d_consts8;
+    uint8_t* ws = static_cast<uint8_t*>(workspace);
+    nm::LiveList live;
+    live.x = reinterpret_cast<uint4*>(ws);
+    live.sx = reinterpret_cast<float*>(ws + cap * 512);
+    live.idx = reinterpret_cast<int*>(ws + cap * 516);
+    live.count = reinterpret_cast<int*>(ws + cap * 520);
+    live.cap = cap;
+    hipStream_t st = nm::as_stream(stream);
+    for (int64_t r0 = 0; r0 < R; r0 += rays) {
+        const int64_t nr = R - r0 < rays ? R - r0 : rays;
+        if (int rc = nm::check_hip(hipMemsetAsync(live.count, 0, 4, st), "nm_mlp_forward_rays_live: counter reset")) return rc;
+        float* o = out + r0 * S * 4;
+        if (int rc = nm::launch_mlp_i8s(L, m->d_trunk8, nullptr, nullptr, origin + r0 * 3, direction + r0 * 3, z_vals + r0 * S, nr * S, S, 1, sigma_scale, o, st,
+                                        nullptr, &live))
+            return rc;
+        if (int rc = nm::launch_mlp_i8h(L, m->d_trunk8 + nm::kTrunkStreamBytes8, direction + r0 * 3, S, live, nr * S, o, st)) return rc;
+    }
+    return NM_OK;
+}
+
 int nm_mlp_sigma_rays(nm_mlp_t mlp, const float* origin, const float* direction, const float* z_vals, int64_t R, int S,
                       int precision, float sigma_scale, float* out, nm_stream_t stream) {
     NM_REQUIRE(R == 0 || (origin && direction && z_vals && out), "nm_mlp_sigma_rays: null pointer");
diff --git a/ml-neuman_amd/csrc/mlp_i8as.h b/ml-neuman_amd/csrc/mlp_i8as.h
--- a/ml-neuman_amd/csrc/mlp_i8as.h
+++ b/ml-neuman_amd/csrc/mlp_i8as.h
@@ -15,6 +15,7 @@
     MlpArgs a;
     const float* consts8;
     const uint4* image8;
+    nm::LiveList live;
 };
 
 __device__ __forceinline__ i32x4 as_i32x4(uint4 v) { return __builtin_bit_cast(i32x4, v); }
@@ -139,5 +140,106 @@
 __device__ __forceinline__ float inv_of(float M) { return M > 0.f ? ((float)nm::kFixedMax / 32767.f) * __builtin_amdgcn_rcpf(M) : 0.f; }
 __device__ __forceinline__ float scale_of(float M) { return M > 0.f ? M * (1.f / (float)nm::kFixedMax) : 1.f; }
 
-
-}
+constexpr int kWaves = 8;
+constexpr int kTile = kWaves * kRows;
+constexpr int kPWaveU4 = nm::kPeChunks * 2 * kRows;
+constexpr int kPeU4 = kWaves * kPWaveU4;
+constexpr int kStepU4 = nm::kStepBytes / 16;
+constexpr int kSlotU4 = 12 * kStepU4;
+constexpr int kSlots = 3;
+constexpr int kBiasU4 = (nm::kBiasFloats + 16 + 3) / 4;
+__host__ __device__ constexpr int block_pieces(int nsteps) { return (2 * nsteps + kWaves - 1) / kWaves; }
+
+template <class S>
+struct RingT {
+    const char* src;
+    const uint4* rd;
+    unsigned lds0;
+    int off;
+    int slot;
+    int refill, np, nsteps2;
+};
+template <class S>
+__device__ __forceinline__ void ring_piece(const RingT<S>& R, int off, int slot, int j) {
+    glds16(R.src + off + j * (kWaves * 1024), __builtin_amdgcn_readfirstlane(R.lds0 + slot * (kSlotU4 * 16) + j * (kWaves * 1024)));
+}
+template <class S>
+__device__ __forceinline__ void ring_advance(RingT<S>& R, int nsteps) {
+    R.off += nsteps * nm::kStepBytes;
+    if (R.off == S::kBytes) R.off = 0;
+}
+template <class S>
+__device__ __forceinline__ const uint4* ring_enter(RingT<S>& R, int i) {
+    const int np1 = block_pieces(S::steps(i + 1));
+    if (np1 == 1) asm volatile("s_waitcnt vmcnt(1)" ::: "memory");
+    else if (np1 == 2) asm volatile("s_waitcnt vmcnt(2)" ::: "memory");
+    else asm volatile("s_waitcnt vmcnt(3)" ::: "memory");
+    __builtin_amdgcn_s_barrier();
+    const uint4* cur = R.rd + R.slot * kSlotU4;
+    R.refill = R.slot == 0 ? kSlots - 1 : R.slot - 1;
+    R.slot = R.slot == kSlots - 1 ? 0 : R.slot + 1;
+    R.np = block_pieces(S::steps(i + 2));
+    R.nsteps2 = S::steps(i + 2);
+    return cur;
+}
+template <class S>
+__device__ __forceinline__ void ring_copy(RingT<S>& R, int j) {
+    if (j < R.np) ring_piece(R, R.off, R.refill, j);
+    if (j == R.np - 1) ring_advance(R, R.nsteps2);
+}
+struct W8 {
+    uint4 h, l;
+};
+
+template <int NSTEPS, bool PEND, bool RELU = true, class Ring>
+__device__ __forceinline__ void k_i8_impl(i32x16& t, const X8& X, const uint4* ws, Ring& R, f32x16& fp, const i32x16& tp, lds_cfloat* bias_blk,
+                                          float sx256, float& m) {
+    i32x16 ah, ac;
+#pragma unroll
+    for (int r = 0; r < 16; ++r) { ah[r] = 0; ac[r] = 0; }
+    W8 w[2];
+    w[0].h = ws[0]; w[0].l = ws[64];
+    w[1].h = ws[kStepU4]; w[1].l = ws[kStepU4 + 64];
+#pragma unroll
+    for (int s = 0; s < NSTEPS; ++s) {
+        const uint4 wh = w[s & 1].h, wl = w[s & 1].l;
+        ac = __builtin_amdgcn_mfma_i32_32x32x32_i8(as_i32x4(wh), as_i32x4(X.l[s]), ac, 0, 0, 0);
+        ah = __builtin_amdgcn_mfma_i32_32x32x32_i8(as_i32x4(wh), as_i32x4(X.h[s]), ah, 0, 0, 0);
+        ac = __builtin_amdgcn_mfma_i32_32x32x32_i8(as_i32x4(wl), as_i32x4(X.h[s]), ac, 0, 0, 0);
+        if (s + 2 < NSTEPS) { w[s & 1].h = ws[(s + 2) * kStepU4]; w[s & 1].l = ws[(s + 2) * kStepU4 + 64]; }
+        if (s == 0 || s == 2 || s == 4) ring_copy(R, s >> 1);
+        if (PEND) {
+            const int r = 2 * s;
+            const float b0 = bias_blk[8 * (r >> 2) + (r & 3)], b1 = bias_blk[8 * (r >> 2) + (r & 3) + 1];
+            const float f0 = fmaf((float)tp[r], sx256, b0), f1 = fmaf((float)tp[r + 1], sx256, b1);
+            fp[r] = f0;
+            fp[r + 1] = f1;
+            m = RELU ? fmaxf(m, fmaxf(f0, f1)) : fmaxf(m, fmaxf(fabsf(f0), fabsf(f1)));
+            __builtin_amdgcn_sched_barrier(0);
+        }
+    }
+#pragma unroll
+    for (int r = 0; r < 16; ++r) t[r] = (ah[r] << 8) + ac[r];
+}
+template <int NSTEPS, class Ring>
+__device__ __forceinline__ void k_i8(i32x16& t, const X8& X, const uint4* ws, Ring& R) {
+    f32x16 nf;
+    float nm_ = 0.f;
+    k_i8_impl<NSTEPS, false>(t, X, ws, R, nf, t, nullptr, 0.f, nm_);
+}
+struct NoRing {};
+__device__ __forceinline__ void ring_copy(NoRing&, int) {}
+template <int NSTEPS, bool COPY = false, class Ring = NoRing>
+__device__ __forceinline__ void k_bf(f32x16& f, const uint4* pw, int g, int s, const uint4* ws, Ring* R = nullptr, int j0 = 0) {
+#pragma unroll
+    for (int t = 0; t < NSTEPS; ++t) {
+        if (COPY && (t == 1 || t == 3)) ring_copy(*R, j0 + (t >> 1));
+        const uint4 wh = ws[t * kStepU4], wl = ws[t * kStepU4 + 64];
+        const uint4 xh = pw[(2 * t + g) * (2 * kRows) + s], xl = pw[(2 * t + g) * (2 * kRows) + kRows + s];
+        f = __builtin_amdgcn_mfma_f32_32x32x16_bf16(as_bf16x8(wh), as_bf16x8(xl), f, 0, 0, 0);
+        f = __builtin_amdgcn_mfma_f32_32x32x16_bf16(as_bf16x8(wl), as_bf16x8(xh), f, 0, 0, 0);
+        f = __builtin_amdgcn_mfma_f32_32x32x16_bf16(as_bf16x8(wh), as_bf16x8(xh), f, 0, 0, 0);
+    }
+}
+
+}
diff --git a/ml-neuman_amd/csrc/mlp_i8h.hip b/ml-neuman_amd/csrc/mlp_i8h.hip
--- /dev/null
+++ b/ml-neuman_amd/csrc/mlp_i8h.hip
@@ -0,0 +1,148 @@
+#include "mlp_i8as.h"
+
+namespace {
+
+constexpr int kHeadBlocks = 13;
+constexpr int kHeadSteps = 8 * 8 + 4 * 10 + 4;
+struct HeadStream {
+    static __host__ __device__ constexpr int steps(int i) {
+        i = i >= kHeadBlocks ? i - kHeadBlocks : i;
+        return i < 8 ? 8 : i < 12 ? 10 : 4;
+    }
+    static constexpr int kBytes = kHeadSteps * nm::kStepBytes;
+};
+typedef RingT<HeadStream> Ring;
+
+__global__ __launch_bounds__(kWaves * 64, 2) void nerf_head_i8s_kernel(const Args8s A) {
+    __shared__ uint4 lds[kPeU4 + kSlots * kSlotU4 + kBiasU4];
+    const MlpArgs a = resolve_args(A.a);
+    const int tid = threadIdx.x, lane = tid & 63;
+    const int w = __builtin_amdgcn_readfirstlane(tid >> 6);
+    const int g = lane >> 5, s = lane & 31;
+    uint4* pw = lds + w * kPWaveU4;
+    Ring R;
+    R.src = reinterpret_cast<const char*>(A.image8) + lane * 16 + w * 1024;
+    R.rd = lds + kPeU4 + lane;
+    R.lds0 = (unsigned)(uintptr_t)(lds + kPeU4) + w * 1024;
+    R.off = 0;
+    R.slot = 0;
+    {
+        float* lb = reinterpret_cast<float*>(lds + kPeU4 + kSlots * kSlotU4);
+        for (int i = tid; i < nm::kBiasFloats + 16; i += kWaves * 64) lb[i] = A.consts8[nm::kBiasFloats + i];
+    }
+    __syncthreads();
+    ring_piece(R, 0, 0, 0);
+    ring_piece(R, 0, 0, 1);
+    ring_piece(R, HeadStream::steps(0) * nm::kStepBytes, 1, 0);
+    ring_piece(R, HeadStream::steps(0) * nm::kStepBytes, 1, 1);
+    R.off = (HeadStream::steps(0) + HeadStream::steps(1)) * nm::kStepBytes;
+    const float u_r = A.consts8[nm::stage_b_off(10)], u_g = A.consts8[nm::stage_b_off(10) + 1], u_b = A.consts8[nm::stage_b_off(10) + 2];
+    const float* kappa = reinterpret_cast<const float*>(lds + kPeU4 + kSlots * kSlotU4) + nm::kBiasFloats;
+    unsigned bias_lds = (unsigned)(uintptr_t)(lds + kPeU4 + kSlots * kSlotU4) + 16 * g;
+    asm volatile("" : "+v"(bias_lds));
+    lds_cfloat* bias = (lds_cfloat*)(uintptr_t)bias_lds;
+    const int64_t ntiles = (a.n + kTile - 1) / kTile;
+    for (int i = lane; i < kPWaveU4; i += 64) pw[i] = make_uint4(0, 0, 0, 0);
+
+#pragma unroll 1
+    for (int64_t tile = blockIdx.x; tile < ntiles; tile += gridDim.x) {
+        const int64_t row0 = tile * kTile + w * kRows;
+        asm volatile("" : "+s"(R.off));
+        int64_t e = row0 + s;
+        const bool mine = e < a.n;
+        if (!mine) e = a.n - 1;
+        X8 X;
+        {
+            const uint4* src = A.live.x + g * A.live.cap + e;
+#pragma unroll
+            for (int k = 0; k < 8; ++k) {
+                X.h[k] = src[(4 * k) * A.live.cap];
+                X.l[k] = src[(4 * k + 2) * A.live.cap];
+            }
+        }
+        float sx = A.live.sx[e];
+        const int rec = A.live.idx[e];
+        fill_pe_wave(pw, true, a, row0, lane);
+        {
+            const float sxin = sx * (256.f * kappa[8]);
+            f32x16 f[8];
+            float m = 0.f;
+#pragma unroll
+            for (int b = 0; b < 8; ++b) {
+                i32x16 t;
+                k_i8<8>(t, X, ring_enter(R, b), R);
+                dequant16(f[b], t, sxin, bias + nm::stage_b_off(8) + 32 * b);
+                m = max16<false>(m, f[b]);
+            }
+            const float M = row_max(m), inv = inv_of(M);
+#pragma unroll
+            for (int b = 0; b < 8; ++b) quant16<false>(f[b], inv, X.h[b], X.l[b]);
+            sx = scale_of(M);
+        }
+        {
+            const float sxin = sx * (256.f * kappa[9]);
+            f32x16 f[4];
+            float m = 0.f;
+#pragma unroll
+            for (int b = 0; b < 4; ++b) {
+                i32x16 t;
+                const uint4* ws = ring_enter(R, 8 + b);
+                k_i8<8>(t, X, ws, R);
+                dequant16(f[b], t, sxin, bias + nm::stage_b_off(9) + 32 * b);
+                k_bf<2>(f[b], pw, g, s, ws + 8 * kStepU4);
+                m = max16<true>(m, f[b]);
+            }
+            const float M = row_max(m), inv = inv_of(M);
+#pragma unroll
+            for (int b = 0; b < 4; ++b) quant16<true>(f[b], inv, X.h[b], X.l[b]);
+            sx = scale_of(M);
+        }
+        {
+            i32x16 t;
+            f32x16 fr;
+            k_i8<4>(t, X, ring_enter(R, 12), R);
+            dequant16(fr, t, sx * (256.f * kappa[10]), bias + nm::stage_b_off(10));
+            if (g == 0 && mine) {
+                float* o = a.out + (int64_t)rec * 4;
+                o[0] = fr[0] * u_r; o[1] = fr[1] * u_g; o[2] = fr[2] * u_b;
+            }
+        }
+    }
+    asm volatile("s_waitcnt vmcnt(0)" ::: "memory");
+}
+
+}
+
+namespace nm {
+
+int launch_mlp_i8h(const MlpLaunch& L, const void* head8, const float* direction, int S, const LiveList& live, int64_t max_entries, float* out,
+                   hipStream_t stream) {
+    Args8s A;
+    MlpArgs& a = A.a;
+    a.ray_idx = live.idx;
+    a.n_rays_dev = live.count;
+    a.s0 = 0;
+    a.S_total = S;
+    a.wpack = nullptr; a.bias = nullptr;
+    a.petab = L.petab;
+    a.pts = nullptr; a.dirs = nullptr; a.origin = nullptr; a.direction = direction; a.z = nullptr;
+    a.out = out; a.dbg = nullptr; a.prof = nullptr; a.n = max_entries; a.S = S; a.in_mode = 3; a.stop_stage = -2; a.sigma_scale = 1.f;
+    a.sigma_only = 0;
+    a.save_h = nullptr; a.save_hv = nullptr; a.save_bits = nullptr; a.save_h16 = nullptr; a.save_feat16 = nullptr; a.save_hvbits = nullptr; a.save_x0h = nullptr; a.save_d0h = nullptr;
+    a.pos = PeSpec{L.pe_kind, L.pos_nfreq, L.pos_octaves};
+    a.dir = PeSpec{L.pe_kind, L.dir_nfreq, L.dir_octaves};
+    A.consts8 = L.consts8;
+    A.image8 = reinterpret_cast<const uint4*>(head8);
+    A.live = live;
+    const int64_t ntiles = (max_entries + kTile - 1) / kTile;
+    int dev = 0, cus = 256;
+    if (hipGetDevice(&dev) == hipSuccess) {
+        int v = 0;
+        if (hipDeviceGetAttribute(&v, hipDeviceAttributeMultiprocessorCount, dev) == hipSuccess && v > 0) cus = v;
+    }
+    const int grid = (int)(ntiles < cus ? ntiles : cus);
+    hipLaunchKernelGGL(nerf_head_i8s_kernel, dim3(grid), dim3(kWaves * 64), 0, stream, A);
+    return check_launch("nerf_head_i8s_kernel");
+}
+
+}
diff --git a/ml-neuman_amd/csrc/mlp_i8s.hip b/ml-neuman_amd/csrc/mlp_i8s.hip
--- a/ml-neuman_amd/csrc/mlp_i8s.hip
+++ b/ml-neuman_amd/csrc/mlp_i8s.hip
@@ -2,106 +2,19 @@
 
 namespace {
 
-constexpr int kWaves = 8;
-constexpr int kTile = kWaves * kRows;
-constexpr int kPWaveU4 = nm::kPeChunks * 2 * kRows;
-constexpr int kPeU4 = kWaves * kPWaveU4;
-constexpr int kStepU4 = nm::kStepBytes / 16;
-constexpr int kSlotU4 = 12 * kStepU4;
-constexpr int kSlots = 3;
-constexpr int kBiasU4 = (nm::kBiasFloats + 16 + 3) / 4;
 constexpr int kTileBlocks = 82;
 __host__ __device__ constexpr int block_steps(int i) {
     i = i >= kTileBlocks ? i - kTileBlocks : i;
     return i < 8 ? 4 : i < 77 ? 8 : i < 81 ? 10 : 4;
 }
-__host__ __device__ constexpr int block_pieces(int nsteps) { return (2 * nsteps + kWaves - 1) / kWaves; }
-
-struct Ring {
-    const char* src;
-    const uint4* rd;
-    unsigned lds0;
-    int off;
-    int slot;
-    int refill, np, nsteps2;
+struct TileStream {
+    static __host__ __device__ constexpr int steps(int i) { return block_steps(i); }
+    static constexpr int kBytes = (int)nm::kWeightBytes8;
 };
-__device__ __forceinline__ void ring_piece(const Ring& R, int off, int slot, int j) {
-    glds16(R.src + off + j * (kWaves * 1024), __builtin_amdgcn_readfirstlane(R.lds0 + slot * (kSlotU4 * 16) + j * (kWaves * 1024)));
-}
-__device__ __forceinline__ void ring_advance(Ring& R, int nsteps) {
-    R.off += nsteps * nm::kStepBytes;
-    if (R.off == (int)nm::kWeightBytes8) R.off = 0;
-}
-__device__ __forceinline__ const uint4* ring_enter(Ring& R, int i) {
-    const int np1 = block_pieces(block_steps(i + 1));
-    if (np1 == 1) asm volatile("s_waitcnt vmcnt(1)" ::: "memory");
-    else if (np1 == 2) asm volatile("s_waitcnt vmcnt(2)" ::: "memory");
-    else asm volatile("s_waitcnt vmcnt(3)" ::: "memory");
-    __builtin_amdgcn_s_barrier();
-    const uint4* cur = R.rd + R.slot * kSlotU4;
-    R.refill = R.slot == 0 ? kSlots - 1 : R.slot - 1;
-    R.slot = R.slot == kSlots - 1 ? 0 : R.slot + 1;
-    R.np = block_pieces(block_steps(i + 2));
-    R.nsteps2 = block_steps(i + 2);
-    return cur;
-}
-__device__ __forceinline__ void ring_copy(Ring& R, int j) {
-    if (j < R.np) ring_piece(R, R.off, R.refill, j);
-    if (j == R.np - 1) ring_advance(R, R.nsteps2);
-}
-struct W8 {
-    uint4 h, l;
-};
-
-template <int NSTEPS, bool PEND, bool RELU = true>
-__device__ __forceinline__ void k_i8_impl(i32x16& t, const X8& X, const uint4* ws, Ring& R, f32x16& fp, const i32x16& tp, lds_cfloat* bias_blk,
-                                          float sx256, float& m) {
-    i32x16 ah, ac;
-#pragma unroll
-    for (int r = 0; r < 16; ++r) { ah[r] = 0; ac[r] = 0; }
-    W8 w[2];
-    w[0].h = ws[0]; w[0].l = ws[64];
-    w[1].h = ws[kStepU4]; w[1].l = ws[kStepU4 + 64];
-#pragma unroll
-    for (int s = 0; s < NSTEPS; ++s) {
-        const uint4 wh = w[s & 1].h, wl = w[s & 1].l;
-        ac = __builtin_amdgcn_mfma_i32_32x32x32_i8(as_i32x4(wh), as_i32x4(X.l[s]), ac, 0, 0, 0);
-        ah = __builtin_amdgcn_mfma_i32_32x32x32_i8(as_i32x4(wh), as_i32x4(X.h[s]), ah, 0, 0, 0);
-        ac = __builtin_amdgcn_mfma_i32_32x32x32_i8(as_i32x4(wl), as_i32x4(X.h[s]), ac, 0, 0, 0);
-        if (s + 2 < NSTEPS) { w[s & 1].h = ws[(s + 2) * kStepU4]; w[s & 1].l = ws[(s + 2) * kStepU4 + 64]; }
-        if (s == 0 || s == 2 || s == 4) ring_copy(R, s >> 1);
-        if (PEND) {
-            const int r = 2 * s;
-            const float b0 = bias_blk[8 * (r >> 2) + (r & 3)], b1 = bias_blk[8 * (r >> 2) + (r & 3) + 1];
-            const float f0 = fmaf((float)tp[r], sx256, b0), f1 = fmaf((float)tp[r + 1], sx256, b1);
-            fp[r] = f0;
-            fp[r + 1] = f1;
-            m = RELU ? fmaxf(m, fmaxf(f0, f1)) : fmaxf(m, fmaxf(fabsf(f0), fabsf(f1)));
-            __builtin_amdgcn_sched_barrier(0);
-        }
-    }
-#pragma unroll
-    for (int r = 0; r < 16; ++r) t[r] = (ah[r] << 8) + ac[r];
-}
-template <int NSTEPS>
-__device__ __forceinline__ void k_i8(i32x16& t, const X8& X, const uint4* ws, Ring& R) {
-    f32x16 nf;
-    float nm_ = 0.f;
-    k_i8_impl<NSTEPS, false>(t, X, ws, R, nf, t, nullptr, 0.f, nm_);
-}
-template <int NSTEPS, bool COPY = false>
-__device__ __forceinline__ void k_bf(f32x16& f, const uint4* pw, int g, int s, const uint4* ws, Ring* R = nullptr, int j0 = 0) {
-#pragma unroll
-    for (int t = 0; t < NSTEPS; ++t) {
-        if (COPY && (t == 1 || t == 3)) ring_copy(*R, j0 + (t >> 1));
-        const uint4 wh = ws[t * kStepU4], wl = ws[t * kStepU4 + 64];
-        const uint4 xh = pw[(2 * t + g) * (2 * kRows) + s], xl = pw[(2 * t + g) * (2 * kRows) + kRows + s];
-        f = __builtin_amdgcn_mfma_f32_32x32x16_bf16(as_bf16x8(wh), as_bf16x8(xl), f, 0, 0, 0);
-        f = __builtin_amdgcn_mfma_f32_32x32x16_bf16(as_bf16x8(wl), as_bf16x8(xh), f, 0, 0, 0);
-        f = __builtin_amdgcn_mfma_f32_32x32x16_bf16(as_bf16x8(wh), as_bf16x8(xh), f, 0, 0, 0);
-    }
-}
-template <bool PLAIN>
+typedef RingT<TileStream> Ring;
+
+enum { WHOLE = 0, PLAIN = 1, TRUNK = 2 };
+template <int MODE>
 __global__ __launch_bounds__(kWaves * 64, 2) void nerf_mlp_i8s_kernel(const Args8s A) {
     __shared__ uint4 lds[kPeU4 + kSlots * kSlotU4 + kBiasU4];
     const MlpArgs a = resolve_args(A.a);
@@ -188,11 +101,11 @@
 #pragma unroll
             for (int b = 0; b < 8; ++b) quant16<true>(f[b], inv, X.h[b], X.l[b]);
             sx = scale_of(M);
-            if (st == 5 && !(PLAIN && a.sigma_only == 2)) {
+            if (st == 5 && !(MODE != WHOLE && a.sigma_only == MODE + 1)) {
                 fill_pe_wave(pw, true, a, row0, lane);
             }
         }
-        if (PLAIN && a.sigma_only == 2) {
+        if (MODE == PLAIN && a.sigma_only == 2) {
             i32x16 t;
             f32x16 fo;
             k_i8<8>(t, X, ring_enter(R, 68), R);
@@ -204,6 +117,34 @@
             R.off = (block_steps(0) + block_steps(1)) * nm::kStepBytes;
             continue;
         }
+        if (MODE == TRUNK && a.sigma_only == 3) {
+            i32x16 t;
+            f32x16 fa;
+            k_i8<8>(t, X, ring_enter(R, 68), R);
+            dequant16(fa, t, sx * (256.f * kappa[8]), bias + nm::stage_b_off(8) + 256);
+            const float sigma = fa[0] * u_sigma;
+            const float v = sigma * a.sigma_scale;
+            const int64_t i = row0 + s;
+            if (g == 0 && i < a.n) reinterpret_cast<float4*>(a.out)[sample_record(a, i)] = make_float4(0.f, 0.f, 0.f, v);
+            const unsigned live = (unsigned)__builtin_amdgcn_ballot_w64(g == 0 && i < a.n && !(v <= 0.f));
+            if (live) {
+                int base = 0;
+                if (lane == 0) base = atomicAdd(A.live.count, __builtin_popcount(live));
+                base = __builtin_amdgcn_readfirstlane(base);
+                if ((live >> s) & 1) {
+                    const int64_t e = base + __builtin_popcount(live & ((1u << s) - 1u));
+                    uint4* dst = A.live.x + g * A.live.cap + e;
+#pragma unroll
+                    for (int k = 0; k < 8; ++k) {
+                        dst[(4 * k) * A.live.cap] = X.h[k];
+                        dst[(4 * k + 2) * A.live.cap] = X.l[k];
+                    }
+                    if (g == 0) { A.live.sx[e] = sx; A.live.idx[e] = (int)i; }
+                }
+            }
+            R.off = (block_steps(0) + block_steps(1)) * nm::kStepBytes;
+            continue;
+        }
         float sigma;
         {
             const float sxin = sx * (256.f * kappa[8]);
@@ -266,7 +207,7 @@
 namespace nm {
 
 int launch_mlp_i8s(const MlpLaunch& L, const void* image8, const float* pts, const float* dirs, const float* origin, const float* direction,
-                   const float* z, int64_t n, int S, int in_mode, float sigma_scale, float* out, hipStream_t stream, const MlpChunk* chunk) {
+                   const float* z, int64_t n, int S, int in_mode, float sigma_scale, float* out, hipStream_t stream, const MlpChunk* chunk, const LiveList* live) {
     Args8s A;
     MlpArgs& a = A.a;
     a.ray_idx = chunk ? chunk->ray_idx : nullptr;
@@ -277,12 +218,13 @@
     a.petab = L.petab;
     a.pts = pts; a.dirs = dirs; a.origin = origin; a.direction = direction; a.z = z;
     a.out = out; a.dbg = nullptr; a.prof = nullptr; a.n = n; a.S = S; a.in_mode = in_mode; a.stop_stage = -2; a.sigma_scale = sigma_scale;
-    a.sigma_only = L.plain_head ? 2 : 0;
+    a.sigma_only = L.plain_head ? 2 : live ? 3 : 0;
     a.save_h = nullptr; a.save_hv = nullptr; a.save_bits = nullptr; a.save_h16 = nullptr; a.save_feat16 = nullptr; a.save_hvbits = nullptr; a.save_x0h = nullptr; a.save_d0h = nullptr;
     a.pos = PeSpec{L.pe_kind, L.pos_nfreq, L.pos_octaves};
     a.dir = PeSpec{L.pe_kind, L.dir_nfreq, L.dir_octaves};
     A.consts8 = L.consts8;
     A.image8 = reinterpret_cast<const uint4*>(image8);
+    A.live = live ? *live : LiveList{nullptr, nullptr, nullptr, nullptr, 0};
     const int64_t ntiles = (n + kTile - 1) / kTile;
     int dev = 0, cus = 256;
     if (hipGetDevice(&dev) == hipSuccess) {
@@ -290,8 +232,9 @@
         if (hipDeviceGetAttribute(&v, hipDeviceAttributeMultiprocessorCount, dev) == hipSuccess && v > 0) cus = v;
     }
     const int grid = (int)(ntiles < cus ? ntiles : cus);
-    if (L.plain_head) hipLaunchKernelGGL(nerf_mlp_i8s_kernel<true>, dim3(grid), dim3(kWaves * 64), 0, stream, A);
-    else hipLaunchKernelGGL(nerf_mlp_i8s_kernel<false>, dim3(grid), dim3(kWaves * 64), 0, stream, A);
+    if (L.plain_head) hipLaunchKernelGGL(nerf_mlp_i8s_kernel<PLAIN>, dim3(grid), dim3(kWaves * 64), 0, stream, A);
+    else if (live) hipLaunchKernelGGL(nerf_mlp_i8s_kernel<TRUNK>, dim3(grid), dim3(kWaves * 64), 0, stream, A);
+    else hipLaunchKernelGGL(nerf_mlp_i8s_kernel<WHOLE>, dim3(grid), dim3(kWaves * 64), 0, stream, A);
     return check_launch("nerf_mlp_i8s_kernel");
 }
 
diff --git a/ml-neuman_amd/csrc/mlp_launch.h b/ml-neuman_amd/csrc/mlp_launch.h
--- a/ml-neuman_amd/csrc/mlp_launch.h
+++ b/ml-neuman_amd/csrc/mlp_launch.h
@@ -37,8 +37,14 @@
 int launch_mlp_mfma(const MlpLaunch& L, const float* pts, const float* dirs, const float* origin, const float* direction,
                     const float* z, int64_t n, int S, int in_mode, int precision, int stop_stage, float sigma_scale, float* out,
                     float* dbg, void* prof, hipStream_t stream, int sigma_only = 0, const MlpChunk* chunk = nullptr);
+struct LiveList {
+    uint4* x; float* sx; int* idx; int* count; int64_t cap;
+};
 int launch_mlp_i8s(const MlpLaunch& L, const void* image8, const float* pts, const float* dirs, const float* origin, const float* direction,
-                   const float* z, int64_t n, int S, int in_mode, float sigma_scale, float* out, hipStream_t stream, const MlpChunk* chunk);
+                   const float* z, int64_t n, int S, int in_mode, float sigma_scale, float* out, hipStream_t stream, const MlpChunk* chunk,
+                   const LiveList* live = nullptr);
+int launch_mlp_i8h(const MlpLaunch& L, const void* head8, const float* direction, int S, const LiveList& live, int64_t max_entries, float* out,
+                   hipStream_t stream);
 int sigma_f16t_ndir();
 int launch_sigma_f16t(const MlpLaunch& L, const void* stream16t, int stream_ndir, const float* pts, const float* dirs, const float* origin, const float* direction,
                       const float* z, int64_t n, int S, int in_mode, float sigma_scale, float* out, hipStream_t stream, const MlpChunk* chunk,
diff --git a/ml-neuman_amd/neuman_hip/_lib.py b/ml-neuman_amd/neuman_hip/_lib.py
--- a/ml-neuman_amd/neuman_hip/_lib.py
+++ b/ml-neuman_amd/neuman_hip/_lib.py
@@ -50,6 +50,9 @@
     "nm_mlp_pack_bytes": (i64, [ctypes.POINTER(MlpDesc)]),
     "nm_mlp_pack_i8s_bytes": (i64, [ctypes.POINTER(MlpDesc)]),
     "nm_mlp_pack_i8s": (i32, [ctypes.POINTER(MlpDesc), ctypes.POINTER(ctypes.c_void_p), ctypes.c_void_p]),
+    "nm_mlp_pack_i8s_trunk_bytes": (i64, [ctypes.POINTER(MlpDesc)]),
+    "nm_mlp_pack_i8s_head_bytes": (i64, [ctypes.POINTER(MlpDesc)]),
+    "nm_mlp_pack_i8s_live": (i32, [ctypes.POINTER(MlpDesc), ctypes.POINTER(ctypes.c_void_p), ctypes.c_void_p, ctypes.c_void_p]),
     "nm_mlp_pack": (i32, [ctypes.POINTER(MlpDesc), ctypes.POINTER(ctypes.c_void_p), ctypes.c_void_p]),
     "nm_mlp_pack_f16": (i32, [ctypes.POINTER(MlpDesc), ctypes.POINTER(ctypes.c_void_p), ctypes.c_void_p]),
     "nm_mlp_pack_i8_bytes": (i64, [ctypes.POINTER(MlpDesc)]),
@@ -71,6 +74,8 @@
     "nm_mlp_backward_chain16": (i32, [ctypes.c_void_p, ctypes.c_void_p, c_f32p, c_f32p, ctypes.c_void_p, i64, c_f32p, ctypes.c_void_p, ctypes.c_void_p, c_f32p, c_f32p,
                                       c_f32p, c_f32p, i64, c_stream]),
     "nm_mlp_forward_rays": (i32, [ctypes.c_void_p, c_f32p, c_f32p, c_f32p, i64, i32, i32, ctypes.c_float, c_f32p, c_stream]),
+    "nm_mlp_forward_rays_live_workspace_bytes": (i64, [i64, i32, i64]),
+    "nm_mlp_forward_rays_live": (i32, [ctypes.c_void_p, c_f32p, c_f32p, c_f32p, i64, i32, i32, ctypes.c_float, c_f32p, ctypes.c_void_p, i64, i64, c_stream]),
     "nm_mlp_sigma_rays": (i32, [ctypes.c_void_p, c_f32p, c_f32p, c_f32p, i64, i32, i32, ctypes.c_float, c_f32p, c_stream]),
     "nm_mlp_forward_ray_chunk": (i32, [ctypes.c_void_p, c_f32p, c_f32p, c_f32p, i32, c_i32p, c_i32p, i64, i32, i32, i32, ctypes.c_float, c_f32p,
                                        c_stream]),
diff --git a/ml-neuman_amd/neuman_hip/render_utils.py b/ml-neuman_amd/neuman_hip/render_utils.py
--- a/ml-neuman_amd/neuman_hip/render_utils.py
+++ b/ml-neuman_amd/neuman_hip/render_utils.py
@@ -263,7 +263,7 @@
     return z_fine, None
 
 
-def bkg_shade(net, o, d, z, precision=None, trace=None, occluder=None, dz=None):
+def bkg_shade(net, o, d, z, precision=None, trace=None, occluder=None, dz=None, composite_only=False):
     if _occupancy_on(net):
         return _occupancy_pass(net, o, d, z, precision, 'shading', False, trace, 'occupancy')
     if TERMINATION_EPS > 0:
@@ -271,11 +271,11 @@
         raw = march_pass_rays(net, o, d, z, TERMINATION_EPS, precision=precision, stats=stats, occluder=occluder, dz=dz)
         _note(trace, march=stats)
         return raw
-    return net.forward_rays(o, d, z, precision=precision, role='shading')
+    return net.forward_rays(o, d, z, precision=precision, role='composite' if composite_only else 'shading')
 
 
 def bkg_pass_rays(coarse_net, fine_net, o, d, near, far, samples_per_ray, importance_samples_per_ray, white_bkg,
-                  precision=None, trace=None, given_z=None, occluder=None, dz=None):
+                  precision=None, trace=None, given_z=None, occluder=None, dz=None, composite_only=False):
     net = fine_net if fine_net is not None else coarse_net
     if given_z is not None:
         z = given_z.to(torch.float32).contiguous()
@@ -283,7 +283,7 @@
         return net.forward_rays(o, d, z, precision=precision, role='shading'), z
     z, raw = bkg_place_z(coarse_net, fine_net, o, d, near, far, samples_per_ray, importance_samples_per_ray, white_bkg, precision, trace)
     if raw is None:
-        raw = bkg_shade(net, o, d, z, precision, trace, occluder, dz)
+        raw = bkg_shade(net, o, d, z, precision, trace, occluder, dz, composite_only)
     _note(trace, bkg_z=z)
     return raw, z
 
@@ -298,7 +298,7 @@
         n = torch.full((j - i,), float(near), device=o.device, dtype=torch.float32)
         f = torch.full((j - i,), float(far), device=o.device, dtype=torch.float32)
         raw, z = bkg_pass_rays(coarse_net, fine_net, oc, dc, n, f, samples_per_ray, importance_samples_per_ray, white_bkg,
-                               precision, trace, given['bkg_z'][i:j] if given is not None and 'bkg_z' in given else None)
+                               precision, trace, given['bkg_z'][i:j] if given is not None and 'bkg_z' in given else None, composite_only=True)
         rgb[i:j], _, _, _, depth[i:j] = raw2outputs(raw, z, dc, white_bkg=white_bkg, want_weights=False)
     return rgb, depth
 
diff --git a/ml-neuman_amd/neuman_hip/vanilla.py b/ml-neuman_amd/neuman_hip/vanilla.py
--- a/ml-neuman_amd/neuman_hip/vanilla.py
+++ b/ml-neuman_amd/neuman_hip/vanilla.py
@@ -176,7 +176,7 @@
     def _prec(self, precision, role=None):
         p = precision or self.precision
         if p == 'mixed':
-            p = 'i8x3' if role == 'shading' else 'fp16x3'
+            p = 'i8x3' if role in ('shading', 'composite') else 'fp16x3'
         return _lib.PRECISIONS[p]
 
     @staticmethod
@@ -220,10 +220,18 @@
             return None
         return train.two_views(self, input_pts, input_views, other_views)
 
-    def forward_rays(self, origin, direction, z_vals, precision=None, sigma_scale=1.0, role=None, sigma_only=False):
+    def forward_rays(self, origin, direction, z_vals, precision=None, sigma_scale=1.0, role=None, sigma_only=False, chunk_samples=0):
         self._guard(origin, direction, z_vals)
         R, S = z_vals.shape
         out = torch.empty((R, S, 4), device=z_vals.device, dtype=torch.float32)
+        if role == 'composite' and not sigma_only and self.nerf.use_viewdirs and self._prec(precision, role) == _lib.NM_PREC_I8X3:
+            nbytes = _lib.lib().nm_mlp_forward_rays_live_workspace_bytes(R, S, int(chunk_samples))
+            ws = torch.empty((nbytes,), device=z_vals.device, dtype=torch.uint8)
+            _lib.check(_lib.lib().nm_mlp_forward_rays_live(
+                self.handle(), _lib.dev_ptr(origin, name='origin'), _lib.dev_ptr(direction, name='direction'), _lib.dev_ptr(z_vals, name='z_vals'), R, S,
+                self._prec(precision, role), float(sigma_scale), _lib.dev_ptr(out), _lib.dev_ptr(ws, torch.uint8), nbytes, int(chunk_samples),
+                _lib.stream_ptr()), "nm_mlp_forward_rays_live")
+            return out
         entry = _lib.lib().nm_mlp_sigma_rays if sigma_only else _lib.lib().nm_mlp_forward_rays
         _lib.check(entry(self.handle(), _lib.dev_ptr(origin, name='origin'), _lib.dev_ptr(direction, name='direction'),
                          _lib.dev_ptr(z_vals, name='z_vals'), R, S, self._prec(precision, role), float(sigma_scale),
```

After: 1.513 million (median of 6 runs). +4.6%, better.
